# Youngju-Na/UFORecon

Hardware: AMD Instinct MI355X
Metric: rays/s (per-ray volume-rendering path, 64+64 hierarchical samples, DTU-shaped 3-view 512x640) (higher is better)
Workload: dtype f32; 1 GPU; configs[1]: full 512x640 frame = 327680 rays, 3 source views, 64+64 samples, rays sharded by row tiles over 1 GPU(s), depth/RGB tiles all-gathered; rays_per_frame=327680, chunk_rays=4096, side_streams=3

## Files before the change

uforecon_amd/csrc/composite.hip:

```cpp
#include "ufr_internal.h"

#pragma clang fp contract(off)

namespace ufr {

constexpr int kMaxK = 4;

__device__ __forceinline__ float sigmoidf(float x) { return 1.f / (1.f + expf(-x)); }

__device__ __forceinline__ float wave_sum(float v) {
#pragma unroll
  for (int d = 32; d >= 1; d >>= 1) v += __shfl_xor(v, d);
  return v;
}

__global__ void __launch_bounds__(256) composite_kernel(const float* __restrict__ z, const float* __restrict__ radiance,
                                                         const int* __restrict__ rad_row, const float* __restrict__ srdf,
                                                         const float* __restrict__ variance, int RN, int SN,
                                                         float* __restrict__ rgb, float* __restrict__ depth,
                                                         float* __restrict__ opacity, float* __restrict__ weight,
                                                         const float* __restrict__ camz, float* __restrict__ depth_z) {
  const int wave = threadIdx.x >> 6, lane = threadIdx.x & 63;
  const int ray = blockIdx.x * 4 + wave;
  if (ray >= RN) return;
  const float* zr = z + (size_t)ray * SN;
  const float* sr = srdf + (size_t)ray * SN;
  const float inv_s = fminf(fmaxf(expf(variance[0] * 10.0f), 1e-6f), 1e6f);
  const int K = (SN + 63) / 64;

  float alpha[kMaxK], zz[kMaxK];
  float prod = 1.f;
#pragma unroll
  for (int k = 0; k < kMaxK; ++k) {
    alpha[k] = 0.f;
    zz[k] = 0.f;
    int i = lane * K + k;
    if (k < K && i < SN) {
      float zc = zr[i];
      float gl = (i == 0) ? zr[1] - zr[0] : zc - zr[i - 1];
      float gr = (i == SN - 1) ? zr[SN - 1] - zr[SN - 2] : zr[i + 1] - zc;
      float interval = (gl + gr) / 2.f;
      float s = sr[i];
      const float iter_cos = -1.5f;
      float nxt = s + iter_cos * interval * 0.5f;
      float prv = s - iter_cos * interval * 0.5f;
      float pc = sigmoidf(prv * inv_s), nc = sigmoidf(nxt * inv_s);
      float a = ((pc - nc) + 1e-5f) / (pc + 1e-5f);
      a = fminf(fmaxf(a, 0.f), 1.f);
      alpha[k] = a;
      zz[k] = zc;
      prod *= (1.f - a) + 1e-7f;
    }
  }
  float incl = prod;
#pragma unroll
  for (int d = 1; d < 64; d <<= 1) {
    float o = __shfl_up(incl, d);
    if (lane >= d) incl *= o;
  }
  float T = __shfl_up(incl, 1);
  if (lane == 0) T = 1.f;

  float acc_d = 0.f, acc_o = 0.f, acc_r = 0.f, acc_g = 0.f, acc_b = 0.f;
#pragma unroll
  for (int k = 0; k < kMaxK; ++k) {
    int i = lane * K + k;
    if (k < K && i < SN) {
      float w = alpha[k] * T;
      T *= (1.f - alpha[k]) + 1e-7f;
      if (weight) weight[(size_t)ray * SN + i] = w;
      const float* c = radiance + (rad_row ? (size_t)rad_row[(size_t)ray * SN + i] : (size_t)ray * SN + i) * 3;
      acc_r += c[0] * w;
      acc_g += c[1] * w;
      acc_b += c[2] * w;
      acc_d += w * zz[k];
      acc_o += w;
    }
  }
  acc_d = wave_sum(acc_d);
  acc_o = wave_sum(acc_o);
  acc_r = wave_sum(acc_r);
  acc_g = wave_sum(acc_g);
  acc_b = wave_sum(acc_b);
  if (lane == 0) {
    depth[ray] = acc_d;
    if (opacity) opacity[ray] = acc_o;
    if (rgb) {
      rgb[3 * ray + 0] = acc_r;
      rgb[3 * ray + 1] = acc_g;
      rgb[3 * ray + 2] = acc_b;
    }
    if (depth_z) depth_z[ray] = acc_d * camz[ray];
  }
}

__global__ void __launch_bounds__(256) composite_bwd_kernel(const float* __restrict__ z, const float* __restrict__ radiance,
                                                             const int* __restrict__ rad_row, int accumulate,
                                                             const float* __restrict__ srdf,
                                                             const float* __restrict__ variance, int RN, int SN,
                                                             const float* __restrict__ d_rgb, const float* __restrict__ d_depth,
                                                             const float* __restrict__ d_opacity,
                                                             const float* __restrict__ d_weight,
                                                             float* __restrict__ d_radiance, float* __restrict__ d_srdf,
                                                             float* __restrict__ d_variance) {
  const int wave = threadIdx.x >> 6, lane = threadIdx.x & 63;
  const int ray = blockIdx.x * 4 + wave;
  if (ray >= RN) return;
  const float* zr = z + (size_t)ray * SN;
  const float* sr = srdf + (size_t)ray * SN;
  const float e10 = expf(variance[0] * 10.0f);
  const float inv_s = fminf(fmaxf(e10, 1e-6f), 1e6f);
  const bool s_live = e10 >= 1e-6f && e10 <= 1e6f;
  const int K = (SN + 63) / 64;
  const float gr = d_rgb ? d_rgb[3 * ray + 0] : 0.f, gg = d_rgb ? d_rgb[3 * ray + 1] : 0.f, gb = d_rgb ? d_rgb[3 * ray + 2] : 0.f;
  const float gd = d_depth ? d_depth[ray] : 0.f, go = d_opacity ? d_opacity[ray] : 0.f;

  float alpha[kMaxK], araw[kMaxK], pcv[kMaxK], ncv[kMaxK], prvv[kMaxK], nxtv[kMaxK];
  float prod = 1.f;
#pragma unroll
  for (int k = 0; k < kMaxK; ++k) {
    alpha[k] = 0.f; araw[k] = 0.f; pcv[k] = 0.f; ncv[k] = 0.f; prvv[k] = 0.f; nxtv[k] = 0.f;
    const int i = lane * K + k;
    if (k < K && i < SN) {
      const float zc = zr[i];
      const float gl = (i == 0) ? zr[1] - zr[0] : zc - zr[i - 1];
      const float gr_ = (i == SN - 1) ? zr[SN - 1] - zr[SN - 2] : zr[i + 1] - zc;
      const float interval = (gl + gr_) / 2.f;
      const float s = sr[i];
      const float nxt = s + -1.5f * interval * 0.5f, prv = s - -1.5f * interval * 0.5f;
      const float pc = sigmoidf(prv * inv_s), nc = sigmoidf(nxt * inv_s);
      const float a = ((pc - nc) + 1e-5f) / (pc + 1e-5f);
      araw[k] = a; pcv[k] = pc; ncv[k] = nc; prvv[k] = prv; nxtv[k] = nxt;
      alpha[k] = fminf(fmaxf(a, 0.f), 1.f);
      prod *= (1.f - alpha[k]) + 1e-7f;
    }
  }
  float incl = prod;
#pragma unroll
  for (int d = 1; d < 64; d <<= 1) {
    const float o = __shfl_up(incl, d);
    if (lane >= d) incl *= o;
  }
  float T = __shfl_up(incl, 1);
  if (lane == 0) T = 1.f;

  float w[kMaxK], dw[kMaxK], Tk[kMaxK], lane_sum = 0.f;
#pragma unroll
  for (int k = 0; k < kMaxK; ++k) {
    w[k] = 0.f; dw[k] = 0.f; Tk[k] = 0.f;
    const int i = lane * K + k;
    if (k < K && i < SN) {
      Tk[k] = T;
      w[k] = alpha[k] * T;
      T *= (1.f - alpha[k]) + 1e-7f;
      const size_t slot = (size_t)ray * SN + i, rrow = rad_row ? (size_t)rad_row[slot] : slot;
      const float* c = radiance + rrow * 3;
      dw[k] = (d_weight ? d_weight[slot] : 0.f) + gr * c[0] + gg * c[1] + gb * c[2] + gd * zr[i] + go;
      lane_sum += dw[k] * w[k];
      float* dr = d_radiance + rrow * 3;
      if (accumulate) { dr[0] += w[k] * gr; dr[1] += w[k] * gg; dr[2] += w[k] * gb; }
      else { dr[0] = w[k] * gr; dr[1] = w[k] * gg; dr[2] = w[k] * gb; }
    }
  }
  float suf = lane_sum;
#pragma unroll
  for (int d = 1; d < 64; d <<= 1) {
    const float o = __shfl_down(suf, d);
    if (lane + d < 64) suf += o;
  }
  float after = __shfl_down(suf, 1);
  if (lane == 63) after = 0.f;

  float dvar = 0.f;
#pragma unroll
  for (int k = kMaxK - 1; k >= 0; --k) {
    const int i = lane * K + k;
    if (k < K && i < SN) {
      const float dalpha = dw[k] * Tk[k] - after / ((1.f - alpha[k]) + 1e-7f);
      after += dw[k] * w[k];
      const float da = (araw[k] >= 0.f && araw[k] <= 1.f) ? dalpha : 0.f;
      const float den = pcv[k] + 1e-5f;
      const float dpc = da * (1.f - araw[k]) / den, dnc = -da / den;
      const float spc = pcv[k] * (1.f - pcv[k]), snc = ncv[k] * (1.f - ncv[k]);
      d_srdf[(size_t)ray * SN + i] = (dpc * spc + dnc * snc) * inv_s;
      dvar += dpc * spc * prvv[k] + dnc * snc * nxtv[k];
    }
  }
  dvar = wave_sum(dvar);
  if (lane == 0 && s_live) atomicAdd(d_variance, dvar * 10.f * inv_s);
}

hipError_t launch_composite_bwd(const float* z, const float* radiance, const int* rad_row, bool accumulate, const float* srdf,
                                const float* variance, int RN, int SN, const float* d_rgb, const float* d_depth,
                                const float* d_opacity, const float* d_weight, float* d_radiance, float* d_srdf,
                                float* d_variance, hipStream_t s) {
  if (SN > 64 * kMaxK || SN < 2) return hipErrorInvalidValue;
  hipLaunchKernelGGL(composite_bwd_kernel, dim3((RN + 3) / 4), dim3(256), 0, s, z, radiance, rad_row, accumulate ? 1 : 0, srdf,
                     variance, RN, SN, d_rgb,
                     d_depth, d_opacity, d_weight, d_radiance, d_srdf, d_variance);
  return hipGetLastError();
}

hipError_t launch_composite(const float* z, const float* radiance, const int* rad_row, const float* srdf,
                            const float* variance, int RN, int SN, float* rgb, float* depth, float* opacity, float* weight,
                            const float* camz, float* depth_z, hipStream_t s) {
  if (SN > 64 * kMaxK || SN < 2) return hipErrorInvalidValue;
  hipLaunchKernelGGL(composite_kernel, dim3((RN + 3) / 4), dim3(256), 0, s, z, radiance, rad_row, srdf, variance, RN, SN, rgb,
                     depth, opacity, weight, camz, depth_z);
  return hipGetLastError();
}

}
```

uforecon_amd/csrc/ray_transformer.hip:

```cpp
#include "bwd_tape.h"
#include "ufr_internal.h"
#include "weight_stream_f16.h"

namespace ufr {

__device__ __forceinline__ void load_ray_tile(const float* __restrict__ token0, const int* __restrict__ tok_row,
                                              const float* __restrict__ order_pe, size_t tok_base, int s_base, int g,
                                              int j, f32x4 (&x)[6]) {
  const float* row = token0 + (tok_row ? (size_t)tok_row[tok_base + j] : tok_base + j) * UFR_TOKEN_DIM;
#pragma unroll
  for (int t = 0; t < 5; ++t) x[t] = ld4(row + 16 * t + 4 * g);
  const float* pe = order_pe + (size_t)(s_base + j) * 8 + 2 * g;
  x[5] = f32x4{pe[0], pe[1], 0.f, 0.f};
}

template <int VW, int VB, int C, class WS>
__device__ __forceinline__ void layer_norm88(f32x4 (&tt)[C][6], const WS& ws, int g, float eps, float asc, f32x4 (*XH)[6] = nullptr, float* RS = nullptr) {
#pragma unroll
  for (int c = 0; c < C; ++c) {
    f32x4 (&t)[6] = tt[c];
    float s = 0.f;
#pragma unroll
    for (int i = 0; i < 5; ++i) s += (t[i][0] + t[i][1]) + (t[i][2] + t[i][3]);
    s += t[5][0] + t[5][1];
    const float mean = sum_groups(s) * (1.f / 88.f);
    float q = 0.f;
#pragma unroll
    for (int i = 0; i < 6; ++i)
#pragma unroll
      for (int r = 0; r < 4; ++r) {
        if (i < 5 || r < 2) {
          float d = t[i][r] - mean;
          q = fmaf(d, d, q);
        }
      }
    const float rstd = fast_rsqrt(sum_groups(q) * (1.f / 88.f) + eps);
    if (RS) RS[c] = rstd * asc;
#pragma unroll
    for (int i = 0; i < 6; ++i) {
      const f32x4 gw = vec_frag<VW>(ws, i, g), gb = vec_frag<VB>(ws, i, g);
#pragma unroll
      for (int r = 0; r < 4; ++r) {
        const float xh = (t[i][r] - mean) * rstd;
        if (XH) XH[c][i][r] = (i == 5 && r >= 2) ? 0.f : xh;
        t[i][r] = xh * gw[r] + gb[r];
      }
    }
  }
}

constexpr int kRtBlock = 256;
constexpr int kRtMinW = 2;
constexpr int kRtWaves = kRtBlock / 64;

#ifdef UFR_PHASE_TIMING
__device__ unsigned long long g_rt_phase[32];
#define UFR_RT_PHASE(i)                                                                \
  {                                                                                    \
    const unsigned long long t_now = __builtin_readcyclecounter();                     \
    rt_acc[i] += t_now - rt_prev;                                                      \
    rt_prev = t_now;                                                                   \
  }
#else
#define UFR_RT_PHASE(i)
#endif

template <bool LOWP, bool TAPE = false>
__global__ void __launch_bounds__(kRtBlock, TAPE ? 2 : kRtMinW) ray_transformer_kernel(const float* __restrict__ packed,
                                                                  const float* __restrict__ token0,
                                                                  const int* __restrict__ tok_row,
                                                                  const float* __restrict__ order_pe, int RN, int SN,
                                                                  float* __restrict__ srdf,
                                                                  float* __restrict__ ray_out,
                                                                  int* __restrict__ status, float* __restrict__ tape = nullptr,
                                                                  float* __restrict__ ray_state = nullptr) {
  extern __shared__ __attribute__((aligned(16))) char smem[];
  auto ws = wstream_f16_begin<kRtWaves, LOWP>(packed, smem);
  wstream_f16_prime<B_RT1, kRtWaves>(ws);
  const int lane = threadIdx.x & 63, g = lane >> 4, j = lane & 15;
  const int ray_raw = (blockIdx.x * blockDim.x + threadIdx.x) >> 6;
  const bool valid = ray_raw < RN;
  const int ray = valid ? ray_raw : RN - 1;
  const int n_tiles = SN / 16;
  const int n_iter = n_tiles;
  const auto sc = scalar_file<false, ray_scalars_offset()>(ws);
  const float xs_x = sc[RS_XS_X];
  const float k_dsc = sc[RS_K_DSC], k_l2e = sc[RS_K_L2E], q_dsc = sc[RS_Q_DSC], q_l2e = sc[RS_Q_L2E];
  const float inv_len = uniform_f32(sc[RS_V_DSC] / (float)SN), f_len = uniform_f32((float)SN * sc[RS_V_ASC]);
  const bool pow2_len = (SN & (SN - 1)) == 0;

#ifdef UFR_PHASE_TIMING
  unsigned long long rt_acc[16] = {};
  unsigned long long rt_prev = __builtin_readcyclecounter();
#endif
  f32x4 KV[8], KVT[TAPE ? 8 : 1];
#pragma unroll
  for (int h = 0; h < 8; ++h) KV[h] = splat4(0.f);
#pragma unroll
  for (int h = 0; h < (TAPE ? 8 : 1); ++h) KVT[h] = splat4(0.f);
  for (int it = 0; it < n_iter; ++it) {
    constexpr int C = 1;
    const bool wrap = it + 1 < n_iter;
    const bool slot_ok = head11_slot(j) >= 0;
    f32x4 x[C][6], kt[C][8], vt[C][8];
    bool live[C];
#pragma unroll
    for (int c = 0; c < C; ++c) {
      const int tile = it * C + c;
      live[c] = tile < n_tiles;
      const int tl = live[c] ? tile : n_tiles - 1;
      load_ray_tile(token0, tok_row, order_pe, (size_t)ray * SN + tl * 16, tl * 16, g, j, x[c]);
#pragma unroll
      for (int h = 0; h < 8; ++h) { kt[c][h] = splat4(0.f); vt[c][h] = splat4(0.f); }
    }
    {
      BWords<C> cur;
      split_units<0, 0, 4 * C>(x, cur, xs_x);
      static_for<3>([&](auto si) __attribute__((always_inline)) {
        constexpr int s = decltype(si)::value;
        BStep b[C];
        bwords_to_bstep(cur, b);
        if constexpr (s < 2) {
          BWords<C> nxt;
          gemm_f16_panel<M_RT_K, s, C, kRtWaves, true>(ws, b, kt, wrap, [&](auto ti) __attribute__((always_inline)) {
            constexpr int to = decltype(ti)::value;
            split_units<s + 1, to * 4 * C / 8, (to + 1) * 4 * C / 8>(x, nxt, xs_x);
          });
          gemm_f16_panel<M_RT_V, s, C, kRtWaves, true>(ws, b, vt, wrap);
          cur = nxt;
        } else {
          gemm_f16_panel<M_RT_K, s, C, kRtWaves, true>(ws, b, kt, wrap);
          gemm_f16_panel<M_RT_V, s, C, kRtWaves, true>(ws, b, vt, wrap);
        }
      });
      probe_gemm(kt, ws);
      probe_gemm(vt, ws);
    }
    UFR_RT_PHASE(0)
    const float pad_v = (TAPE ? j == 3 : (j & 3) == 3) ? 1.f : 0.f;
#pragma unroll
    for (int c = 0; c < C; ++c) {
      float kk[8][4], vv[8][4];
      if (pow2_len) {
#pragma unroll
        for (int h = 0; h < 8; ++h)
#pragma unroll
          for (int r = 0; r < 4; ++r) vv[h][r] = vt[c][h][r] * inv_len;
      } else {
#pragma unroll
        for (int h = 0; h < 8; ++h)
#pragma unroll
          for (int r = 0; r < 4; ++r) vv[h][r] = vt[c][h][r] / f_len;
      }
      const bool k_ok = slot_ok && live[c];
#pragma unroll
      for (int h = 0; h < 8; ++h)
#pragma unroll
        for (int r = 0; r < 4; ++r) {
          const float e = elu1_acc(kt[c][h][r], k_dsc, k_l2e);
          kk[h][r] = k_ok ? e : 0.f;
          vv[h][r] = slot_ok ? vv[h][r] : pad_v;
        }
#pragma unroll
      for (int r = 0; r < 4; ++r) {
#pragma unroll
        for (int h = 0; h < 8; ++h) {
          KV[h] = mfma16(kk[h][r], vv[h][r], KV[h]);
          if constexpr (TAPE) KVT[h] = mfma16(vv[h][r], kk[h][r], KVT[h]);
        }
      }
    }
    wstream_f16_finish<B_RT1, kRtWaves>(ws, wrap);
    UFR_RT_PHASE(1)
  }

  if constexpr (TAPE) {
    if (valid) {
      float* st = ray_state + (size_t)ray * (kRayStateTiles * kTileFloats) + lane * 4;
#pragma unroll
      for (int h = 0; h < 8; ++h) { st4(st + h * kTileFloats, KV[h]); st4(st + (8 + h) * kTileFloats, KVT[h]); }
    }
  }
  wstream_f16_prime<B_RT2, kRtWaves>(ws);
  constexpr int C = 1;
  const int n_iter2 = TAPE ? n_iter + (n_iter & 1) : n_iter;
  typedef RayTapeLayout<LOWP> TapeL;
  for (int it = 0; it < n_iter2; ++it) {
    const bool wrap = it + 1 < n_iter2;
    char* const tape_blk = reinterpret_cast<char*>(tape) + ((size_t)ray * (n_iter2 / 2) + it / 2) * (TapeL::block_units * 512);
    auto tape_st = [&](int tile, f32x4 v) __attribute__((always_inline)) {
      if (valid) tile_store<TapeL>(tape_blk, tile, it & 1, lane, v);
    };
    f32x4 x[C][6], q[C][6], msg[C][6];
    bool live[C];
    int tbase[C];
#pragma unroll
    for (int c = 0; c < C; ++c) {
      const int tile = it * C + c;
      live[c] = tile < n_tiles;
      tbase[c] = (live[c] ? tile : n_tiles - 1) * 16;
      load_ray_tile(token0, tok_row, order_pe, (size_t)ray * SN + tbase[c], tbase[c], g, j, x[c]);
#pragma unroll
      for (int t = 0; t < 6; ++t) q[c][t] = splat4(0.f);
    }
    track_external(x, ws);
    gemm_f16<M_RT_Q, C, kRtWaves>(ws, x, q, wrap, xs_x);
    float zs_all[8];
    if constexpr (TAPE) {
#pragma unroll
      for (int t = 0; t < 6; ++t) {
        tape_st(RT_X + t, live[0] ? x[0][t] : splat4(0.f));
        f32x4 qq;
#pragma unroll
        for (int r = 0; r < 4; ++r) qq[r] = quad11(t, g, r) >= 0 ? elu1_acc(q[0][t][r], q_dsc, q_l2e) : 0.f;
        tape_st(RT_Q + t, qq);
      }
    }
    UFR_RT_PHASE(2)
#pragma unroll
    for (int c = 0; c < C; ++c) {
      static_for<8>([&](auto hi) __attribute__((always_inline)) {
        constexpr int h = decltype(hi)::value;
        f32x4 acc = splat4(0.f);
        static_for<3>([&](auto qi) __attribute__((always_inline)) {
          constexpr int qd = decltype(qi)::value, quad = 3 * h + qd;
          const float qq = (3 * g + qd < 11) ? elu1_acc(q[c][quad >> 2][quad & 3], q_dsc, q_l2e) : 0.f;
          acc = mfma16(KV[h][qd], qq, acc);
        });
        const float den = TAPE ? __shfl(acc[3], j) : acc[3];
        const float Z = fast_rcp(den + 1e-6f);
        const float zs = Z * (float)SN;
        if constexpr (TAPE) zs_all[h] = zs;
        static_for<3>([&](auto ri) __attribute__((always_inline)) {
          constexpr int rr = decltype(ri)::value, quad = 3 * h + rr;
          msg[c][quad >> 2][quad & 3] = acc[rr] * zs;
        });
      });
    }
    UFR_RT_PHASE(3)
    if constexpr (TAPE) {
#pragma unroll
      for (int t = 0; t < 6; ++t) tape_st(RT_MSG + t, msg[0][t]);
      tape_st(RT_ZS, f32x4{zs_all[0], zs_all[1], zs_all[2], zs_all[3]});
      tape_st(RT_ZS + 1, f32x4{zs_all[4], zs_all[5], zs_all[6], zs_all[7]});
    }
    f32x4 m[C][6];
#pragma unroll
    for (int c = 0; c < C; ++c)
#pragma unroll
      for (int t = 0; t < 6; ++t) m[c][t] = splat4(0.f);
    gemm_f16<M_RT_MERGE, C, kRtWaves>(ws, msg, m, wrap, sc[RS_M_XS]);
    UFR_RT_PHASE(4)
    float rstd1[C] = {}, rstd2[C] = {};
    if constexpr (TAPE) {
      f32x4 xh[C][6];
      layer_norm88<V_RT_N1W, V_RT_N1B, C>(m, ws, g, sc[RS_EPS1], sc[RS_M_ASC], xh, rstd1);
#pragma unroll
      for (int t = 0; t < 6; ++t) { tape_st(RT_XH1 + t, xh[0][t]); tape_st(RT_M + t, m[0][t]); }
    } else {
      layer_norm88<V_RT_N1W, V_RT_N1B, C>(m, ws, g, sc[RS_EPS1], 1.f);
    }
    UFR_RT_PHASE(5)

    f32x4 cat[C][12], hid[C][11], o[C][6];
#pragma unroll
    for (int c = 0; c < C; ++c) {
#pragma unroll
      for (int t = 0; t < 6; ++t) { cat[c][t] = x[c][t]; cat[c][6 + t] = m[c][t]; }
#pragma unroll
      for (int t = 0; t < 11; ++t) hid[c][t] = splat4(0.f);
    }
    gemm_f16<M_RT_MLP0, C, kRtWaves>(ws, cat, hid, wrap, xs_x);
    UFR_RT_PHASE(6)
#pragma unroll
    for (int c = 0; c < C; ++c) {
#pragma unroll
      for (int t = 0; t < 11; ++t)
#pragma unroll
        for (int r = 0; r < 4; ++r) hid[c][t][r] = relu_acc(hid[c][t][r]);
#pragma unroll
      for (int t = 0; t < 6; ++t) o[c][t] = splat4(0.f);
    }
    unsigned relu_bits[2] = {0u, 0u};
    if constexpr (TAPE) {
#pragma unroll
      for (int t = 0; t < 11; ++t) {
        tape_st(RT_HID + t, hid[0][t] * sc[RS_MLP0_DSC]);
#pragma unroll
        for (int r = 0; r < 4; ++r)
          if (hid[0][t][r] > 0.f) relu_bits[(4 * t + r) >> 5] |= 1u << ((4 * t + r) & 31);
      }
    }
    gemm_f16<M_RT_MLP2, C, kRtWaves>(ws, hid, o, wrap, sc[RS_M_MLP2]);
    UFR_RT_PHASE(7)
    if constexpr (TAPE) {
      f32x4 xh[C][6];
      layer_norm88<V_RT_N2W, V_RT_N2B, C>(o, ws, g, sc[RS_EPS2], sc[RS_MLP2_ASC], xh, rstd2);
#pragma unroll
      for (int t = 0; t < 6; ++t) tape_st(RT_XH2 + t, xh[0][t]);
    } else {
      layer_norm88<V_RT_N2W, V_RT_N2B, C>(o, ws, g, sc[RS_EPS2], 1.f);
    }
    UFR_RT_PHASE(8)
#pragma unroll
    for (int c = 0; c < C; ++c) {
#pragma unroll
      for (int t = 0; t < 6; ++t)
#pragma unroll
        for (int r = 0; r < 4; ++r) o[c][t][r] += x[c][t][r];
      if constexpr (TAPE) {
#pragma unroll
        for (int t = 0; t < 6; ++t) tape_st(RT_O + t, o[c][t]);
      }
      if (ray_out && valid && live[c]) {
        float* row = ray_out + ((size_t)ray * SN + tbase[c] + j) * UFR_RAY_DIM;
#pragma unroll
        for (int t = 0; t < 5; ++t) st4(row + 16 * t + 4 * g, o[c][t]);
        row[80 + 2 * g] = o[c][5][0];
        row[81 + 2 * g] = o[c][5][1];
      }
    }

    f32x4 d1[C][2], d2[C][1], d3[C][1];
#pragma unroll
    for (int c = 0; c < C; ++c) {
      d1[c][0] = vec_frag<V_DM_B0>(ws, 0, g) * sc[RS_DM0_ASC];
      d1[c][1] = vec_frag<V_DM_B0>(ws, 1, g) * sc[RS_DM0_ASC];
      d2[c][0] = vec_frag<V_DM_B2>(ws, 0, g) * sc[RS_DM2_ASC];
      d3[c][0] = vec_frag<V_DM_B4>(ws, 0, g) * sc[RS_DM4_ASC];
    }
    gemm_f16<M_DM0, C, kRtWaves>(ws, o, d1, wrap, sc[RS_DM0_XS]);
#pragma unroll
    for (int c = 0; c < C; ++c)
#pragma unroll
      for (int t = 0; t < 2; ++t)
#pragma unroll
        for (int r = 0; r < 4; ++r) d1[c][t][r] = relu_acc(d1[c][t][r]);
    gemm_f16<M_DM2, C, kRtWaves>(ws, d1, d2, wrap, sc[RS_M_DM2]);
#pragma unroll
    for (int c = 0; c < C; ++c)
#pragma unroll
      for (int r = 0; r < 4; ++r) d2[c][0][r] = relu_acc(d2[c][0][r]);
    if constexpr (TAPE) {
#pragma unroll
      for (int t = 0; t < 2; ++t) {
        tape_st(RT_D1 + t, d1[0][t] * sc[RS_DM0_DSC]);
#pragma unroll
        for (int r = 0; r < 4; ++r)
          if (d1[0][t][r] > 0.f) relu_bits[(44 + 4 * t + r) >> 5] |= 1u << ((44 + 4 * t + r) & 31);
      }
      tape_st(RT_D2, d2[0][0] * sc[RS_DM2_DSC]);
#pragma unroll
      for (int r = 0; r < 4; ++r)
        if (d2[0][0][r] > 0.f) relu_bits[1] |= 1u << (52 + r - 32);
      tape_st(RT_MISC, f32x4{rstd1[0], rstd2[0], __builtin_bit_cast(float, relu_bits[0]), __builtin_bit_cast(float, relu_bits[1])});
    }
    gemm_f16<M_DM4, C, kRtWaves>(ws, d2, d3, wrap, sc[RS_M_DM4]);
#pragma unroll
    for (int c = 0; c < C; ++c)
      if (g == 0 && valid && live[c]) srdf[(size_t)ray * SN + tbase[c] + j] = d3[c][0][0] * sc[RS_DM4_DSC];
    wstream_f16_finish<B_RT2, kRtWaves>(ws, wrap);
    UFR_RT_PHASE(9)
  }
  wstream_report_range(ws, status);
#ifdef UFR_PHASE_TIMING
  if (ray_raw == 5 && lane == 0)
    for (int i = 0; i < 16; ++i) g_rt_phase[i] += rt_acc[i];
#endif
}

template <bool LOWP, bool TAPE = false>
static hipError_t launch_rt(const float* packed, const float* token0, const int* tok_row, const float* order_pe, int RN,
                            int SN, float* srdf, float* ray_out, int* status, hipStream_t s, float* tape = nullptr,
                            float* ray_state = nullptr) {
  static LdsAttrOnce lds_attr;
  if (const hipError_t attr = lds_attr.set(reinterpret_cast<const void*>(&ray_transformer_kernel<LOWP, TAPE>), kF16LdsBytes); attr != hipSuccess) return attr;
  hipLaunchKernelGGL((ray_transformer_kernel<LOWP, TAPE>), dim3((RN + kRtWaves - 1) / kRtWaves), dim3(kRtBlock), kF16LdsBytes, s,
                     packed, token0, tok_row, order_pe, RN, SN, srdf, ray_out, status, tape, ray_state);
  return hipGetLastError();
}

hipError_t launch_ray_tape(const float* packed, const float* token0, const int* tok_row, const float* order_pe, int RN, int SN,
                           float* srdf, float* tape, float* ray_state, bool lowp, int* status, hipStream_t s) {
  if (SN % 16 != 0 || SN < 16) return hipErrorInvalidValue;
  return lowp ? launch_rt<true, true>(packed, token0, tok_row, order_pe, RN, SN, srdf, nullptr, status, s, tape, ray_state)
              : launch_rt<false, true>(packed, token0, tok_row, order_pe, RN, SN, srdf, nullptr, status, s, tape, ray_state);
}

hipError_t launch_ray_transformer(const float* packed, const float* token0, const int* tok_row, const float* order_pe,
                                  int RN, int SN, float* srdf, float* ray_out, bool lowp, int* status, hipStream_t s) {
  if (SN % 16 != 0 || SN < 16) return hipErrorInvalidValue;
  return lowp ? launch_rt<true>(packed, token0, tok_row, order_pe, RN, SN, srdf, ray_out, status, s)
              : launch_rt<false>(packed, token0, tok_row, order_pe, RN, SN, srdf, ray_out, status, s);
}

}

#ifdef UFR_PHASE_TIMING
extern "C" int ufr_debug_rt_phases(unsigned long long* out, int n, int reset) {
  unsigned long long h[32] = {};
  if (hipMemcpyFromSymbol(h, HIP_SYMBOL(ufr::g_rt_phase), sizeof(h)) != hipSuccess) return -1;
  for (int i = 0; i < n && i < 32; ++i) out[i] = h[i];
  if (reset) {
    unsigned long long z[32] = {};
    if (hipMemcpyToSymbol(HIP_SYMBOL(ufr::g_rt_phase), z, sizeof(z)) != hipSuccess) return -1;
  }
  return 0;
}
#endif
```

uforecon_amd/csrc/sampler.hip:

```cpp
#include "ufr_internal.h"

#pragma clang fp contract(off)

namespace ufr {

__global__ void __launch_bounds__(256) ray_setup_kernel(const int64_t* __restrict__ ray_idx,
                                                         const float* __restrict__ ray_d,
                                                         const float* __restrict__ cam_ray_d, int HW, float near_z,
                                                         float far_z, int RN, float* __restrict__ rd_out,
                                                         float* __restrict__ near_out, float* __restrict__ far_out,
                                                         float* __restrict__ camz_out, float ox, float oy, float oz,
                                                         float* __restrict__ ray_o_out) {
  int i = blockIdx.x * blockDim.x + threadIdx.x;
  if (i == 0 && ray_o_out) { ray_o_out[0] = ox; ray_o_out[1] = oy; ray_o_out[2] = oz; }
  if (i >= RN) return;
  int64_t p = ray_idx[i];
  const bool in_range = p >= 0 && p < (int64_t)HW;
  p = in_range ? p : 0;
  rd_out[3 * i + 0] = ray_d[p];
  rd_out[3 * i + 1] = ray_d[(size_t)HW + p];
  rd_out[3 * i + 2] = ray_d[2 * (size_t)HW + p];
  float cz = cam_ray_d ? cam_ray_d[2 * (size_t)HW + p] : 1.f;
  const float bad = __builtin_nanf("");
  near_out[i] = !in_range ? bad : cam_ray_d ? near_z / cz : near_z;
  far_out[i] = !in_range ? bad : cam_ray_d ? far_z / cz : far_z;
  if (camz_out) camz_out[i] = cz;
}

hipError_t launch_ray_setup(const int64_t* ray_idx, const float* ray_d, const float* cam_ray_d, int HW, float near_z,
                            float far_z, int RN, float* rd_out, float* near_out, float* far_out, float* camz_out,
                            const float* ray_o_host, float* ray_o_out, hipStream_t s) {
  hipLaunchKernelGGL(ray_setup_kernel, dim3((RN + 255) / 256), dim3(256), 0, s, ray_idx, ray_d, cam_ray_d, HW, near_z,
                     far_z, RN, rd_out, near_out, far_out, camz_out, ray_o_host ? ray_o_host[0] : 0.f,
                     ray_o_host ? ray_o_host[1] : 0.f, ray_o_host ? ray_o_host[2] : 0.f, ray_o_out);
  return hipGetLastError();
}

__global__ void __launch_bounds__(256) sample_fixed_kernel(const float* __restrict__ near,
                                                            const float* __restrict__ far,
                                                            const float* __restrict__ U, int u_stride,
                                                            float* __restrict__ z, int RN, int SN) {
  size_t i = (size_t)blockIdx.x * blockDim.x + threadIdx.x;
  if (i >= (size_t)RN * SN) return;
  int s = (int)(i / RN), ray = (int)(i % RN);
  double step = 1.0 / (double)(SN - 1);
  float lin = (s == SN - 1) ? 1.0f : (float)((double)s * step);
  float n = near[ray], f = far[ray];
  float zz = lin * (f - n) + n;
  float interval = (float)(1.0 / (double)(SN - 1));
  zz = zz + (U[(size_t)s * u_stride + ray] - 0.5f) * interval * (f - n);
  z[(size_t)ray * SN + s] = zz;
}

hipError_t launch_sample_fixed(const float* near, const float* far, const float* U, int u_stride, float* z, int RN,
                               int SN, hipStream_t s) {
  size_t n = (size_t)RN * SN;
  hipLaunchKernelGGL(sample_fixed_kernel, dim3((unsigned)((n + 255) / 256)), dim3(256), 0, s, near, far, U, u_stride, z,
                     RN, SN);
  return hipGetLastError();
}

__global__ void __launch_bounds__(256) points_kernel(const float* __restrict__ ray_o, int o_stride,
                                                      const float* __restrict__ ray_d, const float* __restrict__ z,
                                                      float* __restrict__ pts, int RN, int SN) {
  size_t i = (size_t)blockIdx.x * blockDim.x + threadIdx.x;
  if (i >= (size_t)RN * SN) return;
  int ray = (int)(i / SN);
  float zz = z[i];
  const float* o = ray_o + (size_t)ray * o_stride;
  pts[3 * i + 0] = o[0] + zz * ray_d[3 * ray + 0];
  pts[3 * i + 1] = o[1] + zz * ray_d[3 * ray + 1];
  pts[3 * i + 2] = o[2] + zz * ray_d[3 * ray + 2];
}

hipError_t launch_points(const float* ray_o, int o_stride, const float* ray_d, const float* z, float* pts, int RN,
                         int SN, hipStream_t s) {
  size_t n = (size_t)RN * SN;
  hipLaunchKernelGGL(points_kernel, dim3((unsigned)((n + 255) / 256)), dim3(256), 0, s, ray_o, o_stride, ray_d, z, pts,
                     RN, SN);
  return hipGetLastError();
}

constexpr int kMaxS = 256;

__device__ __forceinline__ double wave_incl_scan(double v, int lane) {
#pragma unroll
  for (int d = 1; d < 64; d <<= 1) {
    double o = __shfl_up(v, d);
    if (lane >= d) v += o;
  }
  return v;
}

__global__ void __launch_bounds__(256) importance_merge_kernel(const float* __restrict__ weight,
                                                                const float* __restrict__ z,
                                                                const float* __restrict__ U2, int u_stride,
                                                                float* __restrict__ z_fine, float* __restrict__ z_all,
                                                                int RN, int SN, int PN, float* __restrict__ z_new,
                                                                int* __restrict__ src_row) {
  __shared__ float lds[4][3 * kMaxS];
  const int wave = threadIdx.x >> 6, lane = threadIdx.x & 63;
  const int ray = blockIdx.x * 4 + wave;
  const bool active = ray < RN;
  float* cdf = lds[wave];
  float* all = cdf + kMaxS;
  float* zf = all + SN;
  const float* w = weight + (size_t)(active ? ray : 0) * SN;

  const int K = (SN + 63) / 64;
  double run = 0.0;
  for (int k = 0; k < K; ++k) {
    int i = lane * K + k;
    if (i < SN) run += (double)w[i];
  }
  double incl = wave_incl_scan(run, lane);
  float total;
  {
    float a4[4] = {0.f, 0.f, 0.f, 0.f};
    const int l8 = lane & 7;
    for (int c = 0; c * 32 < SN; ++c)
#pragma unroll
      for (int k = 0; k < 4; ++k) {
        int i = (c * 4 + k) * 8 + l8;
        if (i < SN) a4[k] += w[i];
      }
    const float t = ((a4[0] + a4[1]) + a4[2]) + a4[3];
    total = __shfl(t, 0);
#pragma unroll
    for (int l = 1; l < 8; ++l) total += __shfl(t, l);
  }
  float denom = total + 1e-6f;
  double acc = incl - run;
  for (int k = 0; k < K; ++k) {
    int i = lane * K + k;
    if (i < SN) {
      acc += (double)w[i];
      cdf[i] = (float)acc / denom;
      all[i] = z[(size_t)(active ? ray : 0) * SN + i];
    }
  }
  __syncthreads();

  const float c_first = cdf[0], c_last = cdf[SN - 1];
  for (int k = lane; k < PN; k += 64) {
    float u = U2[(size_t)k * u_stride + (active ? ray : 0)];
    u = fminf(fmaxf(u, c_first), c_last);
    int lo = 0, hi = SN;
    while (lo < hi) {
      int mid = (lo + hi) >> 1;
      if (cdf[mid] < u) lo = mid + 1; else hi = mid;
    }
    int ri = lo < 1 ? 1 : (lo > SN - 1 ? SN - 1 : lo);
    float cl = cdf[ri - 1], cr = cdf[ri], zl = all[ri - 1], zr = all[ri];
    zf[k] = (u - cl) / (cr - cl + 1e-6f) * (zr - zl) + zl;
  }
  __syncthreads();
  if (!active) return;

  if (z_fine) {
    for (int k = lane; k < PN; k += 64) {
      float v = zf[k];
      int rank = 0;
      for (int j = 0; j < PN; ++j) {
        float o = zf[j];
        rank += (o < v || (o == v && j < k)) ? 1 : 0;
      }
      z_fine[(size_t)ray * PN + rank] = v;
    }
  }
  const int T = SN + PN;
  float* out = z_all + (size_t)ray * T;
  bool sorted_coarse = true;
  for (int k = lane; k + 1 < SN; k += 64) sorted_coarse = sorted_coarse && all[k] <= all[k + 1];
  if (__builtin_amdgcn_ballot_w64(!sorted_coarse) == 0ull) {
    float* fs = cdf;
    for (int k = lane; k < PN; k += 64) {
      const float v = zf[k];
      int r = 0;
      for (int j = 0; j < PN; ++j) {
        const float o = zf[j];
        r += (o < v || (o == v && j < k)) ? 1 : 0;
      }
      fs[r] = v;
    }
    __builtin_amdgcn_fence(__ATOMIC_RELEASE, "wavefront");
    __builtin_amdgcn_wave_barrier();
    __builtin_amdgcn_fence(__ATOMIC_ACQUIRE, "wavefront");
    for (int k = lane; k < SN; k += 64) {
      const float v = all[k];
      int lo = 0, hi = PN;
      while (lo < hi) { const int mid = (lo + hi) >> 1; if (fs[mid] < v) lo = mid + 1; else hi = mid; }
      const int rank = k + lo;
      out[rank] = v;
      if (src_row) src_row[(size_t)ray * T + rank] = ray * SN + k;
    }
    for (int r = lane; r < PN; r += 64) {
      const float v = fs[r];
      int lo = 0, hi = SN;
      while (lo < hi) { const int mid = (lo + hi) >> 1; if (all[mid] <= v) lo = mid + 1; else hi = mid; }
      const int rank = r + lo;
      out[rank] = v;
      if (src_row) src_row[(size_t)ray * T + rank] = RN * SN + ray * PN + r;
      if (z_new) z_new[(size_t)ray * PN + r] = v;
    }
    return;
  }
  for (int k = lane; k < T; k += 64) {
    float v = all[k];
    int rank = 0, rank_new = 0;
    for (int j = 0; j < T; ++j) {
      float o = all[j];
      const int before = (o < v || (o == v && j < k)) ? 1 : 0;
      rank += before;
      rank_new += j >= SN ? before : 0;
    }
    out[rank] = v;
    if (src_row) src_row[(size_t)ray * T + rank] = k < SN ? ray * SN + k : RN * SN + ray * PN + rank_new;
    if (z_new && k >= SN) z_new[(size_t)ray * PN + rank_new] = v;
  }
}

hipError_t launch_importance_merge(const float* weight, const float* z, const float* U2, int u_stride, float* z_fine,
                                   float* z_all, int RN, int SN, int PN, float* z_new, int* src_row, hipStream_t s) {
  if (SN > kMaxS || PN > kMaxS || SN < 2) return hipErrorInvalidValue;
  hipLaunchKernelGGL(importance_merge_kernel, dim3((RN + 3) / 4), dim3(256), 0, s, weight, z, U2, u_stride, z_fine,
                     z_all, RN, SN, PN, z_new, src_row);
  return hipGetLastError();
}

}
```

uforecon_amd/csrc/ufr_api.hip:

```cpp
#include <math.h>
#include <stdarg.h>
#include <stdio.h>
#include <stdlib.h>
#include <string.h>

#include <atomic>
#include <mutex>
#include <string>
#include <vector>

#include "bwd_common.h"
#include "bwd_tape.h"
#include "mcubes_table.h"
#include "ufr_internal.h"
#include "ufr_layout_f16.h"

using namespace ufr;

namespace {

thread_local char g_err[512] = "";

int fail(int code, const char* fmt, ...) {
  va_list ap;
  va_start(ap, fmt);
  vsnprintf(g_err, sizeof(g_err), fmt, ap);
  va_end(ap);
  return code;
}
#define UFR_HIP(expr)                                                                    \
  do {                                                                                   \
    hipError_t e_ = (expr);                                                              \
    if (e_ != hipSuccess) return fail(UFR_ERR_HIP, "%s: %s", #expr, hipGetErrorString(e_)); \
  } while (0)
#define UFR_REQUIRE(cond, ...) \
  do {                         \
    if (!(cond)) return fail(UFR_ERR_ARG, __VA_ARGS__); \
  } while (0)

inline size_t align_up(size_t v, size_t a = 256) { return (v + a - 1) / a * a; }

struct Carver {
  char* base;
  size_t off = 0;
  explicit Carver(void* p) : base(static_cast<char*>(p)) {}
  float* f32(size_t n) {
    float* r = base ? reinterpret_cast<float*>(base + off) : nullptr;
    off += align_up(n * sizeof(float));
    return r;
  }
};

struct ProfEntry { const char* name; hipEvent_t a, b; };
std::atomic<bool> g_prof_on{false};
std::vector<ProfEntry> g_prof;
std::mutex g_prof_mu;

struct ProfScope {
  hipStream_t s;
  hipEvent_t a = nullptr, b = nullptr;
  const char* name;
  ProfScope(const char* n, hipStream_t st) : s(st), name(n) {
    if (g_prof_on.load(std::memory_order_relaxed)) {
      hipEventCreate(&a);
      hipEventCreate(&b);
      hipEventRecord(a, s);
    }
  }
  ~ProfScope() {
    if (a) {
      hipEventRecord(b, s);
      std::lock_guard<std::mutex> lock(g_prof_mu);
      g_prof.push_back({name, a, b});
    }
  }
};

__global__ void order_pe_kernel(float* __restrict__ table, int SN) {
  int i = blockIdx.x * blockDim.x + threadIdx.x;
  if (i >= SN * 8) return;
  int pos = i >> 3, jj = i & 7;
  double ang = (double)pos / pow(10000.0, 2.0 * (double)(jj / 2) / 8.0);
  table[i] = (float)((jj & 1) ? cos(ang) : sin(ang));
}

PreSim presim_of(const ufr_raw_weights* r) {
  return PreSim{r->pre_sim.w0, r->pre_sim.b0, r->pre_sim.w2, r->pre_sim.b2, r->pre_sim.w4, r->pre_sim.b4};
}

const FrameDev* frame_of(const ufr_frame* f) {
  const FrameDev* d = reinterpret_cast<const FrameDev*>(f);
  return (f && d->magic == kFrameMagic) ? d : nullptr;
}

}

namespace ufr {
hipError_t launch_order_pe(float* table, int SN, hipStream_t s) {
  hipLaunchKernelGGL(order_pe_kernel, dim3((SN * 8 + 255) / 256), dim3(256), 0, s, table, SN);
  return hipGetLastError();
}
}

namespace {
std::atomic<int> g_matrix_precision{UFR_PRECISION_FP32};

bool resolve_precision(int precision, bool* lowp) {
  if (precision == UFR_PRECISION_DEFAULT) precision = g_matrix_precision.load(std::memory_order_relaxed);
  if (precision != UFR_PRECISION_FP32 && precision != UFR_PRECISION_16BIT) return false;
  *lowp = precision == UFR_PRECISION_16BIT;
  return true;
}
#define UFR_PRECISION(arg, lowp_var, who)                                                        \
  bool lowp_var = false;                                                                          \
  if (!resolve_precision(arg, &lowp_var)) return fail(UFR_ERR_ARG, "%s: unknown precision %d", who, (int)(arg))

struct StatusSlot {
  std::once_flag once;
  int rc = UFR_OK;
  int* dev = nullptr;
  volatile int* host = nullptr;
  std::atomic<int> gen{0};
  std::mutex report_mu;
  hipEvent_t upd = nullptr;
  std::atomic<bool> upd_recorded{false};
};
constexpr int kStatusDevices = 16;
StatusSlot g_status[kStatusDevices];
constexpr int kStatusAll = 7;

__global__ void status_update_kernel(int* dev, int keep_mask, int gen) {
  atomicAnd(dev, keep_mask);
  dev[1] = gen;
}

int status_slot(StatusSlot** out) {
  int dev = 0;
  UFR_HIP(hipGetDevice(&dev));
  UFR_REQUIRE(dev >= 0 && dev < kStatusDevices, "status: device %d out of range", dev);
  StatusSlot& sl = g_status[dev];
  std::call_once(sl.once, [&sl] {
    int* h = nullptr;
    int* d = nullptr;
    if (hipHostMalloc(reinterpret_cast<void**>(&h), 2 * sizeof(int), hipHostMallocDefault) != hipSuccess ||
        hipMalloc(reinterpret_cast<void**>(&d), 2 * sizeof(int)) != hipSuccess || hipMemset(d, 0, 2 * sizeof(int)) != hipSuccess) {
      sl.rc = UFR_ERR_HIP;
      return;
    }
    h[0] = h[1] = 0;
    sl.host = h;
    sl.dev = d;
    if (hipEventCreateWithFlags(&sl.upd, hipEventDisableTiming) != hipSuccess) sl.upd = nullptr;
  });
  if (sl.rc != UFR_OK) return fail(sl.rc, "status: could not allocate the device's status words");
  *out = &sl;
  return UFR_OK;
}

int status_message(int bits, const char* who) {
  return fail(UFR_ERR_RANGE, "%s: range status 0x%x:%s%s%s (include/ufr.h: ufr_status_poll)", who, bits,
              (bits & 1) ? " a dense-layer input left the range of its fp16 planes (a token feature beyond the input_abs_max the weights were packed for -- ufr_weights_pack_for -- or infinite);" : "",
              (bits & 2) ? " NaN among the token / dir inputs handed to a transformer kernel;" : "",
              (bits & 4) ? " ufr_weights_pack met a parameter that is not finite (or an input bound that is not a positive finite number);" : "");
}

int status_consume(StatusSlot* sl, hipStream_t s, int mask, const char* who, int* flags_out) {
  std::lock_guard<std::mutex> lock(sl->report_mu);
  const int bits = sl->host[0], tag = sl->host[1];
  const int cur = sl->gen.load(std::memory_order_relaxed);
  const int hit = tag == cur ? bits & mask : 0;
  if (flags_out) *flags_out = tag == cur ? bits : 0;
  if (hit == 0) return UFR_OK;
  const int next = cur + 1;
  sl->gen.store(next, std::memory_order_relaxed);
  hipLaunchKernelGGL(status_update_kernel, dim3(1), dim3(1), 0, s, sl->dev, ~hit, next);
  UFR_HIP(hipGetLastError());
  if (sl->upd && hipEventRecord(sl->upd, s) == hipSuccess) sl->upd_recorded.store(true, std::memory_order_release);
  return status_message(hit, who);
}
int status_enter(StatusSlot* sl, hipStream_t s, const char* who) { return status_consume(sl, s, kStatusAll, who, nullptr); }
int status_fetch(StatusSlot* sl, hipStream_t s) {
  if (sl->upd_recorded.load(std::memory_order_acquire)) UFR_HIP(hipStreamWaitEvent(s, sl->upd, 0));
  UFR_HIP(hipMemcpyAsync(const_cast<int*>(sl->host), sl->dev, 2 * sizeof(int), hipMemcpyDeviceToHost, s));
  return UFR_OK;
}
int status_leave(StatusSlot* sl, hipStream_t s) { return status_fetch(sl, s); }
}

extern "C" {

int ufr_set_matrix_precision(int mode) {
  UFR_REQUIRE(mode == UFR_PRECISION_FP32 || mode == UFR_PRECISION_16BIT, "ufr_set_matrix_precision: unknown mode %d", mode);
  g_matrix_precision.store(mode, std::memory_order_relaxed);
  return UFR_OK;
}
int ufr_get_matrix_precision(void) { return g_matrix_precision.load(std::memory_order_relaxed); }

int ufr_status_poll_bits(ufr_stream stream, int32_t synchronize, int32_t mask, int32_t* flags_out) {
  StatusSlot* sl = nullptr;
  int rc = status_slot(&sl);
  if (rc != UFR_OK) return rc;
  hipStream_t s = static_cast<hipStream_t>(stream);
  if (synchronize) {
    rc = status_fetch(sl, s);
    if (rc != UFR_OK) return rc;
    UFR_HIP(hipStreamSynchronize(s));
  }
  int flags = 0;
  rc = status_consume(sl, s, mask, "ufr_status_poll", &flags);
  if (flags_out) *flags_out = flags;
  if (rc == UFR_OK && !synchronize) return status_leave(sl, s);
  return rc;
}

int ufr_status_poll(ufr_stream stream, int32_t synchronize, int32_t* flags_out) {
  return ufr_status_poll_bits(stream, synchronize, kStatusAll, flags_out);
}

int ufr_version(void) { return UFR_ABI_VERSION; }
const char* ufr_last_error(void) { return g_err; }

size_t ufr_packed_weights_bytes(void) { return (size_t)blob_floats() * sizeof(float) + (size_t)kF16Bytes + (size_t)kBwdBytes + 16; }
size_t ufr_packed_bwd_halfwords(void) { return (size_t)kBwdHalfwords; }
size_t ufr_packed_fp32_floats(void) { return (size_t)blob_floats(); }
size_t ufr_packed_f16_halfwords(void) { return (size_t)kF16Halfwords; }
size_t ufr_packed_scale_table_offset(void) { return (size_t)scale_table_offset(); }
int ufr_packed_scale_table_entries(void) { return M_COUNT; }

int ufr_pack_plan_f16(int32_t* param_id, int32_t* elem, int32_t* plane) {
  UFR_REQUIRE(param_id && elem && plane, "ufr_pack_plan_f16: null output");
  for (int h = 0; h < kF16Halfwords; ++h) plan_entry_f16(h, &param_id[h], &elem[h], &plane[h]);
  return UFR_OK;
}

int ufr_pack_plan_bwd(int32_t* param_id, int32_t* elem, int32_t* plane) {
  UFR_REQUIRE(param_id && elem && plane, "ufr_pack_plan_bwd: null output");
  for (int h = 0; h < kBwdHalfwords; ++h) plan_entry_f16(kF16Halfwords + h, &param_id[h], &elem[h], &plane[h]);
  return UFR_OK;
}

int ufr_pack_plan(int32_t* param_id, int32_t* elem) {
  UFR_REQUIRE(param_id && elem, "ufr_pack_plan: null output");
  for (int i = 0; i < blob_floats(); ++i) {
    int p, e;
    plan_entry(i, &p, &e);
    param_id[i] = p;
    elem[i] = e;
  }
  return UFR_OK;
}

int ufr_weights_pack_for(const ufr_raw_weights* raw, void* packed, float input_abs_max, ufr_stream stream) {
  UFR_REQUIRE(raw && packed, "ufr_weights_pack: null argument");
  static_assert(sizeof(ufr_raw_weights) == sizeof(RawPtrs), "ufr_raw_weights must be P_COUNT pointers");
  RawPtrs rp;
  memcpy(&rp, raw, sizeof(rp));
  for (int i = 0; i < P_COUNT; ++i) UFR_REQUIRE(rp.p[i], "ufr_weights_pack: parameter %d is null", i);
  UFR_REQUIRE(input_abs_max > 0.f && input_abs_max <= 3.0e38f, "ufr_weights_pack_for: input_abs_max=%g must be positive and finite",
              (double)input_abs_max);
  hipStream_t s = static_cast<hipStream_t>(stream);
  StatusSlot* sl = nullptr;
  int rc = status_slot(&sl);
  if (rc != UFR_OK) return rc;
  UFR_HIP(launch_pack_weights(rp, static_cast<float*>(packed), input_abs_max, sl->dev, s));
  return status_leave(sl, s);
}

int ufr_weights_fit_frame(void* packed, const ufr_frame* frame, ufr_stream stream) {
  const FrameDev* f = frame_of(frame);
  UFR_REQUIRE(packed && f, "ufr_weights_fit_frame: null weights / frame handle not prepared");
  hipStream_t s = static_cast<hipStream_t>(stream);
  StatusSlot* sl = nullptr;
  int rc = status_slot(&sl);
  if (rc != UFR_OK) return rc;
  UFR_HIP(launch_refit_weights(static_cast<float*>(packed), f->abs_max, sl->dev, s));
  return UFR_OK;
}

int ufr_weights_pack(const ufr_raw_weights* raw, void* packed, ufr_stream stream) {
  return ufr_weights_pack_for(raw, packed, kDefaultInputAbsMax, stream);
}

static int frame_check(const ufr_frame_desc* d) {
  UFR_REQUIRE(d, "frame desc is null");
  UFR_REQUIRE(d->NV >= 2 && d->NV <= UFR_MAX_VIEWS, "NV=%d unsupported (2..%d)", d->NV, UFR_MAX_VIEWS);
  UFR_REQUIRE(d->H >= 8 && d->W >= 8 && d->H % 4 == 0 && d->W % 4 == 0, "H,W must be multiples of 4 (got %dx%d)",
              d->H, d->W);
  UFR_REQUIRE(d->source_imgs && d->depth_info && d->feat, "null frame tensor");
  UFR_REQUIRE((long long)d->H * d->W < (1 << 24) && (long long)(d->H / 4) * (d->W / 4) * 32 * (d->NV - 1) < (1ll << 32),
              "image of %dx%d is too large for the gather's 24-bit texel indices", d->H, d->W);
  {
    const long long px = (long long)d->H * d->W, mpx = (long long)(d->H / 4) * (d->W / 4), lim = 1ll << 31;
    UFR_REQUIRE(px * 16 < lim && d->NV * mpx * 128 < lim && d->NV * mpx * 32 * (d->NV - 1) * 4 < lim,
                "frame of %dx%d with %d views: an image / feature-map buffer reaches 2 GiB (the gathers' zero-fill offset)",
                d->H, d->W, d->NV);
  }
  const bool has_vol = d->vol_feat[0] != nullptr;
  for (int s = 0; s < UFR_NUM_STAGES; ++s) {
    UFR_REQUIRE((d->vol_feat[s] != nullptr) == has_vol && (d->vol_weight[s] != nullptr) == has_vol,
                "volumes must be given for all stages or for none (stage %d)", s + 1);
    if (has_vol) UFR_REQUIRE(d->vol_D[s] >= 2 && d->vol_H[s] >= 2 && d->vol_W[s] >= 2, "degenerate volume (stage %d)", s + 1);
    if (has_vol)
      UFR_REQUIRE((long long)d->vol_D[s] * d->vol_H[s] < (1 << 24) && (long long)d->vol_W[s] * kVolCh < (1 << 24) &&
                      (long long)d->vol_D[s] * d->vol_H[s] * d->vol_W[s] * kVolCh * 4 < (1ll << 31),
                  "volume of stage %d is too large for the gather's 31-bit byte offsets (per view: < 2 GiB)", s + 1);
  }
  UFR_REQUIRE(d->source_poses && d->source_cam_pos && d->ref_cam_pos && d->w2c_row2, "null camera constants");
  return UFR_OK;
}

size_t ufr_frame_workspace_bytes(const ufr_frame_desc* d) {
  if (frame_check(d) != UFR_OK) return 0;
  Carver c(nullptr);
  const size_t h = d->H / 4, w = d->W / 4, NV = d->NV;
  c.f32(NV * h * w * 32);
  if (d->match) c.f32(NV * h * w * 32 * (NV - 1));
  c.f32(NV * (size_t)d->H * d->W * 4);
  if (d->vol_feat[0])
    for (int s = 0; s < UFR_NUM_STAGES; ++s) c.f32(NV * (size_t)d->vol_D[s] * d->vol_H[s] * d->vol_W[s] * kVolCh);
  c.f32(64);
  return c.off;
}

int ufr_frame_prepare(const ufr_frame_desc* d, void* workspace, size_t workspace_bytes, ufr_frame* out,
                      ufr_stream stream) {
  int rc = frame_check(d);
  if (rc != UFR_OK) return rc;
  UFR_REQUIRE(workspace && out, "ufr_frame_prepare: null workspace/out");
  if (workspace_bytes < ufr_frame_workspace_bytes(d))
    return fail(UFR_ERR_WORKSPACE, "frame workspace too small: %zu < %zu", workspace_bytes, ufr_frame_workspace_bytes(d));
  hipStream_t s = static_cast<hipStream_t>(stream);
  const int NV = d->NV, h = d->H / 4, w = d->W / 4;
  Carver c(workspace);
  const bool has_vol = d->vol_feat[0] != nullptr;
  float* feat = c.f32((size_t)NV * h * w * 32);
  float* match = d->match ? c.f32((size_t)NV * h * w * 32 * (NV - 1)) : nullptr;
  float* rgb = c.f32((size_t)NV * d->H * d->W * 4);
  float* vol[UFR_NUM_STAGES] = {};
  if (has_vol)
    for (int st = 0; st < UFR_NUM_STAGES; ++st)
      vol[st] = c.f32((size_t)NV * d->vol_D[st] * d->vol_H[st] * d->vol_W[st] * kVolCh);
  unsigned* abs_max = reinterpret_cast<unsigned*>(c.f32(64));

  UFR_HIP(hipMemsetAsync(abs_max, 0, 256, s));
  UFR_HIP(launch_nchw_to_nhwc(d->feat, feat, NV, 32, h * w, 32, s, abs_max));
  if (match) UFR_HIP(launch_nchw_to_nhwc(d->match, match, NV, 32 * (NV - 1), h * w, 32 * (NV - 1), s));
  UFR_HIP(launch_nchw_to_nhwc(d->source_imgs, rgb, NV, 3, d->H * d->W, 4, s));
  if (has_vol)
    for (int st = 0; st < UFR_NUM_STAGES; ++st)
      UFR_HIP(launch_volume_pack(d->vol_feat[st], d->vol_weight[st], vol[st], NV, d->vol_D[st] * d->vol_H[st] * d->vol_W[st], s, abs_max));

  FrameDev f;
  memset(&f, 0, sizeof(f));
  f.NV = NV; f.H = d->H; f.W = d->W; f.h = h; f.w = w; f.match_ch = 32 * (NV - 1);
  f.feat = feat; f.match = match; f.rgb = rgb; f.depth = d->depth_info;
  for (int st = 0; st < UFR_NUM_STAGES; ++st) {
    f.vol[st] = vol[st];
    if (has_vol) { f.vD[st] = d->vol_D[st]; f.vH[st] = d->vol_H[st]; f.vW[st] = d->vol_W[st]; }
  }
  for (int v = 0; v < NV; ++v) {
    memcpy(f.pose[v], d->source_poses + 16 * v, 12 * sizeof(float));
    memcpy(f.cam_pos[v], d->source_cam_pos + 3 * v, 3 * sizeof(float));
    memcpy(f.w2c_z[v], d->w2c_row2 + 4 * v, 4 * sizeof(float));
  }
  memcpy(f.ref_pos, d->ref_cam_pos, 3 * sizeof(float));
  f.vol_near = d->vol_near; f.vol_far = d->vol_far;
  f.abs_max = abs_max;
  f.magic = kFrameMagic;
  memset(out, 0, sizeof(*out));
  memcpy(out, &f, sizeof(f));
  return UFR_OK;
}

int ufr_sample_fixed(const float* near, const float* far, const float* U, float* z_out, int32_t RN, int32_t SN,
                     ufr_stream stream) {
  UFR_REQUIRE(near && far && U && z_out, "ufr_sample_fixed: null argument");
  UFR_REQUIRE(RN > 0 && SN >= 2, "ufr_sample_fixed: RN=%d SN=%d", RN, SN);
  UFR_HIP(launch_sample_fixed(near, far, U, RN, z_out, RN, SN, static_cast<hipStream_t>(stream)));
  return UFR_OK;
}

int ufr_sample_importance_merge(const float* weight, const float* z, const float* U2, float* z_fine, float* z_all,
                                int32_t RN, int32_t SN, int32_t PN, ufr_stream stream) {
  UFR_REQUIRE(weight && z && U2 && z_all, "ufr_sample_importance_merge: null argument");
  UFR_REQUIRE(RN > 0 && SN >= 2 && SN <= 256 && PN >= 1 && PN <= 256, "ufr_sample_importance_merge: RN=%d SN=%d PN=%d",
              RN, SN, PN);
  UFR_HIP(launch_importance_merge(weight, z, U2, RN, z_fine, z_all, RN, SN, PN, nullptr, nullptr,
                                  static_cast<hipStream_t>(stream)));
  return UFR_OK;
}

int ufr_points(const float* ray_o, int32_t ray_o_stride, const float* ray_d, const float* z, float* points, int32_t RN,
               int32_t SN, ufr_stream stream) {
  UFR_REQUIRE(ray_o && ray_d && z && points, "ufr_points: null argument");
  UFR_REQUIRE(ray_o_stride == 0 || ray_o_stride == 3, "ufr_points: ray_o_stride must be 0 or 3");
  UFR_HIP(launch_points(ray_o, ray_o_stride, ray_d, z, points, RN, SN, static_cast<hipStream_t>(stream)));
  return UFR_OK;
}

int ufr_project_gather(const ufr_frame* frame, const ufr_raw_weights* raw, const float* ray_o, int32_t ray_o_stride,
                       const float* ray_d, const float* z, int32_t RN, int32_t SN, float* x_tokens, float* rgb,
                       float* dir, float* sim8, float* vol24, float* xy, float* mask_z, const float* vol24_in,
                       const float* sim8_in, ufr_stream stream) {
  const FrameDev* f = frame_of(frame);
  UFR_REQUIRE(f, "ufr_project_gather: frame handle not prepared");
  UFR_REQUIRE(raw && ray_o && ray_d && z && x_tokens && rgb && dir, "ufr_project_gather: null argument");
  UFR_REQUIRE(ray_o_stride == 0 || ray_o_stride == 3, "ufr_project_gather: ray_o_stride must be 0 or 3");
  UFR_REQUIRE(RN > 0 && SN > 0, "ufr_project_gather: RN=%d SN=%d", RN, SN);
  UFR_REQUIRE(f->match || sim8_in, "ufr_project_gather: the frame has no matching features: sim8_in is required");
  UFR_REQUIRE(f->vol[0] || vol24_in, "ufr_project_gather: the frame has no volumes: vol24_in is required");
  ProfScope prof("gather", static_cast<hipStream_t>(stream));
  UFR_HIP(launch_gather(*f, presim_of(raw), ray_o, ray_o_stride, ray_d, z, RN, SN, x_tokens, nullptr, rgb, dir, sim8, vol24, xy,
                        mask_z, vol24_in, sim8_in, static_cast<hipStream_t>(stream)));
  return UFR_OK;
}

size_t ufr_aggregate_workspace_bytes(int32_t RN, int32_t SN, int32_t NV) {
  (void)NV;
  Carver c(nullptr);
  c.f32((size_t)RN * SN * UFR_TOKEN_DIM);
  c.f32((size_t)SN * 8);
  return c.off;
}

static int aggregate_impl(const void* packed, const float* x_tokens, const float* x_point, const float* rgb, const float* dir, int RN, int SN,
                          int NV, float* radiance, float* srdf, float* token0, float* order_pe, bool pe_ready,
                          float* view_out, float* ray_out, bool lowp, int* status, hipStream_t s) {
  UFR_REQUIRE((unsigned long long)RN * SN * (NV + 1) * UFR_TOKEN_DIM < (1ull << 30),
              "view transformer: %d x %d points x %d tokens exceed the 2^30 token values one call addresses; chunk the points", RN, SN, NV + 1);
  {
    ProfScope ps("view_transformer", s);
    UFR_HIP(launch_view_transformer(static_cast<const float*>(packed), x_tokens, x_point, rgb, dir, RN * SN, NV, token0, radiance,
                                    view_out, lowp, status, s));
  }
  if (!pe_ready) UFR_HIP(launch_order_pe(order_pe, SN, s));
  {
    ProfScope ps("ray_transformer", s);
    UFR_HIP(launch_ray_transformer(static_cast<const float*>(packed), token0, nullptr, order_pe, RN, SN, srdf, ray_out, lowp,
                                   status, s));
  }
  return UFR_OK;
}

int ufr_aggregate(const void* packed_weights, const float* x_tokens, const float* rgb, const float* dir, int32_t RN,
                  int32_t SN, int32_t NV, float* radiance, float* srdf, void* workspace, float* view_out,
                  float* ray_out, int32_t precision, ufr_stream stream) {
  UFR_REQUIRE(packed_weights && x_tokens && rgb && dir && radiance && srdf && workspace, "ufr_aggregate: null argument");
  UFR_REQUIRE(NV >= 2 && NV <= UFR_MAX_VIEWS, "ufr_aggregate: NV=%d unsupported", NV);
  UFR_REQUIRE(RN > 0 && SN >= 16 && SN % 16 == 0 && SN <= 256, "ufr_aggregate: SN=%d must be a multiple of 16 in [16,256]", SN);
  UFR_PRECISION(precision, lowp, "ufr_aggregate");
  hipStream_t s = static_cast<hipStream_t>(stream);
  StatusSlot* sl = nullptr;
  int rc = status_slot(&sl);
  if (rc == UFR_OK) rc = status_enter(sl, s, "ufr_aggregate");
  if (rc != UFR_OK) return rc;
  Carver c(workspace);
  float* token0 = c.f32((size_t)RN * SN * UFR_TOKEN_DIM);
  float* order_pe = c.f32((size_t)SN * 8);
  rc = aggregate_impl(packed_weights, x_tokens, nullptr, rgb, dir, RN, SN, NV, radiance, srdf, token0, order_pe, false, view_out,
                      ray_out, lowp, sl->dev, s);
  return rc != UFR_OK ? rc : status_leave(sl, s);
}

int ufr_composite(const float* z, const float* radiance, const int32_t* row, const float* srdf, const float* variance,
                  int32_t RN, int32_t SN, float* rgb, float* depth, float* opacity, float* weight, ufr_stream stream) {
  UFR_REQUIRE(z && radiance && srdf && variance && depth, "ufr_composite: null argument");
  UFR_REQUIRE(RN > 0 && SN >= 2 && SN <= 256, "ufr_composite: SN=%d out of range [2,256]", SN);
  ProfScope prof("composite", static_cast<hipStream_t>(stream));
  UFR_HIP(launch_composite(z, radiance, row, srdf, variance, RN, SN, rgb, depth, opacity, weight, nullptr, nullptr,
                           static_cast<hipStream_t>(stream)));
  return UFR_OK;
}

static int raw_and_grads(const ufr_raw_weights* raw, const ufr_raw_grads* grads, RawPtrs& rp, GradPtrs& gp, const char* who) {
  static_assert(sizeof(ufr_raw_grads) == sizeof(GradPtrs) && UFR_NUM_PARAMS == P_COUNT, "ufr_raw_grads layout");
  UFR_REQUIRE(raw && grads, "%s: null weights / grads", who);
  memcpy(&rp, raw, sizeof(rp));
  memcpy(&gp, grads, sizeof(gp));
  for (int i = 0; i < P_COUNT; ++i) UFR_REQUIRE(rp.p[i] && gp.p[i], "%s: parameter %d has a null pointer", who, i);
  return UFR_OK;
}

int ufr_composite_bwd(const float* z, const float* radiance, const int32_t* row, const float* srdf, const float* variance,
                      int32_t RN, int32_t SN, const float* d_rgb, const float* d_depth, const float* d_opacity,
                      const float* d_weight, float* d_radiance, int32_t accumulate, float* d_srdf, float* d_variance,
                      ufr_stream stream) {
  UFR_REQUIRE(z && radiance && srdf && variance && d_radiance && d_srdf && d_variance, "ufr_composite_bwd: null argument");
  UFR_REQUIRE(RN > 0 && SN >= 2 && SN <= 256, "ufr_composite_bwd: SN=%d out of range [2,256]", SN);
  hipStream_t s = static_cast<hipStream_t>(stream);
  ProfScope p("composite_bwd", s);
  UFR_HIP(launch_composite_bwd(z, radiance, row, accumulate != 0, srdf, variance, RN, SN, d_rgb, d_depth, d_opacity, d_weight,
                               d_radiance, d_srdf, d_variance, s));
  return UFR_OK;
}

int ufr_render_loss(const float* rgb_c, const float* depth_c, const float* rgb_f, const float* depth_f, const float* rgb_gt,
                    const float* depth_gt, const float* near_far, int32_t nf_stride, int32_t B, int32_t RN, float weight_rgb,
                    float weight_depth, float* loss, float* d_rgb_c, float* d_depth_c, float* d_rgb_f, float* d_depth_f,
                    ufr_stream stream) {
  UFR_REQUIRE(rgb_c && depth_c && rgb_f && depth_f && rgb_gt && depth_gt && near_far && loss && d_rgb_c && d_depth_c && d_rgb_f && d_depth_f,
              "ufr_render_loss: null argument");
  UFR_REQUIRE(B > 0 && RN > 0 && nf_stride >= 2 && (long long)B * RN < (1ll << 24), "ufr_render_loss: B=%d RN=%d nf_stride=%d", B, RN, nf_stride);
  hipStream_t s = static_cast<hipStream_t>(stream);
  ProfScope p("render_loss", s);
  UFR_HIP(launch_render_loss(rgb_c, depth_c, rgb_f, depth_f, rgb_gt, depth_gt, near_far, nf_stride, B, RN, weight_rgb, weight_depth,
                             loss, d_rgb_c, d_depth_c, d_rgb_f, d_depth_f, s));
  return UFR_OK;
}

struct ViewBwdWs { float *tape, *dbuf, *token0, *radiance; int blocks; };
static ViewBwdWs carve_view_bwd(Carver& c, int P, int NV) {
  ViewBwdWs w;
  w.blocks = view_tape_blocks(P, NV);
  w.tape = c.f32((size_t)w.blocks * ViewTapeLayout<false>::block_units * 128);
  w.dbuf = c.f32((size_t)w.blocks * ViewGradLayout<false>::block_units * 128);
  w.token0 = c.f32((size_t)P * UFR_TOKEN_DIM);
  w.radiance = c.f32((size_t)P * 3);
  return w;
}
static int view_bwd_impl(const void* packed, const GradPtrs& gp, const float* x_tokens, const float* rgb, const float* dir,
                         const float* d_tok_a, const float* d_tok_b, const float* d_radiance, int P, int NV, float* d_pv,
                         const ViewBwdWs& w, bool lowp, int* status, hipStream_t s, int stages = UFR_BWD_STAGE_ALL) {
  UFR_REQUIRE((unsigned long long)P * (NV + 1) * UFR_TOKEN_DIM < (1ull << 30),
              "view transformer backward: %d points x %d tokens exceed the 2^30 token values one call addresses; chunk the points", P, NV + 1);
  const float* pk = static_cast<const float*>(packed);
  if (stages & UFR_BWD_STAGE_TAPE) {
    ProfScope p("view_tape", s);
    UFR_HIP(launch_view_tape(pk, x_tokens, rgb, dir, P, NV, w.token0, w.radiance, w.tape, lowp, status, s));
  }
  if (stages & UFR_BWD_STAGE_DGRAD) {
    ProfScope p("view_dgrad", s);
    UFR_HIP(launch_view_dgrad(pk, w.tape, rgb, d_tok_a, d_tok_b, d_radiance, P, NV, w.dbuf, d_pv, gp, lowp, s));
  }
  if (stages & UFR_BWD_STAGE_WGRAD) {
    ProfScope p("view_wgrad", s);
    UFR_HIP(launch_view_wgrad(w.tape, w.dbuf, w.blocks, gp, lowp, s));
  }
  return UFR_OK;
}

struct RayBwdWs { float *order_pe, *tape, *state, *dbuf, *srdf; int blocks; };
static RayBwdWs carve_ray_bwd(Carver& c, int RN, int SN) {
  RayBwdWs w;
  w.blocks = RN * ((SN / 16 + 1) / 2);
  w.order_pe = c.f32((size_t)SN * 8);
  w.tape = c.f32((size_t)w.blocks * RayTapeLayout<false>::block_units * 128);
  w.state = c.f32((size_t)RN * kRayStateTiles * kTileFloats);
  w.dbuf = c.f32((size_t)w.blocks * RayGradLayout<false>::block_units * 128);
  w.srdf = c.f32((size_t)RN * SN);
  return w;
}
static int ray_bwd_impl(const void* packed, const GradPtrs& gp, const float* token0, const int* row, bool accumulate,
                        const float* d_srdf, int RN, int SN, float* d_tok_a, float* d_tok_b, const RayBwdWs& w, bool lowp,
                        int* status, hipStream_t s, int stages = UFR_BWD_STAGE_ALL) {
  const float* pk = static_cast<const float*>(packed);
  if (stages & UFR_BWD_STAGE_TAPE) {
    UFR_HIP(launch_order_pe(w.order_pe, SN, s));
    ProfScope p("ray_tape", s);
    UFR_HIP(launch_ray_tape(pk, token0, row, w.order_pe, RN, SN, w.srdf, w.tape, w.state, lowp, status, s));
  }
  if (stages & UFR_BWD_STAGE_DGRAD) {
    ProfScope p("ray_dgrad", s);
    UFR_HIP(launch_ray_dgrad(pk, w.tape, w.state, d_srdf, row, accumulate, RN, SN, w.dbuf, d_tok_a, d_tok_b, gp, lowp, s));
  }
  if (stages & UFR_BWD_STAGE_WGRAD) {
    ProfScope p("ray_wgrad", s);
    UFR_HIP(launch_ray_wgrad(w.tape, w.dbuf, w.blocks, gp, lowp, s));
  }
  return UFR_OK;
}

size_t ufr_ray_transform_bwd_workspace_bytes(int32_t RN, int32_t SN) {
  if (RN <= 0 || SN < 16 || SN % 16 != 0) return 0;
  Carver c(nullptr);
  carve_ray_bwd(c, RN, SN);
  return c.off;
}

size_t ufr_view_transform_bwd_workspace_bytes(int32_t P, int32_t NV) {
  if (P <= 0 || NV < 2 || NV > UFR_MAX_VIEWS) return 0;
  Carver c(nullptr);
  carve_view_bwd(c, P, NV);
  return c.off;
}

size_t ufr_aggregate_bwd_workspace_bytes(int32_t RN, int32_t SN, int32_t NV) {
  if (RN <= 0 || SN <= 0 || NV < 2 || NV > UFR_MAX_VIEWS) return 0;
  if (SN < 16 || SN % 16 != 0) return 0;
  Carver c(nullptr);
  c.f32((size_t)RN * SN * UFR_TOKEN_DIM);
  carve_ray_bwd(c, RN, SN);
  carve_view_bwd(c, RN * SN, NV);
  return c.off;
}

int ufr_aggregate_bwd(const ufr_raw_weights* raw, const ufr_raw_grads* grads, const void* packed_weights, const float* x_tokens,
                      const float* rgb, const float* dir, const float* token0, int32_t RN, int32_t SN, int32_t NV,
                      const float* d_radiance, const float* d_srdf, float* d_pv, void* workspace,
                      int32_t precision, ufr_stream stream) {
  RawPtrs rp;
  GradPtrs gp;
  int rc = raw_and_grads(raw, grads, rp, gp, "ufr_aggregate_bwd");
  if (rc != UFR_OK) return rc;
  UFR_PRECISION(precision, lowp, "ufr_aggregate_bwd");
  UFR_REQUIRE(packed_weights && x_tokens && rgb && dir && token0 && d_radiance && d_srdf && d_pv && workspace, "ufr_aggregate_bwd: null argument");
  UFR_REQUIRE(NV >= 2 && NV <= UFR_MAX_VIEWS, "ufr_aggregate_bwd: NV=%d unsupported", NV);
  UFR_REQUIRE(RN > 0 && SN >= 16 && SN % 16 == 0 && SN <= 256, "ufr_aggregate_bwd: SN=%d must be a multiple of 16 in [16,256]", SN);
  hipStream_t s = static_cast<hipStream_t>(stream);
  Carver c(workspace);
  float* d_tok = c.f32((size_t)RN * SN * UFR_TOKEN_DIM);
  const RayBwdWs rw = carve_ray_bwd(c, RN, SN);
  const ViewBwdWs vw = carve_view_bwd(c, RN * SN, NV);
  StatusSlot* sl = nullptr;
  rc = status_slot(&sl);
  if (rc != UFR_OK) return rc;
  rc = ray_bwd_impl(packed_weights, gp, token0, nullptr, false, d_srdf, RN, SN, d_tok, nullptr, rw, lowp, sl->dev, s);
  if (rc != UFR_OK) return rc;
  return view_bwd_impl(packed_weights, gp, x_tokens, rgb, dir, d_tok, nullptr, d_radiance, RN * SN, NV, d_pv, vw, lowp, sl->dev, s);
}

size_t ufr_project_gather_bwd_workspace_bytes(const ufr_frame* frame) {
  const FrameDev* f = frame_of(frame);
  return (f && f->vol[0]) ? align_up(gather_bwd_scratch_floats(*f) * sizeof(float)) : 0;
}

int ufr_project_gather_bwd(const ufr_frame* frame, const ufr_raw_weights* raw, const ufr_raw_grads* grads,
                           const float* ray_o, int32_t ray_o_stride, const float* ray_d, const float* z, int32_t RN,
                           int32_t SN, const float* sim8, const float* d_pv, const int32_t* row,
                           float* const* grad_vol_feat, float* const* grad_vol_weight, int32_t accumulate, void* workspace,
                           int32_t precision, ufr_stream stream) {
  const FrameDev* f = frame_of(frame);
  UFR_REQUIRE(f, "ufr_project_gather_bwd: frame handle not prepared");
  UFR_PRECISION(precision, lowp, "ufr_project_gather_bwd");
  RawPtrs rp;
  GradPtrs gp;
  int rc = raw_and_grads(raw, grads, rp, gp, "ufr_project_gather_bwd");
  if (rc != UFR_OK) return rc;
  UFR_REQUIRE(ray_o && ray_d && z && sim8 && d_pv, "ufr_project_gather_bwd: null argument");
  const bool scatter = grad_vol_feat != nullptr || grad_vol_weight != nullptr;
  UFR_REQUIRE(!scatter || (grad_vol_feat && grad_vol_weight && f->vol[0]),
              "ufr_project_gather_bwd: volume gradients need both pointer arrays and a frame prepared with volumes");
  UFR_REQUIRE(ray_o_stride == 0 || ray_o_stride == 3, "ufr_project_gather_bwd: ray_o_stride must be 0 or 3");
  UFR_REQUIRE(RN > 0 && SN > 0, "ufr_project_gather_bwd: RN=%d SN=%d", RN, SN);
  for (int i = 0; scatter && i < UFR_NUM_STAGES; ++i)
    UFR_REQUIRE(grad_vol_feat[i] && grad_vol_weight[i], "ufr_project_gather_bwd: null volume gradient (stage %d)", i + 1);
  UFR_REQUIRE(!scatter || workspace, "ufr_project_gather_bwd: the volume scatter needs its workspace");
  hipStream_t s = static_cast<hipStream_t>(stream);
  if (scatter) {
    ProfScope p("gather_bwd", s);
    UFR_HIP(launch_gather_bwd(*f, grad_vol_feat, grad_vol_weight, ray_o, ray_o_stride, ray_d, z, d_pv, row, RN, SN,
                              static_cast<float*>(workspace), (accumulate & UFR_GBWD_ACCUMULATE) != 0,
                              (accumulate & UFR_GBWD_WORKSPACE_ZEROED) != 0, s));
  }
  if (!(accumulate & UFR_GBWD_NO_PRESIM)) {
    ProfScope p("presim_bwd", s);
    UFR_HIP(launch_presim_bwd(rp, gp, sim8, d_pv, RN * SN, lowp, s));
  }
  return UFR_OK;
}

int ufr_sample_importance_pool(const float* weight, const float* z, const float* U2, float* z_all, float* z_new,
                               int32_t* row, int32_t RN, int32_t SN, int32_t PN, ufr_stream stream) {
  UFR_REQUIRE(weight && z && U2 && z_all && z_new && row, "ufr_sample_importance_pool: null argument");
  UFR_REQUIRE(RN > 0 && SN >= 2 && SN <= 256 && PN >= 1 && PN <= 256, "ufr_sample_importance_pool: RN=%d SN=%d PN=%d", RN, SN, PN);
  UFR_HIP(launch_importance_merge(weight, z, U2, RN, nullptr, z_all, RN, SN, PN, z_new, row, static_cast<hipStream_t>(stream)));
  return UFR_OK;
}

int ufr_view_transform(const void* packed_weights, const float* x_tokens, const float* rgb, const float* dir, int32_t P,
                       int32_t NV, float* token0, float* radiance, int32_t precision, ufr_stream stream) {
  UFR_REQUIRE(packed_weights && x_tokens && rgb && dir && token0 && radiance, "ufr_view_transform: null argument");
  UFR_REQUIRE(NV >= 2 && NV <= UFR_MAX_VIEWS && P > 0, "ufr_view_transform: P=%d NV=%d", P, NV);
  UFR_PRECISION(precision, lowp, "ufr_view_transform");
  hipStream_t s = static_cast<hipStream_t>(stream);
  StatusSlot* sl = nullptr;
  int rc = status_slot(&sl);
  if (rc == UFR_OK) rc = status_enter(sl, s, "ufr_view_transform");
  if (rc != UFR_OK) return rc;
  {
    ProfScope p("view_transformer", s);
    UFR_REQUIRE((unsigned long long)P * (NV + 1) * UFR_TOKEN_DIM < (1ull << 30),
                "ufr_view_transform: %d points x %d tokens exceed the 2^30 token values one call addresses; chunk the points", P, NV + 1);
    UFR_HIP(launch_view_transformer(static_cast<const float*>(packed_weights), x_tokens, nullptr, rgb, dir, P, NV, token0, radiance,
                                    nullptr, lowp, sl->dev, s));
  }
  return status_leave(sl, s);
}

int32_t ufr_view_tape_block_points(int32_t NV) {
  return (NV >= 2 && NV <= UFR_MAX_VIEWS) ? (16 / (NV + 1)) * kBlockCols : 0;
}

int ufr_view_transform_tape(const void* packed_weights, const float* x_tokens, const float* rgb, const float* dir, int32_t P,
                            int32_t NV, float* token0, float* radiance, void* workspace, int32_t p0, int32_t P_total,
                            int32_t precision, ufr_stream stream) {
  UFR_REQUIRE(packed_weights && x_tokens && rgb && dir && token0 && radiance && workspace, "ufr_view_transform_tape: null argument");
  UFR_REQUIRE(NV >= 2 && NV <= UFR_MAX_VIEWS && P > 0 && p0 >= 0 && p0 + P <= P_total, "ufr_view_transform_tape: P=%d p0=%d P_total=%d NV=%d",
              P, p0, P_total, NV);
  const int ppw = ufr_view_tape_block_points(NV);
  UFR_REQUIRE(p0 % ppw == 0 && (p0 + P == P_total || P % ppw == 0),
              "ufr_view_transform_tape: the point range [%d, %d) must start and (unless it closes the pool) end on a multiple of %d points",
              p0, p0 + P, ppw);
  UFR_REQUIRE((unsigned long long)P_total * (NV + 1) * UFR_TOKEN_DIM < (1ull << 30),
              "ufr_view_transform_tape: %d points x %d tokens exceed the 2^30 token values one backward addresses", P_total, NV + 1);
  UFR_PRECISION(precision, lowp, "ufr_view_transform_tape");
  hipStream_t s = static_cast<hipStream_t>(stream);
  Carver c(workspace);
  const ViewBwdWs vw = carve_view_bwd(c, P_total, NV);
  StatusSlot* sl = nullptr;
  int rc = status_slot(&sl);
  if (rc == UFR_OK) rc = status_enter(sl, s, "ufr_view_transform_tape");
  if (rc != UFR_OK) return rc;
  const size_t blk_floats = (size_t)(lowp ? ViewTapeLayout<true>::block_units : ViewTapeLayout<false>::block_units) * 128;
  {
    ProfScope p("view_tape", s);
    UFR_HIP(launch_view_tape(static_cast<const float*>(packed_weights), x_tokens, rgb, dir, P, NV, token0, radiance,
                             vw.tape + (size_t)(p0 / ppw) * blk_floats, lowp, sl->dev, s));
  }
  return status_leave(sl, s);
}

int ufr_ray_transform_tape(const void* packed_weights, const float* token0, const int32_t* row, int32_t RN, int32_t SN,
                           float* srdf, void* workspace, int32_t precision, ufr_stream stream) {
  UFR_REQUIRE(packed_weights && token0 && srdf && workspace, "ufr_ray_transform_tape: null argument");
  UFR_REQUIRE(RN > 0 && SN >= 16 && SN % 16 == 0 && SN <= 256, "ufr_ray_transform_tape: SN=%d must be a multiple of 16 in [16,256]", SN);
  UFR_PRECISION(precision, lowp, "ufr_ray_transform_tape");
  hipStream_t s = static_cast<hipStream_t>(stream);
  Carver c(workspace);
  const RayBwdWs rw = carve_ray_bwd(c, RN, SN);
  StatusSlot* sl = nullptr;
  int rc = status_slot(&sl);
  if (rc == UFR_OK) rc = status_enter(sl, s, "ufr_ray_transform_tape");
  if (rc != UFR_OK) return rc;
  UFR_HIP(launch_order_pe(rw.order_pe, SN, s));
  {
    ProfScope p("ray_tape", s);
    UFR_HIP(launch_ray_tape(static_cast<const float*>(packed_weights), token0, row, rw.order_pe, RN, SN, srdf, rw.tape, rw.state, lowp,
                            sl->dev, s));
  }
  return status_leave(sl, s);
}

size_t ufr_ray_transform_workspace_bytes(int32_t SN) { return align_up((size_t)(SN > 0 ? SN : 1) * 8 * sizeof(float)); }

int ufr_ray_transform(const void* packed_weights, const float* token0, const int32_t* row, int32_t RN, int32_t SN,
                      float* srdf, void* workspace, int32_t precision, ufr_stream stream) {
  UFR_REQUIRE(packed_weights && token0 && srdf && workspace, "ufr_ray_transform: null argument");
  UFR_REQUIRE(RN > 0 && SN >= 16 && SN % 16 == 0 && SN <= 256, "ufr_ray_transform: SN=%d must be a multiple of 16 in [16,256]", SN);
  UFR_PRECISION(precision, lowp, "ufr_ray_transform");
  hipStream_t s = static_cast<hipStream_t>(stream);
  StatusSlot* sl = nullptr;
  int rc = status_slot(&sl);
  if (rc == UFR_OK) rc = status_enter(sl, s, "ufr_ray_transform");
  if (rc != UFR_OK) return rc;
  float* order_pe = static_cast<float*>(workspace);
  UFR_HIP(launch_order_pe(order_pe, SN, s));
  {
    ProfScope p("ray_transformer", s);
    UFR_HIP(launch_ray_transformer(static_cast<const float*>(packed_weights), token0, row, order_pe, RN, SN, srdf, nullptr,
                                   lowp, sl->dev, s));
  }
  return status_leave(sl, s);
}

int ufr_ray_transform_bwd(const ufr_raw_weights* raw, const ufr_raw_grads* grads, const void* packed_weights, const float* token0,
                          const int32_t* row, int32_t RN, int32_t SN, const float* d_srdf, float* d_token0_a, float* d_token0_b,
                          int32_t accumulate, void* workspace, int32_t precision, ufr_stream stream) {
  return ufr_ray_transform_bwd_stages(raw, grads, packed_weights, token0, row, RN, SN, d_srdf, d_token0_a, d_token0_b, accumulate,
                                      workspace, UFR_BWD_STAGE_ALL, precision, stream);
}

int ufr_ray_transform_bwd_stages(const ufr_raw_weights* raw, const ufr_raw_grads* grads, const void* packed_weights,
                                 const float* token0, const int32_t* row, int32_t RN, int32_t SN, const float* d_srdf,
                                 float* d_token0_a, float* d_token0_b, int32_t accumulate, void* workspace, int32_t stages,
                                 int32_t precision, ufr_stream stream) {
  RawPtrs rp;
  GradPtrs gp;
  int rc = raw_and_grads(raw, grads, rp, gp, "ufr_ray_transform_bwd");
  if (rc != UFR_OK) return rc;
  UFR_PRECISION(precision, lowp, "ufr_ray_transform_bwd");
  UFR_REQUIRE(stages > 0 && (stages & ~UFR_BWD_STAGE_ALL) == 0, "ufr_ray_transform_bwd_stages: stages=%d", stages);
  UFR_REQUIRE(packed_weights && workspace, "ufr_ray_transform_bwd: null argument");
  UFR_REQUIRE(!(stages & UFR_BWD_STAGE_TAPE) || token0, "ufr_ray_transform_bwd: the tape stage needs token0");
  UFR_REQUIRE(!(stages & UFR_BWD_STAGE_DGRAD) || (d_srdf && d_token0_a), "ufr_ray_transform_bwd: the data-gradient stage needs d_srdf, d_token0_a");
  UFR_REQUIRE(RN > 0 && SN >= 16 && SN % 16 == 0 && SN <= 256, "ufr_ray_transform_bwd: SN=%d must be a multiple of 16 in [16,256]", SN);
  hipStream_t s = static_cast<hipStream_t>(stream);
  Carver c(workspace);
  const RayBwdWs rw = carve_ray_bwd(c, RN, SN);
  StatusSlot* sl = nullptr;
  rc = status_slot(&sl);
  if (rc != UFR_OK) return rc;
  return ray_bwd_impl(packed_weights, gp, token0, row, accumulate != 0, d_srdf, RN, SN, d_token0_a, d_token0_b, rw, lowp, sl->dev, s,
                      stages);
}

int ufr_view_transform_bwd(const ufr_raw_weights* raw, const ufr_raw_grads* grads, const void* packed_weights,
                           const float* x_tokens, const float* rgb, const float* dir, const float* d_token0_a,
                           const float* d_token0_b, const float* d_radiance, int32_t P, int32_t NV, float* d_pv, void* workspace,
                           int32_t precision, ufr_stream stream) {
  return ufr_view_transform_bwd_stages(raw, grads, packed_weights, x_tokens, rgb, dir, d_token0_a, d_token0_b, d_radiance, P, NV, d_pv,
                                       workspace, UFR_BWD_STAGE_ALL, precision, stream);
}

int ufr_view_transform_bwd_stages(const ufr_raw_weights* raw, const ufr_raw_grads* grads, const void* packed_weights,
                                  const float* x_tokens, const float* rgb, const float* dir, const float* d_token0_a,
                                  const float* d_token0_b, const float* d_radiance, int32_t P, int32_t NV, float* d_pv,
                                  void* workspace, int32_t stages, int32_t precision, ufr_stream stream) {
  RawPtrs rp;
  GradPtrs gp;
  int rc = raw_and_grads(raw, grads, rp, gp, "ufr_view_transform_bwd");
  if (rc != UFR_OK) return rc;
  UFR_PRECISION(precision, lowp, "ufr_view_transform_bwd");
  UFR_REQUIRE(stages > 0 && (stages & ~UFR_BWD_STAGE_ALL) == 0, "ufr_view_transform_bwd_stages: stages=%d", stages);
  UFR_REQUIRE(packed_weights && workspace, "ufr_view_transform_bwd: null argument");
  UFR_REQUIRE(!(stages & UFR_BWD_STAGE_TAPE) || (x_tokens && rgb && dir), "ufr_view_transform_bwd: the tape stage needs x_tokens, rgb, dir");
  UFR_REQUIRE(!(stages & UFR_BWD_STAGE_DGRAD) || (rgb && d_token0_a && d_radiance && d_pv),
              "ufr_view_transform_bwd: the data-gradient stage needs rgb, d_token0_a, d_radiance, d_pv");
  UFR_REQUIRE(NV >= 2 && NV <= UFR_MAX_VIEWS && P > 0, "ufr_view_transform_bwd: P=%d NV=%d", P, NV);
  hipStream_t s = static_cast<hipStream_t>(stream);
  Carver c(workspace);
  const ViewBwdWs vw = carve_view_bwd(c, P, NV);
  StatusSlot* sl = nullptr;
  rc = status_slot(&sl);
  if (rc != UFR_OK) return rc;
  return view_bwd_impl(packed_weights, gp, x_tokens, rgb, dir, d_token0_a, d_token0_b, d_radiance, P, NV, d_pv, vw, lowp, sl->dev, s, stages);
}

int32_t ufr_default_chunk_rays(void) { return 4096; }

namespace {
struct RenderWs {
  float *ray_o, *rd, *near, *far, *camz, *z1, *w1, *srdf1, *depth1, *rgb1, *z2, *srdf2, *rad, *x, *xp, *rgbm, *dir, *token0,
      *pe1, *pe2, *z_new;
  int* row;
  size_t bytes;
};
RenderWs carve_render(void* ws, int R, int SN, int PN, int NV) {
  const size_t S2 = (size_t)SN + PN, Smax = S2 > (size_t)SN ? S2 : SN, Sg = (size_t)(SN > PN ? SN : PN);
  Carver c(ws);
  RenderWs r;
  r.ray_o = c.f32(4);
  r.rd = c.f32((size_t)R * 3);
  r.near = c.f32(R);
  r.far = c.f32(R);
  r.camz = c.f32(R);
  r.z1 = c.f32((size_t)R * SN);
  r.w1 = c.f32((size_t)R * SN);
  r.srdf1 = c.f32((size_t)R * SN);
  r.depth1 = c.f32(R);
  r.rgb1 = c.f32((size_t)R * 3);
  r.z2 = c.f32((size_t)R * S2);
  r.srdf2 = c.f32((size_t)R * S2);
  r.rad = c.f32((size_t)R * Smax * 3);
  r.x = c.f32((size_t)R * Sg * NV * kViewCols);
  r.xp = c.f32((size_t)R * Sg * kPointCols);
  r.rgbm = c.f32((size_t)R * Sg * NV * 4);
  r.dir = c.f32((size_t)R * Sg * NV * 4);
  r.z_new = c.f32((size_t)R * (PN > 0 ? PN : 1));
  r.row = reinterpret_cast<int*>(c.f32((size_t)R * S2));
  r.token0 = c.f32((size_t)R * Smax * UFR_TOKEN_DIM);
  r.pe1 = c.f32((size_t)SN * 8);
  r.pe2 = c.f32(S2 * 8);
  r.bytes = c.off;
  return r;
}
}

size_t ufr_render_workspace_bytes(int32_t chunk_rays, int32_t SN, int32_t PN, int32_t NV) {
  if (chunk_rays <= 0) chunk_rays = ufr_default_chunk_rays();
  return carve_render(nullptr, chunk_rays, SN, PN, NV).bytes;
}

namespace {
constexpr int kMaxLanes = 4;
struct SidePool {
  hipStream_t s[kMaxLanes] = {};
  hipEvent_t fork = nullptr, join[kMaxLanes] = {};
  int n = 0;
};
constexpr int kMaxDevices = 16;
thread_local SidePool g_side_by_device[kMaxDevices];

int side_pool_get(int n, SidePool** out) {
  int dev = 0;
  UFR_HIP(hipGetDevice(&dev));
  UFR_REQUIRE(dev >= 0 && dev < kMaxDevices, "side streams: device %d out of range", dev);
  SidePool& p = g_side_by_device[dev];
  if (!p.fork) UFR_HIP(hipEventCreateWithFlags(&p.fork, hipEventDisableTiming));
  for (; p.n < n; ++p.n) {
    int least = 0, greatest = 0;
    UFR_HIP(hipDeviceGetStreamPriorityRange(&least, &greatest));
    UFR_HIP(hipStreamCreateWithPriority(&p.s[p.n], hipStreamNonBlocking, greatest));
    UFR_HIP(hipEventCreateWithFlags(&p.join[p.n], hipEventDisableTiming));
  }
  *out = &p;
  return UFR_OK;
}

int render_chunk(const ufr_render_args* a, const FrameDev* f, const RenderWs& w, bool& pe_ready, int r0, int R, bool lowp,
                 int* status, hipStream_t s) {
  const int RN = a->RN, SN = a->SN, PN = a->coarse_only ? 0 : a->PN, NV = f->NV;
  const PreSim ps = presim_of(a->raw);
  const int S2 = SN + PN, HW = f->H * f->W;
  {
    ProfScope p("sampler", s);
    UFR_HIP(launch_ray_setup(a->ray_idx + r0, a->ray_d, a->cam_ray_d, HW, a->near_z, a->far_z, R, w.rd, w.near, w.far,
                             w.camz, a->ray_o, w.ray_o, s));
    UFR_HIP(launch_sample_fixed(w.near, w.far, a->U1 + r0, RN, w.z1, R, SN, s));
    if (!pe_ready) {
      UFR_HIP(launch_order_pe(w.pe1, SN, s));
      if (!a->coarse_only) UFR_HIP(launch_order_pe(w.pe2, S2, s));
      pe_ready = true;
    }
  }
  {
    ProfScope p("gather", s);
    UFR_HIP(launch_gather(*f, ps, w.ray_o, 0, w.rd, w.z1, R, SN, w.x, w.xp, w.rgbm, w.dir, nullptr, nullptr, nullptr, nullptr, nullptr, nullptr, s));
  }
  int rc = aggregate_impl(a->packed_weights, w.x, w.xp, w.rgbm, w.dir, R, SN, NV, w.rad, w.srdf1, w.token0, w.pe1, true,
                          nullptr, nullptr, lowp, status, s);
  if (rc != UFR_OK) return rc;
  const bool last = a->coarse_only != 0;
  {
    ProfScope p("composite", s);
    UFR_HIP(launch_composite(w.z1, w.rad, nullptr, w.srdf1, a->raw->variance, R, SN, last ? a->rgb + 3 * (size_t)r0 : w.rgb1,
                             last ? a->depth + r0 : w.depth1, nullptr, w.w1, w.camz,
                             (last && a->depth_z) ? a->depth_z + r0 : nullptr, s));
  }
  if (last) {
    if (a->srdf) UFR_HIP(hipMemcpyAsync(a->srdf + (size_t)r0 * SN, w.srdf1, (size_t)R * SN * 4, hipMemcpyDeviceToDevice, s));
    if (a->z_all) UFR_HIP(hipMemcpyAsync(a->z_all + (size_t)r0 * SN, w.z1, (size_t)R * SN * 4, hipMemcpyDeviceToDevice, s));
    return UFR_OK;
  }
  {
    ProfScope p("sampler", s);
    UFR_HIP(launch_importance_merge(w.w1, w.z1, a->U2 + r0, RN, nullptr, w.z2, R, SN, PN, w.z_new, w.row, s));
  }
  {
    ProfScope p("gather", s);
    UFR_HIP(launch_gather(*f, ps, w.ray_o, 0, w.rd, w.z_new, R, PN, w.x, w.xp, w.rgbm, w.dir, nullptr, nullptr, nullptr, nullptr, nullptr, nullptr, s));
  }
  {
    ProfScope p("view_transformer", s);
    UFR_HIP(launch_view_transformer(static_cast<const float*>(a->packed_weights), w.x, w.xp, w.rgbm, w.dir, R * PN, NV,
                                    w.token0 + (size_t)R * SN * UFR_TOKEN_DIM, w.rad + (size_t)R * SN * 3, nullptr, lowp,
                                    status, s));
  }
  {
    ProfScope p("ray_transformer", s);
    UFR_HIP(launch_ray_transformer(static_cast<const float*>(a->packed_weights), w.token0, w.row, w.pe2, R, S2, w.srdf2,
                                   nullptr, lowp, status, s));
  }
  {
    ProfScope p("composite", s);
    UFR_HIP(launch_composite(w.z2, w.rad, w.row, w.srdf2, a->raw->variance, R, S2, a->rgb + 3 * (size_t)r0, a->depth + r0,
                             nullptr, nullptr, w.camz, a->depth_z ? a->depth_z + r0 : nullptr, s));
  }
  if (a->srdf) UFR_HIP(hipMemcpyAsync(a->srdf + (size_t)r0 * S2, w.srdf2, (size_t)R * S2 * 4, hipMemcpyDeviceToDevice, s));
  if (a->z_all) UFR_HIP(hipMemcpyAsync(a->z_all + (size_t)r0 * S2, w.z2, (size_t)R * S2 * 4, hipMemcpyDeviceToDevice, s));
  return UFR_OK;
}
}

int ufr_render_rays(const ufr_render_args* a, ufr_stream stream) {
  UFR_REQUIRE(a, "ufr_render_rays: null args");
  const FrameDev* f = frame_of(a->frame);
  UFR_REQUIRE(f, "ufr_render_rays: frame handle not prepared");
  UFR_REQUIRE(f->match && f->vol[0], "ufr_render_rays: the frame was prepared without matching features / volumes");
  UFR_REQUIRE(a->packed_weights && a->raw && a->ray_idx && a->ray_d && a->U1 && a->depth && a->rgb && a->workspace,
              "ufr_render_rays: null argument");
  UFR_REQUIRE(a->coarse_only || a->U2, "ufr_render_rays: U2 required unless coarse_only");
  const int RN = a->RN, SN = a->SN, PN = a->coarse_only ? 0 : a->PN, NV = f->NV;
  UFR_REQUIRE(RN > 0, "ufr_render_rays: RN=%d", RN);
  UFR_REQUIRE(SN >= 16 && SN % 16 == 0 && SN <= 256, "ufr_render_rays: coarse samples %d must be a multiple of 16 in [16,256]", SN);
  UFR_REQUIRE(a->coarse_only || (PN >= 16 && (SN + PN) % 16 == 0 && SN + PN <= 256 && PN <= 256),
              "ufr_render_rays: fine samples %d unsupported", PN);
  const int chunk = a->chunk_rays > 0 ? a->chunk_rays : ufr_default_chunk_rays();
  UFR_REQUIRE((unsigned long long)chunk * (SN > PN ? SN : PN) * (NV + 1) * UFR_TOKEN_DIM < (1ull << 30),
              "ufr_render_rays: chunk_rays=%d x %d samples x %d tokens exceeds the 2^30 token values one launch addresses; use a "
              "smaller chunk", chunk, SN > PN ? SN : PN, NV + 1);
  const size_t need = ufr_render_workspace_bytes(chunk, SN, PN, NV);
  if (a->workspace_bytes < need) return fail(UFR_ERR_WORKSPACE, "render workspace too small: %zu < %zu", a->workspace_bytes, need);
  UFR_PRECISION(a->precision, lowp, "ufr_render_rays");
  hipStream_t s = static_cast<hipStream_t>(stream);
  StatusSlot* sl = nullptr;
  int src = status_slot(&sl);
  if (src == UFR_OK) src = status_enter(sl, s, "ufr_render_rays");
  if (src != UFR_OK) return src;
  UFR_HIP(launch_refit_weights(static_cast<float*>(const_cast<void*>(a->packed_weights)), f->abs_max, sl->dev, s));
  int lanes = a->n_streams > 1 ? a->n_streams : 1;
  if (lanes > kMaxLanes) lanes = kMaxLanes;
  if ((size_t)lanes * need > a->workspace_bytes) lanes = (int)(a->workspace_bytes / need);
  int eff_chunk = chunk;
  if (lanes > 1) {
    int target = (RN + 4 * lanes - 1) / (4 * lanes) / 2048 * 2048;
    if (target < 2048) target = 2048;
    if (target < eff_chunk) eff_chunk = target;
  }
  const int n_chunks = (RN + eff_chunk - 1) / eff_chunk;
  if (lanes > n_chunks) lanes = n_chunks;

  if (lanes <= 1) {
    RenderWs w = carve_render(a->workspace, chunk, SN, PN, NV);
    bool pe_ready = false;
    for (int r0 = 0; r0 < RN; r0 += eff_chunk) {
      int rc = render_chunk(a, f, w, pe_ready, r0, (RN - r0) < eff_chunk ? (RN - r0) : eff_chunk, lowp, sl->dev, s);
      if (rc != UFR_OK) return rc;
    }
    return status_leave(sl, s);
  }
  SidePool* side = nullptr;
  int rc = side_pool_get(lanes, &side);
  if (rc != UFR_OK) return rc;
  UFR_HIP(hipEventRecord(side->fork, s));
  RenderWs w[kMaxLanes];
  bool pe_ready[kMaxLanes] = {};
  for (int l = 0; l < lanes; ++l) {
    w[l] = carve_render(static_cast<char*>(a->workspace) + (size_t)l * need, chunk, SN, PN, NV);
    UFR_HIP(hipStreamWaitEvent(side->s[l], side->fork, 0));
  }
  for (int c = 0; c < n_chunks && rc == UFR_OK; ++c) {
    const int l = c % lanes, r0 = c * eff_chunk;
    rc = render_chunk(a, f, w[l], pe_ready[l], r0, (RN - r0) < eff_chunk ? (RN - r0) : eff_chunk, lowp, sl->dev, side->s[l]);
  }
  for (int l = 0; l < lanes; ++l) {
    hipError_t e = hipEventRecord(side->join[l], side->s[l]);
    if (e == hipSuccess) e = hipStreamWaitEvent(s, side->join[l], 0);
    if (e != hipSuccess) hipStreamSynchronize(side->s[l]);
  }
  return rc != UFR_OK ? rc : status_leave(sl, s);
}

size_t ufr_correlate_workspace_bytes(int32_t C, int32_t H, int32_t W, int32_t NS) {
  Carver c(nullptr);
  c.f32((size_t)H * W * C);
  c.f32((size_t)NS * H * W * C);
  return c.off;
}

int ufr_frustum_correlate(const float* ref_fea, const float* src_fea, const float* rel_proj, const float* depth_values,
                          const float* view_weights, int32_t C, int32_t H, int32_t W, int32_t D, int32_t NS,
                          float* similarity, float* aggregated, void* workspace, size_t workspace_bytes,
                          ufr_stream stream) {
  UFR_REQUIRE(ref_fea && src_fea && rel_proj && depth_values && workspace, "ufr_frustum_correlate: null argument");
  UFR_REQUIRE(similarity || aggregated, "ufr_frustum_correlate: no output requested");
  UFR_REQUIRE(!aggregated || view_weights, "ufr_frustum_correlate: aggregated output needs view_weights");
  UFR_REQUIRE(C == 4 || C == 8 || C == 16 || C == 32 || C == 64, "ufr_frustum_correlate: C=%d unsupported (4,8,16,32,64)", C);
  UFR_REQUIRE(NS >= 1 && NS <= UFR_MAX_VIEWS, "ufr_frustum_correlate: NS=%d unsupported (1..%d)", NS, UFR_MAX_VIEWS);
  UFR_REQUIRE(H >= 2 && W >= 2 && D >= 1, "ufr_frustum_correlate: H=%d W=%d D=%d", H, W, D);
  const size_t need = ufr_correlate_workspace_bytes(C, H, W, NS);
  if (workspace_bytes < need) return fail(UFR_ERR_WORKSPACE, "correlate workspace too small: %zu < %zu", workspace_bytes, need);
  hipStream_t s = static_cast<hipStream_t>(stream);
  Carver c(workspace);
  float* ref_cl = c.f32((size_t)H * W * C);
  float* src_cl = c.f32((size_t)NS * H * W * C);
  ProfScope p("correlate", s);
  UFR_HIP(launch_chw_to_hwc(ref_fea, ref_cl, 1, C, H * W, s));
  UFR_HIP(launch_chw_to_hwc(src_fea, src_cl, NS, C, H * W, s));
  UFR_HIP(launch_correlate(ref_cl, src_cl, rel_proj, NS, depth_values, view_weights, similarity, aggregated, C, H, W, D, s));
  return UFR_OK;
}

int ufr_conv3d(const float* in, const float* weight, const float* weight2, const float* bias, const float* bn_scale,
               const float* bn_shift, const float* skip, float* out, float* out2, int32_t B, int32_t D, int32_t H,
               int32_t W, int32_t cin, int32_t cout, int32_t cout2, int32_t mode, int32_t relu, int32_t out_ncdhw,
               float* out_absmax, ufr_stream stream) {
  UFR_REQUIRE(in && weight && out, "ufr_conv3d: null argument");
  UFR_REQUIRE(B > 0 && D > 0 && H > 0 && W > 0, "ufr_conv3d: B=%d D=%d H=%d W=%d", B, D, H, W);
  UFR_REQUIRE(mode == UFR_CONV3D_S1 || mode == UFR_CONV3D_S2 || mode == UFR_CONV3D_T2, "ufr_conv3d: unknown mode %d", mode);
  UFR_REQUIRE((bn_scale == nullptr) == (bn_shift == nullptr), "ufr_conv3d: bn_scale and bn_shift go together");
  UFR_REQUIRE(cout2 == 0 || (weight2 && out2 && out_ncdhw && mode == UFR_CONV3D_S1),
              "ufr_conv3d: a second head needs weight2, out2, out_ncdhw and stride 1");
  UFR_REQUIRE(out_ncdhw || (cout % 4 == 0 && cout2 == 0), "ufr_conv3d: channel-last outputs need cout %% 4 == 0 (got %d)", cout);
  UFR_REQUIRE(!skip || !out_ncdhw, "ufr_conv3d: skip is a channel-last tensor; not with out_ncdhw");
  UFR_REQUIRE((long long)B * D * H * W * (cin > cout ? cin : cout) < (1ll << 40), "ufr_conv3d: volume too large");
  hipStream_t s = static_cast<hipStream_t>(stream);
  ProfScope p("conv3d", s);
  UFR_REQUIRE(!out_absmax || (!out_ncdhw && cout <= 16), "ufr_conv3d: out_absmax goes with channel-last outputs of at most 16 channels");
  const hipError_t e = launch_conv3d(in, weight, weight2, bias, bn_scale, bn_shift, skip, out, out2, B, D, H, W, cin, cout,
                                     cout2, mode, relu, out_ncdhw, s, 0, out_absmax);
  if (e == hipErrorInvalidValue)
    return fail(UFR_ERR_ARG, "ufr_conv3d: (cin %d, cout %d+%d, mode %d) is not a layer of CostRegNet / CostRegNetWeight", cin,
                cout, cout2, mode);
  UFR_HIP(e);
  return UFR_OK;
}

size_t ufr_conv3d_planes_workspace_bytes(int32_t cin, int32_t cout, int32_t cout2, int32_t mode) {
  return conv3d_planes_workspace_bytes(cin, cout, cout2, mode);
}

int ufr_conv3d_planes(const float* in, const float* in_absmax, const float* weight, const float* weight2, const float* bias,
                      const float* bn_scale, const float* bn_shift, const float* skip, float* out, float* out2,
                      float* out_absmax, int32_t B, int32_t D, int32_t H, int32_t W, int32_t cin, int32_t cout, int32_t cout2,
                      int32_t mode, int32_t relu, int32_t out_ncdhw, int32_t flip, void* workspace, size_t workspace_bytes, int32_t planes_ready,
                      ufr_stream stream) {
  UFR_REQUIRE(in && in_absmax && weight && out && workspace, "ufr_conv3d_planes: null argument");
  UFR_REQUIRE(B > 0 && D > 0 && H > 0 && W > 0, "ufr_conv3d_planes: B=%d D=%d H=%d W=%d", B, D, H, W);
  UFR_REQUIRE((bn_scale == nullptr) == (bn_shift == nullptr), "ufr_conv3d_planes: bn_scale and bn_shift go together");
  UFR_REQUIRE(cout2 == 0 || (weight2 && out2 && out_ncdhw && !flip), "ufr_conv3d_planes: a second head needs weight2, out2, out_ncdhw");
  UFR_REQUIRE(out_ncdhw || (cout % 4 == 0 && cout2 == 0), "ufr_conv3d_planes: channel-last outputs need cout %% 4 == 0 (got %d)", cout);
  UFR_REQUIRE(!(out_ncdhw && (skip || out_absmax)), "ufr_conv3d_planes: skip / out_absmax go with channel-last outputs");
  UFR_REQUIRE(mode == UFR_CONV3D_S1 || mode == UFR_CONV3D_S2 || mode == UFR_CONV3D_T2, "ufr_conv3d_planes: unknown mode %d", mode);
  UFR_REQUIRE(!(mode != UFR_CONV3D_S1 && flip), "ufr_conv3d_planes: flip is the stride-1 data gradient");
  UFR_REQUIRE(!(mode == UFR_CONV3D_T2 && out_ncdhw), "ufr_conv3d_planes: the transposed layers write channel-last");
  const size_t need = conv3d_planes_workspace_bytes(cin, cout, cout2, mode);
  if (!need) return fail(UFR_ERR_ARG, "ufr_conv3d_planes: (cin %d, cout %d+%d, mode %d) is not a layer of this kernel family", cin, cout, cout2, mode);
  if (workspace_bytes < need) return fail(UFR_ERR_WORKSPACE, "ufr_conv3d_planes: workspace %zu < %zu", workspace_bytes, need);
  UFR_REQUIRE((long long)D * H * W * cin * 4 < (1ll << 31), "ufr_conv3d_planes: one batch element reaches 2 GiB");
  hipStream_t s = static_cast<hipStream_t>(stream);
  ProfScope p(flip ? "conv3d_dgrad" : "conv3d", s);
  UFR_HIP(launch_conv3d_planes(in, in_absmax, weight, weight2, bias, bn_scale, bn_shift, skip, out, out2, out_absmax, B, D, H, W, cin,
                               cout, cout2, mode, relu, out_ncdhw, flip, workspace, planes_ready != 0, s));
  return UFR_OK;
}

int ufr_absmax(const float* x, size_t n, float* absmax, ufr_stream stream) {
  UFR_REQUIRE(x && absmax, "ufr_absmax: null argument");
  UFR_HIP(launch_absmax(x, n, absmax, static_cast<hipStream_t>(stream)));
  return UFR_OK;
}

int ufr_conv3d_bwd_data(const float* d_out, const float* weight, const float* accumulate, float* d_in, int32_t B, int32_t D,
                        int32_t H, int32_t W, int32_t cin, int32_t cout, int32_t mode, ufr_stream stream) {
  UFR_REQUIRE(d_out && weight && d_in, "ufr_conv3d_bwd_data: null argument");
  UFR_REQUIRE(B > 0 && D > 0 && H > 0 && W > 0, "ufr_conv3d_bwd_data: B=%d D=%d H=%d W=%d", B, D, H, W);
  UFR_REQUIRE(mode == UFR_CONV3D_S1 || mode == UFR_CONV3D_S2 || mode == UFR_CONV3D_T2, "ufr_conv3d_bwd_data: unknown mode %d", mode);
  UFR_REQUIRE(mode != UFR_CONV3D_S2 || (D % 2 == 0 && H % 2 == 0 && W % 2 == 0), "ufr_conv3d_bwd_data: stride 2 needs even extents");
  UFR_REQUIRE(cin == 1 || cin % 4 == 0, "ufr_conv3d_bwd_data: cin=%d", cin);
  UFR_REQUIRE(!(cin == 1 && accumulate), "ufr_conv3d_bwd_data: no fused addition into a 1-channel gradient");
  hipStream_t s = static_cast<hipStream_t>(stream);
  ProfScope p("conv3d_dgrad", s);
  const hipError_t e = launch_conv3d_bwd_data(d_out, weight, accumulate, d_in, B, D, H, W, cin, cout, mode, s);
  if (e == hipErrorInvalidValue)
    return fail(UFR_ERR_ARG, "ufr_conv3d_bwd_data: (cin %d, cout %d, mode %d) is not a layer of CostRegNetWeight", cin, cout, mode);
  UFR_HIP(e);
  return UFR_OK;
}

int ufr_conv3d_bwd_weight(const float* in, const float* d_out, float* d_weight, float* d_bias, int32_t B, int32_t D, int32_t H,
                          int32_t W, int32_t cin, int32_t cout, int32_t mode, ufr_stream stream) {
  UFR_REQUIRE(in && d_out && d_weight, "ufr_conv3d_bwd_weight: null argument");
  UFR_REQUIRE(B > 0 && D > 0 && H > 0 && W > 0, "ufr_conv3d_bwd_weight: B=%d D=%d H=%d W=%d", B, D, H, W);
  UFR_REQUIRE(mode == UFR_CONV3D_S1 || mode == UFR_CONV3D_S2 || mode == UFR_CONV3D_T2, "ufr_conv3d_bwd_weight: unknown mode %d", mode);
  UFR_REQUIRE(mode != UFR_CONV3D_S2 || (D % 2 == 0 && H % 2 == 0 && W % 2 == 0), "ufr_conv3d_bwd_weight: stride 2 needs even extents");
  hipStream_t s = static_cast<hipStream_t>(stream);
  ProfScope p("conv3d_wgrad", s);
  const hipError_t e = launch_conv3d_bwd_weight(in, d_out, d_weight, d_bias, B, D, H, W, cin, cout, mode, s);
  if (e == hipErrorInvalidValue)
    return fail(UFR_ERR_ARG, "ufr_conv3d_bwd_weight: (cin %d, cout %d, mode %d) is not a layer of CostRegNetWeight", cin, cout, mode);
  UFR_HIP(e);
  return UFR_OK;
}

int ufr_conv3d_bwd_weight_heads(const float* in, const float* d_out, const float* d_out2, float* d_weight, float* d_weight2, int32_t B,
                                int32_t D, int32_t H, int32_t W, ufr_stream stream) {
  UFR_REQUIRE(in && d_out && d_out2 && d_weight && d_weight2, "ufr_conv3d_bwd_weight_heads: null argument");
  UFR_REQUIRE(B > 0 && D > 0 && H > 0 && W > 0, "ufr_conv3d_bwd_weight_heads: B=%d D=%d H=%d W=%d", B, D, H, W);
  UFR_REQUIRE((long long)D * H * W * 32 < (1ll << 31), "ufr_conv3d_bwd_weight_heads: one batch element reaches 2 GiB");
  hipStream_t s = static_cast<hipStream_t>(stream);
  ProfScope p("conv3d_wgrad", s);
  UFR_HIP(launch_conv3d_wgrad_heads(in, d_out, d_out2, d_weight, d_weight2, B, D, H, W, s));
  return UFR_OK;
}

int ufr_tsdf_integrate(float* tsdf, float* weight, float* color, const int32_t* dim, const float* origin,
                       float voxel_size, float trunc_margin, const float* cam_intr, const float* cam_pose,
                       const float* depth_im, const float* color_im, int32_t im_h, int32_t im_w, float obs_weight,
                       int32_t integrate_color, ufr_stream stream) {
  UFR_REQUIRE(tsdf && weight && dim && origin && cam_intr && cam_pose && depth_im, "ufr_tsdf_integrate: null argument");
  UFR_REQUIRE(dim[0] > 0 && dim[1] > 0 && dim[2] > 0, "ufr_tsdf_integrate: volume %dx%dx%d", dim[0], dim[1], dim[2]);
  UFR_REQUIRE(im_h > 0 && im_w > 0, "ufr_tsdf_integrate: image %dx%d", im_h, im_w);
  UFR_REQUIRE(voxel_size > 0.f && trunc_margin > 0.f, "ufr_tsdf_integrate: voxel_size %g, trunc_margin %g", voxel_size, trunc_margin);
  UFR_REQUIRE(!integrate_color || (color && color_im), "ufr_tsdf_integrate: colour integration needs color and color_im");
  hipStream_t s = static_cast<hipStream_t>(stream);
  ProfScope p("tsdf_integrate", s);
  UFR_HIP(launch_tsdf_integrate(tsdf, weight, color, dim, origin, voxel_size, trunc_margin, cam_intr, cam_pose, depth_im,
                                color_im, im_h, im_w, obs_weight, integrate_color, s));
  return UFR_OK;
}

namespace {
struct McWorkspace {
  int* tile_counts;
  long long *tile_off, *totals;
  int* index;
  size_t bytes;
  McWorkspace(void* base, const int32_t* dim) {
    const size_t tiles = (size_t)mcubes_tiles(dim), n = (size_t)dim[0] * dim[1] * dim[2];
    char* b = static_cast<char*>(base);
    size_t off = 0;
    tile_counts = reinterpret_cast<int*>(b + off);
    off += align_up(tiles * 2 * sizeof(int));
    tile_off = reinterpret_cast<long long*>(b + off);
    off += align_up(tiles * 2 * sizeof(long long));
    totals = reinterpret_cast<long long*>(b + off);
    off += align_up(2 * sizeof(long long));
    index = reinterpret_cast<int*>(b + off);
    off += align_up(n * sizeof(int));
    bytes = off;
  }
};

int mc_check(const char* who, const float* vol, const int32_t* dim, void* ws, size_t ws_bytes) {
  UFR_REQUIRE(vol && dim && ws, "%s: null argument", who);
  UFR_REQUIRE(dim[0] >= 2 && dim[1] >= 2 && dim[2] >= 2, "%s: volume %dx%dx%d (every dim must be >= 2)", who, dim[0], dim[1], dim[2]);
  UFR_REQUIRE((long long)dim[0] * dim[1] * dim[2] < (1ll << 31), "%s: volume %dx%dx%d has 2^31 voxels or more", who, dim[0], dim[1],
              dim[2]);
  const size_t need = McWorkspace(nullptr, dim).bytes;
  if (ws_bytes < need) return fail(UFR_ERR_WORKSPACE, "%s: workspace %zu bytes, needs %zu", who, ws_bytes, need);
  return UFR_OK;
}
}

size_t ufr_marching_cubes_workspace_bytes(const int32_t* dim) {
  if (!dim || dim[0] < 2 || dim[1] < 2 || dim[2] < 2 || (long long)dim[0] * dim[1] * dim[2] >= (1ll << 31)) return 0;
  return McWorkspace(nullptr, dim).bytes;
}

int ufr_marching_cubes_count(const float* vol, const int32_t* dim, float level, void* workspace, size_t workspace_bytes,
                             int32_t* counts_host, ufr_stream stream) {
  if (int rc = mc_check("ufr_marching_cubes_count", vol, dim, workspace, workspace_bytes)) return rc;
  UFR_REQUIRE(counts_host, "ufr_marching_cubes_count: null argument (counts_host)");
  hipStream_t s = static_cast<hipStream_t>(stream);
  McWorkspace w(workspace, dim);
  {
    ProfScope p("mcubes_count", s);
    UFR_HIP(launch_mcubes_count(vol, dim, level, w.tile_counts, s));
  }
  {
    ProfScope p("mcubes_scan", s);
    UFR_HIP(launch_mcubes_scan(w.tile_counts, mcubes_tiles(dim), w.tile_off, w.totals, s));
  }
  long long tot[2] = {0, 0};
  UFR_HIP(hipMemcpyAsync(tot, w.totals, sizeof(tot), hipMemcpyDeviceToHost, s));
  UFR_HIP(hipStreamSynchronize(s));
  UFR_REQUIRE(tot[0] < (1ll << 31) && tot[1] < (1ll << 31), "ufr_marching_cubes_count: %lld vertices, %lld faces: 2^31 or more",
              tot[0], tot[1]);
  counts_host[0] = (int32_t)tot[0];
  counts_host[1] = (int32_t)tot[1];
  return UFR_OK;
}

int ufr_marching_cubes_emit(const float* vol, const int32_t* dim, float level, void* workspace, size_t workspace_bytes,
                            float* verts, float* normals, int32_t* faces, int32_t n_verts, int32_t n_faces, ufr_stream stream) {
  if (int rc = mc_check("ufr_marching_cubes_emit", vol, dim, workspace, workspace_bytes)) return rc;
  UFR_REQUIRE(n_verts >= 0 && n_faces >= 0, "ufr_marching_cubes_emit: n_verts %d, n_faces %d", n_verts, n_faces);
  UFR_REQUIRE((n_verts == 0 || (verts && normals)) && (n_faces == 0 || faces), "ufr_marching_cubes_emit: null argument");
  hipStream_t s = static_cast<hipStream_t>(stream);
  McWorkspace w(workspace, dim);
  if (n_verts == 0 && n_faces == 0) return UFR_OK;
  {
    ProfScope p("mcubes_verts", s);
    UFR_HIP(launch_mcubes_verts(vol, dim, level, w.tile_off, w.index, verts, normals, n_verts, s));
  }
  if (n_faces > 0) {
    ProfScope p("mcubes_faces", s);
    UFR_HIP(launch_mcubes_faces(vol, dim, level, w.tile_off, w.index, faces, n_faces, s));
  }
  return UFR_OK;
}

int ufr_marching_cubes_table(int8_t* out, int32_t out_len) {
  static_assert(sizeof(kMcTable[0]) == UFR_MC_TABLE_ROW, "mcubes_table.h and ufr.h disagree on the row length");
  UFR_REQUIRE(out, "ufr_marching_cubes_table: null argument");
  UFR_REQUIRE(out_len >= 256 * UFR_MC_TABLE_ROW, "ufr_marching_cubes_table: out_len %d < %d", out_len, 256 * UFR_MC_TABLE_ROW);
  memcpy(out, kMcTable, sizeof(kMcTable));
  return UFR_MC_TABLE_ROW;
}

namespace {
constexpr long long kChMax = (1ll << 31) - 1;

struct SampleWorkspace {
  long long *tri_off, *block_tot, *block_off, *total;
  size_t bytes;
  SampleWorkspace(void* base, long long F) {
    const size_t blocks = (size_t)chamfer_blocks(F);
    char* b = static_cast<char*>(base);
    size_t off = 0;
    tri_off = reinterpret_cast<long long*>(b + off);
    off += align_up((size_t)F * sizeof(long long));
    block_tot = reinterpret_cast<long long*>(b + off);
    off += align_up(blocks * sizeof(long long));
    block_off = reinterpret_cast<long long*>(b + off);
    off += align_up(blocks * sizeof(long long));
    total = reinterpret_cast<long long*>(b + off);
    off += align_up(sizeof(long long));
    bytes = off;
  }
};

int sample_check(const char* who, const double* verts, const int32_t* faces, int64_t V, int64_t F, double density, void* ws,
                 size_t ws_bytes) {
  UFR_REQUIRE(verts && faces && ws, "%s: null argument", who);
  UFR_REQUIRE(V >= 1 && V <= kChMax && F >= 1 && F <= kChMax, "%s: V %lld, F %lld (each must be 1 .. 2^31 - 1)", who, (long long)V,
              (long long)F);
  UFR_REQUIRE(density > 0.0 && std::isfinite(density), "%s: density %g (must be positive and finite)", who, density);
  const size_t need = SampleWorkspace(nullptr, F).bytes;
  if (ws_bytes < need) return fail(UFR_ERR_WORKSPACE, "%s: workspace %zu bytes, needs %zu", who, ws_bytes, need);
  return UFR_OK;
}

struct NnWorkspace {
  double* block_sum;
  long long* block_cnt;
  size_t bytes;
  NnWorkspace(void* base, long long nq) {
    const size_t blocks = (size_t)chamfer_blocks(nq);
    char* b = static_cast<char*>(base);
    block_sum = reinterpret_cast<double*>(b);
    size_t off = align_up(blocks * sizeof(double));
    block_cnt = reinterpret_cast<long long*>(b + off);
    off += align_up(blocks * sizeof(long long));
    bytes = off;
  }
};
}

size_t ufr_mesh_sample_workspace_bytes(int64_t F) { return (F >= 1 && F <= kChMax) ? SampleWorkspace(nullptr, F).bytes : 0; }

int ufr_mesh_sample_count(const double* verts, const int32_t* faces, int64_t V, int64_t F, double density, void* workspace,
                          size_t workspace_bytes, int64_t* total_host, ufr_stream stream) {
  if (int rc = sample_check("ufr_mesh_sample_count", verts, faces, V, F, density, workspace, workspace_bytes)) return rc;
  UFR_REQUIRE(total_host, "ufr_mesh_sample_count: null argument (total_host)");
  hipStream_t s = static_cast<hipStream_t>(stream);
  SampleWorkspace w(workspace, F);
  {
    ProfScope p("mesh_sample_count", s);
    UFR_HIP(launch_mesh_sample_count(verts, faces, V, F, density, w.tri_off, w.block_tot, s));
  }
  {
    ProfScope p("mesh_sample_scan", s);
    UFR_HIP(launch_mesh_sample_scan(w.block_tot, chamfer_blocks(F), w.block_off, w.total, s));
  }
  long long tot = 0;
  UFR_HIP(hipMemcpyAsync(&tot, w.total, sizeof(tot), hipMemcpyDeviceToHost, s));
  UFR_HIP(hipStreamSynchronize(s));
  *total_host = (int64_t)tot;
  return UFR_OK;
}

int ufr_mesh_sample_emit(const double* verts, const int32_t* faces, int64_t V, int64_t F, double density, void* workspace,
                         size_t workspace_bytes, double* out, int64_t capacity, ufr_stream stream) {
  if (int rc = sample_check("ufr_mesh_sample_emit", verts, faces, V, F, density, workspace, workspace_bytes)) return rc;
  UFR_REQUIRE(capacity >= 0, "ufr_mesh_sample_emit: capacity %lld", (long long)capacity);
  UFR_REQUIRE(capacity == 0 || out, "ufr_mesh_sample_emit: null argument (out)");
  if (capacity == 0) return UFR_OK;
  hipStream_t s = static_cast<hipStream_t>(stream);
  SampleWorkspace w(workspace, F);
  ProfScope p("mesh_sample_emit", s);
  UFR_HIP(launch_mesh_sample_emit(verts, faces, V, F, density, w.tri_off, w.block_off, out, capacity, s));
  return UFR_OK;
}

int ufr_points_cell_keys(const double* points, int64_t n, const double* origin, double cell, int64_t* keys, ufr_stream stream) {
  UFR_REQUIRE(points && origin && keys, "ufr_points_cell_keys: null argument");
  UFR_REQUIRE(n >= 1 && n <= kChMax, "ufr_points_cell_keys: n %lld (must be 1 .. 2^31 - 1)", (long long)n);
  UFR_REQUIRE(cell > 0.0 && std::isfinite(cell) && std::isfinite(origin[0]) && std::isfinite(origin[1]) && std::isfinite(origin[2]),
              "ufr_points_cell_keys: cell %g, origin (%g, %g, %g) (cell must be positive, all finite)", cell, origin[0], origin[1],
              origin[2]);
  hipStream_t s = static_cast<hipStream_t>(stream);
  ProfScope p("points_cell_keys", s);
  UFR_HIP(launch_points_cell_keys(points, n, origin, cell, reinterpret_cast<long long*>(keys), s));
  return UFR_OK;
}

size_t ufr_points_thin_workspace_bytes(int64_t n) { return (n >= 1 && n <= kChMax) ? align_up(sizeof(int)) : 0; }

int ufr_points_thin(const double* points, const int64_t* keys, const int32_t* rank, int64_t n, double radius, uint8_t* state,
                    void* workspace, size_t workspace_bytes, int32_t* rounds_host, ufr_stream stream) {
  UFR_REQUIRE(points && keys && rank && state && workspace, "ufr_points_thin: null argument");
  UFR_REQUIRE(n >= 1 && n <= kChMax, "ufr_points_thin: n %lld (must be 1 .. 2^31 - 1)", (long long)n);
  UFR_REQUIRE(radius >= 0.0 && std::isfinite(radius), "ufr_points_thin: radius %g (must be finite and >= 0)", radius);
  const size_t need = ufr_points_thin_workspace_bytes(n);
  if (workspace_bytes < need) return fail(UFR_ERR_WORKSPACE, "ufr_points_thin: workspace %zu bytes, needs %zu", workspace_bytes, need);
  hipStream_t s = static_cast<hipStream_t>(stream);
  int* undecided = static_cast<int*>(workspace);
  UFR_HIP(hipMemsetAsync(state, 0, (size_t)n, s));
  long long prev = n;
  int rounds = 0;
  while (prev > 0) {
    if (rounds >= n) return fail(UFR_ERR_HIP, "ufr_points_thin: no fixpoint after %d rounds", rounds);
    int und = 0;
    UFR_HIP(hipMemsetAsync(undecided, 0, sizeof(int), s));
    {
      ProfScope p("points_thin_round", s);
      UFR_HIP(launch_thin_round(points, reinterpret_cast<const long long*>(keys), rank, n, radius, state, undecided, s));
    }
    UFR_HIP(hipMemcpyAsync(&und, undecided, sizeof(int), hipMemcpyDeviceToHost, s));
    UFR_HIP(hipStreamSynchronize(s));
    ++rounds;
    if (und < 0 || und >= prev)
      return fail(UFR_ERR_HIP, "ufr_points_thin: round %d left %d of %lld points undecided (rank is not a permutation?)", rounds, und,
                  prev);
    prev = und;
  }
  if (rounds_host) *rounds_host = rounds;
  return UFR_OK;
}

size_t ufr_points_nn_dist_workspace_bytes(int64_t nq) { return (nq >= 1 && nq <= kChMax) ? NnWorkspace(nullptr, nq).bytes : 0; }

int ufr_points_nn_dist(const double* query, int64_t nq, const double* ref, const int64_t* ref_keys, int64_t nr,
                       const double* origin, double cell, double max_dist, double* dist, double* mean_out, void* workspace,
                       size_t workspace_bytes, ufr_stream stream) {
  UFR_REQUIRE(query && ref && ref_keys && origin && dist && workspace, "ufr_points_nn_dist: null argument");
  UFR_REQUIRE(nq >= 1 && nq <= kChMax && nr >= 1 && nr <= kChMax, "ufr_points_nn_dist: nq %lld, nr %lld (each must be 1 .. 2^31 - 1)",
              (long long)nq, (long long)nr);
  UFR_REQUIRE(cell > 0.0 && std::isfinite(cell) && std::isfinite(origin[0]) && std::isfinite(origin[1]) && std::isfinite(origin[2]),
              "ufr_points_nn_dist: cell %g, origin (%g, %g, %g) (cell must be positive, all finite)", cell, origin[0], origin[1],
              origin[2]);
  UFR_REQUIRE(max_dist > 0.0 && max_dist < 1e150, "ufr_points_nn_dist: max_dist %g (must be positive, below 1e150)", max_dist);
  const size_t need = NnWorkspace(nullptr, nq).bytes;
  if (workspace_bytes < need) return fail(UFR_ERR_WORKSPACE, "ufr_points_nn_dist: workspace %zu bytes, needs %zu", workspace_bytes, need);
  hipStream_t s = static_cast<hipStream_t>(stream);
  NnWorkspace w(workspace, nq);
  ProfScope p("points_nn_dist", s);
  UFR_HIP(launch_nn_dist(query, nq, ref, reinterpret_cast<const long long*>(ref_keys), nr, origin, cell, max_dist, dist, w.block_sum,
                         w.block_cnt, mean_out, s));
  return UFR_OK;
}

int ufr_pixelwise_view_weights(const float* similarity, const float* params, float* view_weights, float* aggregated, int32_t NS,
                               int32_t D, int32_t H, int32_t W, ufr_stream stream) {
  UFR_REQUIRE(similarity && params && view_weights, "ufr_pixelwise_view_weights: null argument");
  UFR_REQUIRE(NS >= 1 && NS <= UFR_MAX_VIEWS && D >= 1 && H >= 1 && W >= 1, "ufr_pixelwise_view_weights: NS=%d D=%d H=%d W=%d", NS, D, H, W);
  hipStream_t s = static_cast<hipStream_t>(stream);
  ProfScope p("pixelwise_view_weights", s);
  UFR_HIP(launch_pixelwise_weights(similarity, params, view_weights, aggregated, NS, D, H, W, s));
  return UFR_OK;
}

size_t ufr_deform_conv2d_workspace_bytes(int32_t B, int32_t C, int32_t H, int32_t W) {
  Carver c(nullptr);
  c.f32((size_t)B * H * W * C);
  return c.off;
}

int ufr_deform_conv2d(const float* input, const float* offset, const float* mask, const float* weight,
                      const float* bias, float* output, int32_t B, int32_t C, int32_t Cout, int32_t H, int32_t W,
                      void* workspace, size_t workspace_bytes, ufr_stream stream) {
  UFR_REQUIRE(input && offset && weight && output && workspace, "ufr_deform_conv2d: null argument");
  UFR_REQUIRE(C > 0 && C % 4 == 0 && C <= 32, "ufr_deform_conv2d: C=%d unsupported (multiple of 4, <= 32)", C);
  UFR_REQUIRE(Cout == 8 || Cout == 16 || Cout == 32, "ufr_deform_conv2d: Cout=%d unsupported (8, 16, 32)", Cout);
  UFR_REQUIRE(B > 0 && H > 0 && W > 0, "ufr_deform_conv2d: B=%d H=%d W=%d", B, H, W);
  const size_t need = ufr_deform_conv2d_workspace_bytes(B, C, H, W);
  if (workspace_bytes < need) return fail(UFR_ERR_WORKSPACE, "deform_conv2d workspace too small: %zu < %zu", workspace_bytes, need);
  hipStream_t s = static_cast<hipStream_t>(stream);
  Carver c(workspace);
  float* in_cl = c.f32((size_t)B * H * W * C);
  ProfScope p("deform_conv2d", s);
  UFR_HIP(launch_chw_to_hwc(input, in_cl, B, C, H * W, s));
  UFR_HIP(launch_deform_conv3x3(in_cl, offset, mask, weight, bias, output, B, C, Cout, H, W, s));
  return UFR_OK;
}

int ufr_conv2d(const float* input, const float* weight, const float* scale, const float* shift, const float* skip, float* output,
               int32_t B, int32_t cin, int32_t cout, int32_t H, int32_t W, int32_t ksize, int32_t stride, int32_t flags,
               int32_t sigmoid_from, ufr_stream stream) {
  UFR_REQUIRE(input && weight && output, "ufr_conv2d: null argument");
  UFR_REQUIRE(B > 0 && H > 0 && W > 0 && cout > 0 && cout <= 32, "ufr_conv2d: B=%d H=%d W=%d cout=%d", B, H, W, cout);
  UFR_REQUIRE((ksize == 1 || ksize == 3 || ksize == 5) && (stride == 1 || stride == 2), "ufr_conv2d: ksize=%d stride=%d", ksize, stride);
  UFR_REQUIRE((unsigned long long)H * W * (cin > 3 ? cin : 4) * 4ull < (1ull << 31), "ufr_conv2d: %d x %d x %d exceeds 2^31 bytes per image", H, W, cin);
  Conv2dArgs a;
  a.in = input; a.w = weight; a.scale = scale; a.shift = shift; a.skip = skip; a.out = output;
  a.B = B; a.H = H; a.W = W; a.cout = cout;
  a.Ho = (H + 2 * (ksize / 2) - ksize) / stride + 1;
  a.Wo = (W + 2 * (ksize / 2) - ksize) / stride + 1;
  a.relu = (flags & UFR_CONV2D_RELU) != 0;
  a.out_planar = (flags & UFR_CONV2D_OUT_PLANAR) != 0;
  a.sigmoid_from = sigmoid_from;
  UFR_REQUIRE(!skip || (a.Ho % 2 == 0 && a.Wo % 2 == 0 && cout % 4 == 0), "ufr_conv2d: the upsampled skip needs even output extents and cout %% 4 == 0");
  hipStream_t s = static_cast<hipStream_t>(stream);
  ProfScope p("conv2d", s);
  const hipError_t e = launch_conv2d(a, cin, ksize, stride, (flags & UFR_CONV2D_IN_PLANAR) != 0, s);
  if (e == hipErrorInvalidValue)
    return fail(UFR_ERR_ARG, "ufr_conv2d: %d -> %d channels, %dx%d, stride %d is not a layer shape of FeatureNet (conv2d.hip)", cin, cout, ksize, ksize, stride);
  UFR_HIP(e);
  return UFR_OK;
}

int ufr_upsample_add(const float* reduced_cl, const float* fine, float* output_cl, int32_t B, int32_t C, int32_t h, int32_t w,
                     ufr_stream stream) {
  UFR_REQUIRE(reduced_cl && fine && output_cl, "ufr_upsample_add: null argument");
  UFR_REQUIRE((C == 8 || C == 16) && B > 0 && h > 0 && w > 0, "ufr_upsample_add: B=%d C=%d h=%d w=%d (C in {8, 16})", B, C, h, w);
  hipStream_t s = static_cast<hipStream_t>(stream);
  ProfScope p("upsample_add", s);
  UFR_HIP(launch_upsample_add(reduced_cl, fine, output_cl, B, C, h, w, s));
  return UFR_OK;
}

int ufr_deform_conv2d_cl(const float* input_cl, const float* offset_mask, const float* weight, const float* bias,
                         const float* scale, const float* shift, float* output, int32_t B, int32_t C, int32_t Cout, int32_t H,
                         int32_t W, int32_t flags, ufr_stream stream) {
  const float* offset = offset_mask;
  UFR_REQUIRE(input_cl && offset && weight && output, "ufr_deform_conv2d_cl: null argument");
  const float* mask = offset_mask + (size_t)18 * H * W;
  UFR_REQUIRE(C == 32, "ufr_deform_conv2d_cl: C=%d (the channel-last form exists for the 32-channel layers of FeatureNet)", C);
  UFR_REQUIRE(Cout == 8 || Cout == 16 || Cout == 32, "ufr_deform_conv2d_cl: Cout=%d unsupported (8, 16, 32)", Cout);
  UFR_REQUIRE(B > 0 && H > 0 && W > 0, "ufr_deform_conv2d_cl: B=%d H=%d W=%d", B, H, W);
  UFR_REQUIRE((scale == nullptr) == (shift == nullptr), "ufr_deform_conv2d_cl: scale and shift come together");
  hipStream_t s = static_cast<hipStream_t>(stream);
  ProfScope p("deform_conv2d", s);
  UFR_HIP(launch_deform_conv3x3(input_cl, offset, mask, weight, bias, output, B, C, Cout, H, W, s,
                                DcnEpilogue{scale, shift, (flags & UFR_CONV2D_RELU) != 0, (flags & UFR_CONV2D_OUT_PLANAR) == 0, 27}));
  return UFR_OK;
}

size_t ufr_fmt_layer_workspace_bytes(int32_t N, int32_t S) {
  return align_up((size_t)(N > 0 ? N : 1) * 160 * sizeof(float) * (1 + (size_t)fmt_state_parts(S > 0 ? S : 1)));
}

int ufr_fmt_layer(const ufr_fmt_layer_weights* w, const float* x, const float* src, int32_t N, int32_t T, int32_t S,
                  float* out, void* workspace, ufr_stream stream) {
  static_assert(sizeof(ufr_fmt_layer_weights) == sizeof(FmtWeights), "ufr_fmt_layer_weights layout");
  UFR_REQUIRE(w && x && out && workspace, "ufr_fmt_layer: null argument");
  FmtWeights fw;
  memcpy(&fw, w, sizeof(fw));
  const float* const* pw = reinterpret_cast<const float* const*>(&fw);
  for (int i = 0; i < 16; ++i) UFR_REQUIRE(pw[i], "ufr_fmt_layer: weight pointer %d is null", i);
  if (!src) { src = x; S = T; }
  UFR_REQUIRE(N > 0 && T > 0 && S > 0, "ufr_fmt_layer: N=%d T=%d S=%d", N, T, S);
  UFR_REQUIRE(out != x && out != src, "ufr_fmt_layer: out must not alias an input");
  hipStream_t s = static_cast<hipStream_t>(stream);
  ProfScope p("fmt_layer", s);
  UFR_HIP(launch_fmt_layer(fw, x, src, N, T, S, out, static_cast<float*>(workspace), s));
  return UFR_OK;
}

void ufr_profile_enable(int on) {
  std::lock_guard<std::mutex> lock(g_prof_mu);
  for (auto& e : g_prof) { hipEventDestroy(e.a); hipEventDestroy(e.b); }
  g_prof.clear();
  g_prof_on.store(on != 0, std::memory_order_relaxed);
}

int ufr_profile_read(const char** names, float* ms, int32_t* launches, int cap) {
  std::lock_guard<std::mutex> lock(g_prof_mu);
  int n = 0;
  for (auto& e : g_prof) {
    float t = 0.f;
    if (hipEventSynchronize(e.b) != hipSuccess || hipEventElapsedTime(&t, e.a, e.b) != hipSuccess) continue;
    int k = 0;
    for (; k < n; ++k)
      if (strcmp(names[k], e.name) == 0) break;
    if (k == n) {
      if (n >= cap) continue;
      names[n] = e.name; ms[n] = 0.f; launches[n] = 0; ++n;
    }
    ms[k] += t;
    launches[k] += 1;
  }
  for (auto& e : g_prof) { hipEventDestroy(e.a); hipEventDestroy(e.b); }
  g_prof.clear();
  return n;
}

}
```

uforecon_amd/csrc/ufr_internal.h:

```cpp
#pragma once
#include <hip/hip_runtime.h>
#include <stdint.h>

#include <mutex>

#include "../../include/ufr.h"
#include "ufr_layout.h"

namespace ufr {

constexpr int kVolCh = 12;

struct FrameDev {
  int32_t NV, H, W, h, w, match_ch;
  const float* feat;
  const float* match;
  const float* rgb;
  const float* depth;
  const float* vol[UFR_NUM_STAGES];
  int32_t vD[UFR_NUM_STAGES], vH[UFR_NUM_STAGES], vW[UFR_NUM_STAGES];
  float pose[UFR_MAX_VIEWS][12];
  float cam_pos[UFR_MAX_VIEWS][3];
  float w2c_z[UFR_MAX_VIEWS][4];
  float ref_pos[3];
  float vol_near, vol_far;
  uint32_t magic;
  const unsigned* abs_max;
};
static_assert(sizeof(FrameDev) <= sizeof(ufr_frame), "ufr_frame too small");
constexpr uint32_t kFrameMagic = 0x55465246u;

struct PreSim {
  const float *w0, *b0, *w2, *b2, *w4, *b4;
};

struct LdsAttrOnce {
  std::once_flag flag[16];
  hipError_t err[16];
  hipError_t set(const void* kernel, int bytes) {
    int dev = 0;
    if (hipGetDevice(&dev) != hipSuccess || dev < 0 || dev >= 16) return hipErrorInvalidDevice;
    std::call_once(flag[dev], [&] { err[dev] = hipFuncSetAttribute(kernel, hipFuncAttributeMaxDynamicSharedMemorySize, bytes); });
    return err[dev];
  }
};

hipError_t launch_nchw_to_nhwc(const float* in, float* out, int N, int C, int S, int Cpad, hipStream_t s, unsigned* abs_max = nullptr);
hipError_t launch_volume_pack(const float* feat, const float* weight, float* out, int N, int S, hipStream_t s, unsigned* abs_max = nullptr);
hipError_t launch_ray_setup(const int64_t* ray_idx, const float* ray_d, const float* cam_ray_d, int HW, float near_z,
                            float far_z, int RN, float* rd_out, float* near_out, float* far_out, float* camz_out,
                            const float* ray_o_host, float* ray_o_out, hipStream_t s);
hipError_t launch_sample_fixed(const float* near, const float* far, const float* U, int u_stride, float* z, int RN,
                               int SN, hipStream_t s);
hipError_t launch_importance_merge(const float* weight, const float* z, const float* U2, int u_stride, float* z_fine,
                                   float* z_all, int RN, int SN, int PN, float* z_new, int* src_row, hipStream_t s);
hipError_t launch_order_pe(float* table, int SN, hipStream_t s);
hipError_t launch_points(const float* ray_o, int o_stride, const float* ray_d, const float* z, float* pts, int RN,
                         int SN, hipStream_t s);
constexpr int kViewCols = 40, kPointCols = 40;
hipError_t launch_gather(const FrameDev& f, const PreSim& ps, const float* ray_o, int o_stride, const float* ray_d,
                         const float* z, int RN, int SN, float* x_tokens, float* x_point, float* rgb, float* dir, float* sim8,
                         float* vol24, float* xy, float* mask_z, const float* vol24_in, const float* sim8_in,
                         hipStream_t s);
hipError_t launch_view_transformer(const float* packed, const float* x_tokens, const float* x_point, const float* rgb,
                                   const float* dir, int P, int NV, float* token0, float* radiance, float* view_out, bool lowp, int* status,
                                   hipStream_t s);
hipError_t launch_ray_transformer(const float* packed, const float* token0, const int* tok_row, const float* order_pe,
                                  int RN, int SN, float* srdf, float* ray_out, bool lowp, int* status, hipStream_t s);
hipError_t launch_composite(const float* z, const float* radiance, const int* rad_row, const float* srdf,
                            const float* variance, int RN, int SN, float* rgb, float* depth, float* opacity, float* weight,
                            const float* camz, float* depth_z, hipStream_t s);
hipError_t launch_render_loss(const float* rgb_c, const float* depth_c, const float* rgb_f, const float* depth_f,
                              const float* rgb_gt, const float* depth_gt, const float* near_far, int nf_stride, int B, int RN,
                              float weight_rgb, float weight_depth, float* loss, float* d_rgb_c, float* d_depth_c,
                              float* d_rgb_f, float* d_depth_f, hipStream_t s);
hipError_t launch_composite_bwd(const float* z, const float* radiance, const int* rad_row, bool accumulate, const float* srdf,
                                const float* variance, int RN, int SN, const float* d_rgb, const float* d_depth,
                                const float* d_opacity, const float* d_weight, float* d_radiance, float* d_srdf,
                                float* d_variance, hipStream_t s);
struct GradPtrs;
int view_tape_blocks(int P, int NV);
hipError_t launch_view_tape(const float* packed, const float* x_tokens, const float* rgb, const float* dir, int P, int NV,
                            float* token0, float* radiance, float* tape, bool lowp, int* status, hipStream_t s);
hipError_t launch_view_dgrad(const float* packed, const float* tape, const float* rgbm, const float* d_tok_a,
                             const float* d_tok_b, const float* d_radiance, int P, int NV, float* dbuf, float* d_pv,
                             const GradPtrs& gp, bool lowp, hipStream_t s);
hipError_t launch_view_wgrad(const float* tape, const float* dbuf, int n_blocks, const GradPtrs& gp, bool lowp, hipStream_t s);
hipError_t launch_ray_tape(const float* packed, const float* token0, const int* tok_row, const float* order_pe, int RN, int SN,
                           float* srdf, float* tape, float* ray_state, bool lowp, int* status, hipStream_t s);
hipError_t launch_ray_dgrad(const float* packed, const float* tape, const float* ray_state, const float* d_srdf, const int* tok_row,
                            bool accumulate, int RN, int SN, float* dbuf, float* d_tok_a, float* d_tok_b, const GradPtrs& gp, bool lowp,
                            hipStream_t s);
hipError_t launch_ray_wgrad(const float* tape, const float* dbuf, int n_blocks, const GradPtrs& gp, bool lowp, hipStream_t s);
hipError_t launch_presim_bwd(const RawPtrs& wp, const GradPtrs& gp, const float* sim8, const float* d_pv, int P, bool lowp,
                             hipStream_t s);
size_t gather_bwd_scratch_floats(const FrameDev& f);
hipError_t launch_gather_bwd(const FrameDev& f, float* const* grad_feat, float* const* grad_weight, const float* ray_o,
                             int o_stride, const float* ray_d, const float* z, const float* d_pv, const int* pv_row, int RN,
                             int SN, float* scratch, bool accumulate, bool scratch_zeroed, hipStream_t s);
struct FmtWeights {
  const float *wq, *bq, *wk, *bk, *wv, *bv, *wo, *bo, *w1, *b1, *w2, *b2, *n1w, *n1b, *n2w, *n2b;
};
int fmt_state_parts(int S);
hipError_t launch_fmt_layer(const FmtWeights& w, const float* x, const float* src, int N, int T, int S, float* out,
                            float* state, hipStream_t s);
hipError_t launch_pack_weights(const RawPtrs& raw, float* packed, float input_abs_max, int* range_flag, hipStream_t s);
hipError_t launch_refit_weights(float* packed, const unsigned* frame_bound, int* range_flag, hipStream_t s);
hipError_t launch_tsdf_integrate(float* tsdf, float* weight, float* color, const int* dim, const float* origin,
                                 float voxel_size, float trunc_margin, const float* K, const float* P,
                                 const float* depth_im, const float* color_im, int im_h, int im_w, float obs_weight,
                                 int integrate_color, hipStream_t s);
int mcubes_tiles(const int* dim);
hipError_t launch_mcubes_count(const float* vol, const int* dim, float level, int* tile_counts, hipStream_t s);
hipError_t launch_mcubes_scan(const int* tile_counts, int n_tiles, long long* tile_off, long long* totals, hipStream_t s);
hipError_t launch_mcubes_verts(const float* vol, const int* dim, float level, const long long* tile_off, int* index,
                               float* verts, float* normals, long long n_verts, hipStream_t s);
hipError_t launch_mcubes_faces(const float* vol, const int* dim, float level, const long long* tile_off, const int* index,
                               int* faces, long long n_faces, hipStream_t s);
long long chamfer_blocks(long long n);
hipError_t launch_points_cell_keys(const double* pts, long long n, const double* origin, double cell, long long* keys,
                                   hipStream_t s);
hipError_t launch_mesh_sample_count(const double* verts, const int* faces, long long V, long long F, double density,
                                    long long* tri_off, long long* block_tot, hipStream_t s);
hipError_t launch_mesh_sample_scan(const long long* block_tot, long long n_blocks, long long* block_off, long long* total,
                                   hipStream_t s);
hipError_t launch_mesh_sample_emit(const double* verts, const int* faces, long long V, long long F, double density,
                                   const long long* tri_off, const long long* block_off, double* out, long long capacity,
                                   hipStream_t s);
hipError_t launch_thin_round(const double* pts, const long long* keys, const int* rank, long long n, double radius,
                             unsigned char* state, int* undecided, hipStream_t s);
hipError_t launch_nn_dist(const double* query, long long nq, const double* ref, const long long* keys, long long nr,
                          const double* origin, double cell, double max_dist, double* dist, double* block_sum,
                          long long* block_cnt, double* mean_out, hipStream_t s);
struct Conv2dArgs {
  const float* in;
  const float* w;
  const float* scale;
  const float* shift;
  const float* skip;
  float* out;
  int B, H, W, Ho, Wo, cout;
  int relu, out_planar, sigmoid_from;
};
hipError_t launch_conv2d(const Conv2dArgs& a, int cin, int ks, int stride, int in_planar, hipStream_t s);
hipError_t launch_upsample_add(const float* reduced, const float* fine, float* out, int B, int C, int h, int w, hipStream_t s);
struct DcnEpilogue {
  const float* scale;
  const float* shift;
  int relu, out_cl;
  int om_planes;
};
hipError_t launch_deform_conv3x3(const float* in_cl, const float* offset, const float* mask, const float* weight,
                                 const float* bias, float* out, int B, int C, int Cout, int H, int W, hipStream_t s,
                                 DcnEpilogue ep = DcnEpilogue{nullptr, nullptr, 0, 0, 0});
size_t conv3d_planes_workspace_bytes(int cin, int cout, int cout2, int mode);
hipError_t launch_conv3d_wgrad_heads(const float* in, const float* d_out, const float* d_out2, float* dw, float* dw2, int B, int D, int H,
                                     int W, hipStream_t s);
hipError_t launch_conv3d_wgrad_planes(const float* tp, const float* tq, float* dw, float* dbias, int B, int Dp, int Hp, int Wp, int Dq,
                                      int Hq, int Wq, int ca, int cb, int S, hipStream_t s);
hipError_t launch_absmax(const float* x, size_t n, float* absmax, hipStream_t s);
hipError_t launch_conv3d_planes(const float* in, const float* in_absmax, const float* weight, const float* weight2, const float* bias,
                                const float* scale, const float* shift, const float* skip, float* out, float* out2, float* out_absmax,
                                int B, int D, int H, int W, int cin, int cout, int cout2, int mode, int relu, int ncdhw, int flip,
                                void* ws, int planes_ready, hipStream_t s);
hipError_t launch_conv3d(const float* in, const float* weight, const float* weight2, const float* bias, const float* scale,
                         const float* shift, const float* skip, float* out, float* out2, int B, int D, int H, int W,
                         int cin, int cout, int cout2, int mode, int relu, int ncdhw, hipStream_t s, int flip = 0,
                         float* out_absmax = nullptr);
hipError_t launch_conv3d_bwd_data(const float* d_out, const float* weight, const float* accumulate, float* d_in, int B, int D,
                                  int H, int W, int cin, int cout, int mode, hipStream_t s);
hipError_t launch_conv3d_bwd_weight(const float* in, const float* d_out, float* d_weight, float* d_bias, int B, int D, int H, int W,
                                    int cin, int cout, int mode, hipStream_t s);
hipError_t launch_chw_to_hwc(const float* in, float* out, int N, int C, int S, hipStream_t s);
hipError_t launch_pixelwise_weights(const float* sim, const float* params, float* vw, float* agg, int NS, int D, int H, int W,
                                    hipStream_t s);
hipError_t launch_correlate(const float* ref_cl, const float* src_cl, const float* proj_host, int NS, const float* depth,
                            const float* vw, float* sim, float* agg, int C, int H, int W, int D, hipStream_t s);

}
```

Baseline: 2.680 million rays/s.

## Fuse composite and importance merge into ray transformer epilogue; merge ray setup and sampling

Moves per-ray compositing, and for the coarse pass also importance resampling, into an epilogue of the ray transformer kernel. Each wave composites its own ray right after writing srdf, which removes two or three separate kernel launches per chunk and the re-reads of srdf and weights. Ray setup and fixed sampling are merged into one kernel, so the near/far buffers are no longer needed. The cost is extra LDS for the merge region and more register pressure in the transformer kernel, which could lower its occupancy.

```diff
diff --git a/uforecon_amd/csrc/composite.hip b/uforecon_amd/csrc/composite.hip
--- a/uforecon_amd/csrc/composite.hip
+++ b/uforecon_amd/csrc/composite.hip
@@ -1,18 +1,9 @@
+#include "composite_device.h"
 #include "ufr_internal.h"
 
 #pragma clang fp contract(off)
 
 namespace ufr {
-
-constexpr int kMaxK = 4;
-
-__device__ __forceinline__ float sigmoidf(float x) { return 1.f / (1.f + expf(-x)); }
-
-__device__ __forceinline__ float wave_sum(float v) {
-#pragma unroll
-  for (int d = 32; d >= 1; d >>= 1) v += __shfl_xor(v, d);
-  return v;
-}
 
 __global__ void __launch_bounds__(256) composite_kernel(const float* __restrict__ z, const float* __restrict__ radiance,
                                                          const int* __restrict__ rad_row, const float* __restrict__ srdf,
@@ -23,75 +14,7 @@
   const int wave = threadIdx.x >> 6, lane = threadIdx.x & 63;
   const int ray = blockIdx.x * 4 + wave;
   if (ray >= RN) return;
-  const float* zr = z + (size_t)ray * SN;
-  const float* sr = srdf + (size_t)ray * SN;
-  const float inv_s = fminf(fmaxf(expf(variance[0] * 10.0f), 1e-6f), 1e6f);
-  const int K = (SN + 63) / 64;
-
-  float alpha[kMaxK], zz[kMaxK];
-  float prod = 1.f;
-#pragma unroll
-  for (int k = 0; k < kMaxK; ++k) {
-    alpha[k] = 0.f;
-    zz[k] = 0.f;
-    int i = lane * K + k;
-    if (k < K && i < SN) {
-      float zc = zr[i];
-      float gl = (i == 0) ? zr[1] - zr[0] : zc - zr[i - 1];
-      float gr = (i == SN - 1) ? zr[SN - 1] - zr[SN - 2] : zr[i + 1] - zc;
-      float interval = (gl + gr) / 2.f;
-      float s = sr[i];
-      const float iter_cos = -1.5f;
-      float nxt = s + iter_cos * interval * 0.5f;
-      float prv = s - iter_cos * interval * 0.5f;
-      float pc = sigmoidf(prv * inv_s), nc = sigmoidf(nxt * inv_s);
-      float a = ((pc - nc) + 1e-5f) / (pc + 1e-5f);
-      a = fminf(fmaxf(a, 0.f), 1.f);
-      alpha[k] = a;
-      zz[k] = zc;
-      prod *= (1.f - a) + 1e-7f;
-    }
-  }
-  float incl = prod;
-#pragma unroll
-  for (int d = 1; d < 64; d <<= 1) {
-    float o = __shfl_up(incl, d);
-    if (lane >= d) incl *= o;
-  }
-  float T = __shfl_up(incl, 1);
-  if (lane == 0) T = 1.f;
-
-  float acc_d = 0.f, acc_o = 0.f, acc_r = 0.f, acc_g = 0.f, acc_b = 0.f;
-#pragma unroll
-  for (int k = 0; k < kMaxK; ++k) {
-    int i = lane * K + k;
-    if (k < K && i < SN) {
-      float w = alpha[k] * T;
-      T *= (1.f - alpha[k]) + 1e-7f;
-      if (weight) weight[(size_t)ray * SN + i] = w;
-      const float* c = radiance + (rad_row ? (size_t)rad_row[(size_t)ray * SN + i] : (size_t)ray * SN + i) * 3;
-      acc_r += c[0] * w;
-      acc_g += c[1] * w;
-      acc_b += c[2] * w;
-      acc_d += w * zz[k];
-      acc_o += w;
-    }
-  }
-  acc_d = wave_sum(acc_d);
-  acc_o = wave_sum(acc_o);
-  acc_r = wave_sum(acc_r);
-  acc_g = wave_sum(acc_g);
-  acc_b = wave_sum(acc_b);
-  if (lane == 0) {
-    depth[ray] = acc_d;
-    if (opacity) opacity[ray] = acc_o;
-    if (rgb) {
-      rgb[3 * ray + 0] = acc_r;
-      rgb[3 * ray + 1] = acc_g;
-      rgb[3 * ray + 2] = acc_b;
-    }
-    if (depth_z) depth_z[ray] = acc_d * camz[ray];
-  }
+  composite_ray(ray, lane, z, radiance, rad_row, srdf, variance, SN, rgb, depth, opacity, weight, camz, depth_z);
 }
 
 __global__ void __launch_bounds__(256) composite_bwd_kernel(const float* __restrict__ z, const float* __restrict__ radiance,
diff --git a/uforecon_amd/csrc/composite_device.h b/uforecon_amd/csrc/composite_device.h
--- /dev/null
+++ b/uforecon_amd/csrc/composite_device.h
@@ -0,0 +1,97 @@
+#pragma once
+#include <hip/hip_runtime.h>
+
+namespace ufr {
+
+constexpr int kMaxK = 4;
+
+__device__ __forceinline__ float sigmoidf(float x) {
+#pragma clang fp contract(off)
+  return 1.f / (1.f + expf(-x));
+}
+
+__device__ __forceinline__ float wave_sum(float v) {
+#pragma unroll
+  for (int d = 32; d >= 1; d >>= 1) v += __shfl_xor(v, d);
+  return v;
+}
+
+__device__ __forceinline__ void composite_ray(int ray, int lane, const float* __restrict__ z, const float* __restrict__ radiance,
+                                              const int* __restrict__ rad_row, const float* __restrict__ srdf,
+                                              const float* __restrict__ variance, int SN, float* __restrict__ rgb,
+                                              float* __restrict__ depth, float* __restrict__ opacity,
+                                              float* __restrict__ weight, const float* __restrict__ camz,
+                                              float* __restrict__ depth_z) {
+#pragma clang fp contract(off)
+  const float* zr = z + (size_t)ray * SN;
+  const float* sr = srdf + (size_t)ray * SN;
+  const float inv_s = fminf(fmaxf(expf(variance[0] * 10.0f), 1e-6f), 1e6f);
+  const int K = (SN + 63) / 64;
+
+  float alpha[kMaxK], zz[kMaxK];
+  float prod = 1.f;
+#pragma unroll
+  for (int k = 0; k < kMaxK; ++k) {
+    alpha[k] = 0.f;
+    zz[k] = 0.f;
+    int i = lane * K + k;
+    if (k < K && i < SN) {
+      float zc = zr[i];
+      float gl = (i == 0) ? zr[1] - zr[0] : zc - zr[i - 1];
+      float gr = (i == SN - 1) ? zr[SN - 1] - zr[SN - 2] : zr[i + 1] - zc;
+      float interval = (gl + gr) / 2.f;
+      float s = sr[i];
+      const float iter_cos = -1.5f;
+      float nxt = s + iter_cos * interval * 0.5f;
+      float prv = s - iter_cos * interval * 0.5f;
+      float pc = sigmoidf(prv * inv_s), nc = sigmoidf(nxt * inv_s);
+      float a = ((pc - nc) + 1e-5f) / (pc + 1e-5f);
+      a = fminf(fmaxf(a, 0.f), 1.f);
+      alpha[k] = a;
+      zz[k] = zc;
+      prod *= (1.f - a) + 1e-7f;
+    }
+  }
+  float incl = prod;
+#pragma unroll
+  for (int d = 1; d < 64; d <<= 1) {
+    float o = __shfl_up(incl, d);
+    if (lane >= d) incl *= o;
+  }
+  float T = __shfl_up(incl, 1);
+  if (lane == 0) T = 1.f;
+
+  float acc_d = 0.f, acc_o = 0.f, acc_r = 0.f, acc_g = 0.f, acc_b = 0.f;
+#pragma unroll
+  for (int k = 0; k < kMaxK; ++k) {
+    int i = lane * K + k;
+    if (k < K && i < SN) {
+      float w = alpha[k] * T;
+      T *= (1.f - alpha[k]) + 1e-7f;
+      if (weight) weight[(size_t)ray * SN + i] = w;
+      const float* c = radiance + (rad_row ? (size_t)rad_row[(size_t)ray * SN + i] : (size_t)ray * SN + i) * 3;
+      acc_r += c[0] * w;
+      acc_g += c[1] * w;
+      acc_b += c[2] * w;
+      acc_d += w * zz[k];
+      acc_o += w;
+    }
+  }
+  acc_d = wave_sum(acc_d);
+  acc_o = wave_sum(acc_o);
+  acc_r = wave_sum(acc_r);
+  acc_g = wave_sum(acc_g);
+  acc_b = wave_sum(acc_b);
+  if (lane == 0) {
+    depth[ray] = acc_d;
+    if (opacity) opacity[ray] = acc_o;
+    if (rgb) {
+      rgb[3 * ray + 0] = acc_r;
+      rgb[3 * ray + 1] = acc_g;
+      rgb[3 * ray + 2] = acc_b;
+    }
+    if (depth_z) depth_z[ray] = acc_d * camz[ray];
+  }
+}
+
+}
diff --git a/uforecon_amd/csrc/ray_transformer.hip b/uforecon_amd/csrc/ray_transformer.hip
--- a/uforecon_amd/csrc/ray_transformer.hip
+++ b/uforecon_amd/csrc/ray_transformer.hip
@@ -1,4 +1,6 @@
 #include "bwd_tape.h"
+#include "composite_device.h"
+#include "sampler_device.h"
 #include "ufr_internal.h"
 #include "weight_stream_f16.h"
 
@@ -52,6 +54,8 @@
 constexpr int kRtBlock = 256;
 constexpr int kRtMinW = 2;
 constexpr int kRtWaves = kRtBlock / 64;
+constexpr int kRayMergeLdsBytes = kRtWaves * 3 * kMaxS * 4;
+static_assert(kF16LdsBytes % 16 == 0, "the merge region follows the vector region");
 
 #ifdef UFR_PHASE_TIMING
 __device__ unsigned long long g_rt_phase[32];
@@ -72,8 +76,8 @@
                                                                   const float* __restrict__ order_pe, int RN, int SN,
                                                                   float* __restrict__ srdf,
                                                                   float* __restrict__ ray_out,
-                                                                  int* __restrict__ status, float* __restrict__ tape = nullptr,
-                                                                  float* __restrict__ ray_state = nullptr) {
+                                                                  int* __restrict__ status, float* __restrict__ tape,
+                                                                  float* __restrict__ ray_state, const RayEpilogue ep) {
   extern __shared__ __attribute__((aligned(16))) char smem[];
   auto ws = wstream_f16_begin<kRtWaves, LOWP>(packed, smem);
   wstream_f16_prime<B_RT1, kRtWaves>(ws);
@@ -363,6 +367,20 @@
     UFR_RT_PHASE(9)
   }
   wstream_report_range(ws, status);
+  if constexpr (!TAPE) {
+    if (ep.z && valid) {
+      wave_sync_memory();
+      composite_ray(ray, lane, ep.z, ep.radiance, ep.rad_row, srdf, ep.variance, SN, ep.rgb, ep.depth, nullptr, ep.weight, ep.camz,
+                    ep.depth_z);
+      if (ep.U2) {
+        wave_sync_memory();
+        float* const lds = reinterpret_cast<float*>(smem + kF16LdsBytes) + ws.wave * (3 * kMaxS);
+        importance_merge_ray(lds, ray, lane, ep.weight, ep.z, ep.U2, ep.u_stride, nullptr, ep.z_all, RN, SN, ep.PN, ep.z_new,
+                             ep.src_row);
+      }
+    }
+  }
+  UFR_RT_PHASE(10)
 #ifdef UFR_PHASE_TIMING
   if (ray_raw == 5 && lane == 0)
     for (int i = 0; i < 16; ++i) g_rt_phase[i] += rt_acc[i];
@@ -372,11 +390,17 @@
 template <bool LOWP, bool TAPE = false>
 static hipError_t launch_rt(const float* packed, const float* token0, const int* tok_row, const float* order_pe, int RN,
                             int SN, float* srdf, float* ray_out, int* status, hipStream_t s, float* tape = nullptr,
-                            float* ray_state = nullptr) {
+                            float* ray_state = nullptr, const RayEpilogue* epilogue = nullptr) {
+  const RayEpilogue ep = (epilogue && !TAPE) ? *epilogue : RayEpilogue{};
+  if (ep.z) {
+    if (SN > 64 * kMaxK) return hipErrorInvalidValue;
+    if (ep.U2 && (SN > kMaxS || ep.PN > kMaxS || ep.PN < 1)) return hipErrorInvalidValue;
+  }
+  const int lds_max = kF16LdsBytes + (TAPE ? 0 : kRayMergeLdsBytes), lds_bytes = kF16LdsBytes + (ep.U2 ? kRayMergeLdsBytes : 0);
   static LdsAttrOnce lds_attr;
-  if (const hipError_t attr = lds_attr.set(reinterpret_cast<const void*>(&ray_transformer_kernel<LOWP, TAPE>), kF16LdsBytes); attr != hipSuccess) return attr;
-  hipLaunchKernelGGL((ray_transformer_kernel<LOWP, TAPE>), dim3((RN + kRtWaves - 1) / kRtWaves), dim3(kRtBlock), kF16LdsBytes, s,
-                     packed, token0, tok_row, order_pe, RN, SN, srdf, ray_out, status, tape, ray_state);
+  if (const hipError_t attr = lds_attr.set(reinterpret_cast<const void*>(&ray_transformer_kernel<LOWP, TAPE>), lds_max); attr != hipSuccess) return attr;
+  hipLaunchKernelGGL((ray_transformer_kernel<LOWP, TAPE>), dim3((RN + kRtWaves - 1) / kRtWaves), dim3(kRtBlock), lds_bytes, s,
+                     packed, token0, tok_row, order_pe, RN, SN, srdf, ray_out, status, tape, ray_state, ep);
   return hipGetLastError();
 }
 
@@ -388,10 +412,11 @@
 }
 
 hipError_t launch_ray_transformer(const float* packed, const float* token0, const int* tok_row, const float* order_pe,
-                                  int RN, int SN, float* srdf, float* ray_out, bool lowp, int* status, hipStream_t s) {
+                                  int RN, int SN, float* srdf, float* ray_out, bool lowp, int* status, hipStream_t s,
+                                  const RayEpilogue* epilogue) {
   if (SN % 16 != 0 || SN < 16) return hipErrorInvalidValue;
-  return lowp ? launch_rt<true>(packed, token0, tok_row, order_pe, RN, SN, srdf, ray_out, status, s)
-              : launch_rt<false>(packed, token0, tok_row, order_pe, RN, SN, srdf, ray_out, status, s);
+  return lowp ? launch_rt<true>(packed, token0, tok_row, order_pe, RN, SN, srdf, ray_out, status, s, nullptr, nullptr, epilogue)
+              : launch_rt<false>(packed, token0, tok_row, order_pe, RN, SN, srdf, ray_out, status, s, nullptr, nullptr, epilogue);
 }
 
 }
diff --git a/uforecon_amd/csrc/sampler.hip b/uforecon_amd/csrc/sampler.hip
--- a/uforecon_amd/csrc/sampler.hip
+++ b/uforecon_amd/csrc/sampler.hip
@@ -1,3 +1,4 @@
+#include "sampler_device.h"
 #include "ufr_internal.h"
 
 #pragma clang fp contract(off)
@@ -14,16 +15,14 @@
   int i = blockIdx.x * blockDim.x + threadIdx.x;
   if (i == 0 && ray_o_out) { ray_o_out[0] = ox; ray_o_out[1] = oy; ray_o_out[2] = oz; }
   if (i >= RN) return;
-  int64_t p = ray_idx[i];
-  const bool in_range = p >= 0 && p < (int64_t)HW;
-  p = in_range ? p : 0;
+  int64_t p;
+  float cz, n, f;
+  ray_near_far(ray_idx, cam_ray_d, HW, near_z, far_z, i, p, cz, n, f);
   rd_out[3 * i + 0] = ray_d[p];
   rd_out[3 * i + 1] = ray_d[(size_t)HW + p];
   rd_out[3 * i + 2] = ray_d[2 * (size_t)HW + p];
-  float cz = cam_ray_d ? cam_ray_d[2 * (size_t)HW + p] : 1.f;
-  const float bad = __builtin_nanf("");
-  near_out[i] = !in_range ? bad : cam_ray_d ? near_z / cz : near_z;
-  far_out[i] = !in_range ? bad : cam_ray_d ? far_z / cz : far_z;
+  near_out[i] = n;
+  far_out[i] = f;
   if (camz_out) camz_out[i] = cz;
 }
 
@@ -43,13 +42,7 @@
   size_t i = (size_t)blockIdx.x * blockDim.x + threadIdx.x;
   if (i >= (size_t)RN * SN) return;
   int s = (int)(i / RN), ray = (int)(i % RN);
-  double step = 1.0 / (double)(SN - 1);
-  float lin = (s == SN - 1) ? 1.0f : (float)((double)s * step);
-  float n = near[ray], f = far[ray];
-  float zz = lin * (f - n) + n;
-  float interval = (float)(1.0 / (double)(SN - 1));
-  zz = zz + (U[(size_t)s * u_stride + ray] - 0.5f) * interval * (f - n);
-  z[(size_t)ray * SN + s] = zz;
+  z[(size_t)ray * SN + s] = fixed_sample_z(near[ray], far[ray], U[(size_t)s * u_stride + ray], s, SN);
 }
 
 hipError_t launch_sample_fixed(const float* near, const float* far, const float* U, int u_stride, float* z, int RN,
@@ -57,6 +50,38 @@
   size_t n = (size_t)RN * SN;
   hipLaunchKernelGGL(sample_fixed_kernel, dim3((unsigned)((n + 255) / 256)), dim3(256), 0, s, near, far, U, u_stride, z,
                      RN, SN);
+  return hipGetLastError();
+}
+
+__global__ void __launch_bounds__(256) ray_begin_kernel(const int64_t* __restrict__ ray_idx, const float* __restrict__ ray_d,
+                                                         const float* __restrict__ cam_ray_d, int HW, float near_z,
+                                                         float far_z, const float* __restrict__ U, int u_stride, int RN,
+                                                         int SN, float* __restrict__ rd_out, float* __restrict__ camz_out,
+                                                         float* __restrict__ z, float ox, float oy, float oz,
+                                                         float* __restrict__ ray_o_out) {
+  size_t i = (size_t)blockIdx.x * blockDim.x + threadIdx.x;
+  if (i == 0 && ray_o_out) { ray_o_out[0] = ox; ray_o_out[1] = oy; ray_o_out[2] = oz; }
+  if (i >= (size_t)RN * SN) return;
+  int s = (int)(i / RN), ray = (int)(i % RN);
+  int64_t p;
+  float cz, n, f;
+  ray_near_far(ray_idx, cam_ray_d, HW, near_z, far_z, ray, p, cz, n, f);
+  if (s == 0) {
+    rd_out[3 * ray + 0] = ray_d[p];
+    rd_out[3 * ray + 1] = ray_d[(size_t)HW + p];
+    rd_out[3 * ray + 2] = ray_d[2 * (size_t)HW + p];
+    if (camz_out) camz_out[ray] = cz;
+  }
+  z[(size_t)ray * SN + s] = fixed_sample_z(n, f, U[(size_t)s * u_stride + ray], s, SN);
+}
+
+hipError_t launch_ray_begin(const int64_t* ray_idx, const float* ray_d, const float* cam_ray_d, int HW, float near_z,
+                            float far_z, const float* U, int u_stride, int RN, int SN, float* rd_out, float* camz_out,
+                            float* z, const float* ray_o_host, float* ray_o_out, hipStream_t s) {
+  size_t n = (size_t)RN * SN;
+  hipLaunchKernelGGL(ray_begin_kernel, dim3((unsigned)((n + 255) / 256)), dim3(256), 0, s, ray_idx, ray_d, cam_ray_d, HW,
+                     near_z, far_z, U, u_stride, RN, SN, rd_out, camz_out, z, ray_o_host ? ray_o_host[0] : 0.f,
+                     ray_o_host ? ray_o_host[1] : 0.f, ray_o_host ? ray_o_host[2] : 0.f, ray_o_out);
   return hipGetLastError();
 }
 
@@ -81,17 +106,6 @@
   return hipGetLastError();
 }
 
-constexpr int kMaxS = 256;
-
-__device__ __forceinline__ double wave_incl_scan(double v, int lane) {
-#pragma unroll
-  for (int d = 1; d < 64; d <<= 1) {
-    double o = __shfl_up(v, d);
-    if (lane >= d) v += o;
-  }
-  return v;
-}
-
 __global__ void __launch_bounds__(256) importance_merge_kernel(const float* __restrict__ weight,
                                                                 const float* __restrict__ z,
                                                                 const float* __restrict__ U2, int u_stride,
@@ -101,123 +115,8 @@
   __shared__ float lds[4][3 * kMaxS];
   const int wave = threadIdx.x >> 6, lane = threadIdx.x & 63;
   const int ray = blockIdx.x * 4 + wave;
-  const bool active = ray < RN;
-  float* cdf = lds[wave];
-  float* all = cdf + kMaxS;
-  float* zf = all + SN;
-  const float* w = weight + (size_t)(active ? ray : 0) * SN;
-
-  const int K = (SN + 63) / 64;
-  double run = 0.0;
-  for (int k = 0; k < K; ++k) {
-    int i = lane * K + k;
-    if (i < SN) run += (double)w[i];
-  }
-  double incl = wave_incl_scan(run, lane);
-  float total;
-  {
-    float a4[4] = {0.f, 0.f, 0.f, 0.f};
-    const int l8 = lane & 7;
-    for (int c = 0; c * 32 < SN; ++c)
-#pragma unroll
-      for (int k = 0; k < 4; ++k) {
-        int i = (c * 4 + k) * 8 + l8;
-        if (i < SN) a4[k] += w[i];
-      }
-    const float t = ((a4[0] + a4[1]) + a4[2]) + a4[3];
-    total = __shfl(t, 0);
-#pragma unroll
-    for (int l = 1; l < 8; ++l) total += __shfl(t, l);
-  }
-  float denom = total + 1e-6f;
-  double acc = incl - run;
-  for (int k = 0; k < K; ++k) {
-    int i = lane * K + k;
-    if (i < SN) {
-      acc += (double)w[i];
-      cdf[i] = (float)acc / denom;
-      all[i] = z[(size_t)(active ? ray : 0) * SN + i];
-    }
-  }
-  __syncthreads();
-
-  const float c_first = cdf[0], c_last = cdf[SN - 1];
-  for (int k = lane; k < PN; k += 64) {
-    float u = U2[(size_t)k * u_stride + (active ? ray : 0)];
-    u = fminf(fmaxf(u, c_first), c_last);
-    int lo = 0, hi = SN;
-    while (lo < hi) {
-      int mid = (lo + hi) >> 1;
-      if (cdf[mid] < u) lo = mid + 1; else hi = mid;
-    }
-    int ri = lo < 1 ? 1 : (lo > SN - 1 ? SN - 1 : lo);
-    float cl = cdf[ri - 1], cr = cdf[ri], zl = all[ri - 1], zr = all[ri];
-    zf[k] = (u - cl) / (cr - cl + 1e-6f) * (zr - zl) + zl;
-  }
-  __syncthreads();
-  if (!active) return;
-
-  if (z_fine) {
-    for (int k = lane; k < PN; k += 64) {
-      float v = zf[k];
-      int rank = 0;
-      for (int j = 0; j < PN; ++j) {
-        float o = zf[j];
-        rank += (o < v || (o == v && j < k)) ? 1 : 0;
-      }
-      z_fine[(size_t)ray * PN + rank] = v;
-    }
-  }
-  const int T = SN + PN;
-  float* out = z_all + (size_t)ray * T;
-  bool sorted_coarse = true;
-  for (int k = lane; k + 1 < SN; k += 64) sorted_coarse = sorted_coarse && all[k] <= all[k + 1];
-  if (__builtin_amdgcn_ballot_w64(!sorted_coarse) == 0ull) {
-    float* fs = cdf;
-    for (int k = lane; k < PN; k += 64) {
-      const float v = zf[k];
-      int r = 0;
-      for (int j = 0; j < PN; ++j) {
-        const float o = zf[j];
-        r += (o < v || (o == v && j < k)) ? 1 : 0;
-      }
-      fs[r] = v;
-    }
-    __builtin_amdgcn_fence(__ATOMIC_RELEASE, "wavefront");
-    __builtin_amdgcn_wave_barrier();
-    __builtin_amdgcn_fence(__ATOMIC_ACQUIRE, "wavefront");
-    for (int k = lane; k < SN; k += 64) {
-      const float v = all[k];
-      int lo = 0, hi = PN;
-      while (lo < hi) { const int mid = (lo + hi) >> 1; if (fs[mid] < v) lo = mid + 1; else hi = mid; }
-      const int rank = k + lo;
-      out[rank] = v;
-      if (src_row) src_row[(size_t)ray * T + rank] = ray * SN + k;
-    }
-    for (int r = lane; r < PN; r += 64) {
-      const float v = fs[r];
-      int lo = 0, hi = SN;
-      while (lo < hi) { const int mid = (lo + hi) >> 1; if (all[mid] <= v) lo = mid + 1; else hi = mid; }
-      const int rank = r + lo;
-      out[rank] = v;
-      if (src_row) src_row[(size_t)ray * T + rank] = RN * SN + ray * PN + r;
-      if (z_new) z_new[(size_t)ray * PN + r] = v;
-    }
-    return;
-  }
-  for (int k = lane; k < T; k += 64) {
-    float v = all[k];
-    int rank = 0, rank_new = 0;
-    for (int j = 0; j < T; ++j) {
-      float o = all[j];
-      const int before = (o < v || (o == v && j < k)) ? 1 : 0;
-      rank += before;
-      rank_new += j >= SN ? before : 0;
-    }
-    out[rank] = v;
-    if (src_row) src_row[(size_t)ray * T + rank] = k < SN ? ray * SN + k : RN * SN + ray * PN + rank_new;
-    if (z_new && k >= SN) z_new[(size_t)ray * PN + rank_new] = v;
-  }
+  if (ray >= RN) return;
+  importance_merge_ray(lds[wave], ray, lane, weight, z, U2, u_stride, z_fine, z_all, RN, SN, PN, z_new, src_row);
 }
 
 hipError_t launch_importance_merge(const float* weight, const float* z, const float* U2, int u_stride, float* z_fine,
diff --git a/uforecon_amd/csrc/sampler_device.h b/uforecon_amd/csrc/sampler_device.h
--- /dev/null
+++ b/uforecon_amd/csrc/sampler_device.h
@@ -0,0 +1,167 @@
+#pragma once
+#include <hip/hip_runtime.h>
+#include <stdint.h>
+
+namespace ufr {
+
+__device__ __forceinline__ void ray_near_far(const int64_t* __restrict__ ray_idx, const float* __restrict__ cam_ray_d, int HW,
+                                             float near_z, float far_z, int i, int64_t& p, float& cz, float& n, float& f) {
+#pragma clang fp contract(off)
+  p = ray_idx[i];
+  const bool in_range = p >= 0 && p < (int64_t)HW;
+  p = in_range ? p : 0;
+  cz = cam_ray_d ? cam_ray_d[2 * (size_t)HW + p] : 1.f;
+  const float bad = __builtin_nanf("");
+  n = !in_range ? bad : cam_ray_d ? near_z / cz : near_z;
+  f = !in_range ? bad : cam_ray_d ? far_z / cz : far_z;
+}
+
+__device__ __forceinline__ float fixed_sample_z(float n, float f, float u, int s, int SN) {
+#pragma clang fp contract(off)
+  double step = 1.0 / (double)(SN - 1);
+  float lin = (s == SN - 1) ? 1.0f : (float)((double)s * step);
+  float zz = lin * (f - n) + n;
+  float interval = (float)(1.0 / (double)(SN - 1));
+  zz = zz + (u - 0.5f) * interval * (f - n);
+  return zz;
+}
+
+constexpr int kMaxS = 256;
+
+__device__ __forceinline__ double wave_incl_scan(double v, int lane) {
+#pragma unroll
+  for (int d = 1; d < 64; d <<= 1) {
+    double o = __shfl_up(v, d);
+    if (lane >= d) v += o;
+  }
+  return v;
+}
+
+__device__ __forceinline__ void wave_sync_memory() {
+  __builtin_amdgcn_fence(__ATOMIC_RELEASE, "wavefront");
+  __builtin_amdgcn_wave_barrier();
+  __builtin_amdgcn_fence(__ATOMIC_ACQUIRE, "wavefront");
+}
+
+__device__ __forceinline__ void importance_merge_ray(float* lds, int ray, int lane, const float* __restrict__ weight,
+                                                     const float* __restrict__ z, const float* __restrict__ U2,
+                                                     int u_stride, float* __restrict__ z_fine, float* __restrict__ z_all,
+                                                     int RN, int SN, int PN, float* __restrict__ z_new,
+                                                     int* __restrict__ src_row) {
+#pragma clang fp contract(off)
+  float* cdf = lds;
+  float* all = cdf + kMaxS;
+  float* zf = all + SN;
+  const float* w = weight + (size_t)ray * SN;
+
+  const int K = (SN + 63) / 64;
+  double run = 0.0;
+  for (int k = 0; k < K; ++k) {
+    int i = lane * K + k;
+    if (i < SN) run += (double)w[i];
+  }
+  double incl = wave_incl_scan(run, lane);
+  float total;
+  {
+    float a4[4] = {0.f, 0.f, 0.f, 0.f};
+    const int l8 = lane & 7;
+    for (int c = 0; c * 32 < SN; ++c)
+#pragma unroll
+      for (int k = 0; k < 4; ++k) {
+        int i = (c * 4 + k) * 8 + l8;
+        if (i < SN) a4[k] += w[i];
+      }
+    const float t = ((a4[0] + a4[1]) + a4[2]) + a4[3];
+    total = __shfl(t, 0);
+#pragma unroll
+    for (int l = 1; l < 8; ++l) total += __shfl(t, l);
+  }
+  float denom = total + 1e-6f;
+  double acc = incl - run;
+  for (int k = 0; k < K; ++k) {
+    int i = lane * K + k;
+    if (i < SN) {
+      acc += (double)w[i];
+      cdf[i] = (float)acc / denom;
+      all[i] = z[(size_t)ray * SN + i];
+    }
+  }
+  wave_sync_memory();
+
+  const float c_first = cdf[0], c_last = cdf[SN - 1];
+  for (int k = lane; k < PN; k += 64) {
+    float u = U2[(size_t)k * u_stride + ray];
+    u = fminf(fmaxf(u, c_first), c_last);
+    int lo = 0, hi = SN;
+    while (lo < hi) {
+      int mid = (lo + hi) >> 1;
+      if (cdf[mid] < u) lo = mid + 1; else hi = mid;
+    }
+    int ri = lo < 1 ? 1 : (lo > SN - 1 ? SN - 1 : lo);
+    float cl = cdf[ri - 1], cr = cdf[ri], zl = all[ri - 1], zr = all[ri];
+    zf[k] = (u - cl) / (cr - cl + 1e-6f) * (zr - zl) + zl;
+  }
+  wave_sync_memory();
+
+  if (z_fine) {
+    for (int k = lane; k < PN; k += 64) {
+      float v = zf[k];
+      int rank = 0;
+      for (int j = 0; j < PN; ++j) {
+        float o = zf[j];
+        rank += (o < v || (o == v && j < k)) ? 1 : 0;
+      }
+      z_fine[(size_t)ray * PN + rank] = v;
+    }
+  }
+  const int T = SN + PN;
+  float* out = z_all + (size_t)ray * T;
+  bool sorted_coarse = true;
+  for (int k = lane; k + 1 < SN; k += 64) sorted_coarse = sorted_coarse && all[k] <= all[k + 1];
+  if (__builtin_amdgcn_ballot_w64(!sorted_coarse) == 0ull) {
+    float* fs = cdf;
+    for (int k = lane; k < PN; k += 64) {
+      const float v = zf[k];
+      int r = 0;
+      for (int j = 0; j < PN; ++j) {
+        const float o = zf[j];
+        r += (o < v || (o == v && j < k)) ? 1 : 0;
+      }
+      fs[r] = v;
+    }
+    wave_sync_memory();
+    for (int k = lane; k < SN; k += 64) {
+      const float v = all[k];
+      int lo = 0, hi = PN;
+      while (lo < hi) { const int mid = (lo + hi) >> 1; if (fs[mid] < v) lo = mid + 1; else hi = mid; }
+      const int rank = k + lo;
+      out[rank] = v;
+      if (src_row) src_row[(size_t)ray * T + rank] = ray * SN + k;
+    }
+    for (int r = lane; r < PN; r += 64) {
+      const float v = fs[r];
+      int lo = 0, hi = SN;
+      while (lo < hi) { const int mid = (lo + hi) >> 1; if (all[mid] <= v) lo = mid + 1; else hi = mid; }
+      const int rank = r + lo;
+      out[rank] = v;
+      if (src_row) src_row[(size_t)ray * T + rank] = RN * SN + ray * PN + r;
+      if (z_new) z_new[(size_t)ray * PN + r] = v;
+    }
+    return;
+  }
+  for (int k = lane; k < T; k += 64) {
+    float v = all[k];
+    int rank = 0, rank_new = 0;
+    for (int j = 0; j < T; ++j) {
+      float o = all[j];
+      const int before = (o < v || (o == v && j < k)) ? 1 : 0;
+      rank += before;
+      rank_new += j >= SN ? before : 0;
+    }
+    out[rank] = v;
+    if (src_row) src_row[(size_t)ray * T + rank] = k < SN ? ray * SN + k : RN * SN + ray * PN + rank_new;
+    if (z_new && k >= SN) z_new[(size_t)ray * PN + rank_new] = v;
+  }
+}
+
+}
diff --git a/uforecon_amd/csrc/ufr_api.hip b/uforecon_amd/csrc/ufr_api.hip
--- a/uforecon_amd/csrc/ufr_api.hip
+++ b/uforecon_amd/csrc/ufr_api.hip
@@ -425,7 +425,8 @@
 
 static int aggregate_impl(const void* packed, const float* x_tokens, const float* x_point, const float* rgb, const float* dir, int RN, int SN,
                           int NV, float* radiance, float* srdf, float* token0, float* order_pe, bool pe_ready,
-                          float* view_out, float* ray_out, bool lowp, int* status, hipStream_t s) {
+                          float* view_out, float* ray_out, bool lowp, int* status, hipStream_t s,
+                          const RayEpilogue* epilogue = nullptr) {
   UFR_REQUIRE((unsigned long long)RN * SN * (NV + 1) * UFR_TOKEN_DIM < (1ull << 30),
               "view transformer: %d x %d points x %d tokens exceed the 2^30 token values one call addresses; chunk the points", RN, SN, NV + 1);
   {
@@ -437,7 +438,7 @@
   {
     ProfScope ps("ray_transformer", s);
     UFR_HIP(launch_ray_transformer(static_cast<const float*>(packed), token0, nullptr, order_pe, RN, SN, srdf, ray_out, lowp,
-                                   status, s));
+                                   status, s, epilogue));
   }
   return UFR_OK;
 }
@@ -830,7 +831,7 @@
 
 namespace {
 struct RenderWs {
-  float *ray_o, *rd, *near, *far, *camz, *z1, *w1, *srdf1, *depth1, *rgb1, *z2, *srdf2, *rad, *x, *xp, *rgbm, *dir, *token0,
+  float *ray_o, *rd, *camz, *z1, *w1, *srdf1, *depth1, *rgb1, *z2, *srdf2, *rad, *x, *xp, *rgbm, *dir, *token0,
       *pe1, *pe2, *z_new;
   int* row;
   size_t bytes;
@@ -841,8 +842,6 @@
   RenderWs r;
   r.ray_o = c.f32(4);
   r.rd = c.f32((size_t)R * 3);
-  r.near = c.f32(R);
-  r.far = c.f32(R);
   r.camz = c.f32(R);
   r.z1 = c.f32((size_t)R * SN);
   r.w1 = c.f32((size_t)R * SN);
@@ -904,9 +903,8 @@
   const int S2 = SN + PN, HW = f->H * f->W;
   {
     ProfScope p("sampler", s);
-    UFR_HIP(launch_ray_setup(a->ray_idx + r0, a->ray_d, a->cam_ray_d, HW, a->near_z, a->far_z, R, w.rd, w.near, w.far,
-                             w.camz, a->ray_o, w.ray_o, s));
-    UFR_HIP(launch_sample_fixed(w.near, w.far, a->U1 + r0, RN, w.z1, R, SN, s));
+    UFR_HIP(launch_ray_begin(a->ray_idx + r0, a->ray_d, a->cam_ray_d, HW, a->near_z, a->far_z, a->U1 + r0, RN, R, SN, w.rd, w.camz,
+                             w.z1, a->ray_o, w.ray_o, s));
     if (!pe_ready) {
       UFR_HIP(launch_order_pe(w.pe1, SN, s));
       if (!a->coarse_only) UFR_HIP(launch_order_pe(w.pe2, S2, s));
@@ -917,26 +915,33 @@
     ProfScope p("gather", s);
     UFR_HIP(launch_gather(*f, ps, w.ray_o, 0, w.rd, w.z1, R, SN, w.x, w.xp, w.rgbm, w.dir, nullptr, nullptr, nullptr, nullptr, nullptr, nullptr, s));
   }
+  const bool last = a->coarse_only != 0;
+  RayEpilogue ep{};
+  ep.z = w.z1;
+  ep.radiance = w.rad;
+  ep.variance = a->raw->variance;
+  ep.camz = w.camz;
+  ep.rgb = last ? a->rgb + 3 * (size_t)r0 : w.rgb1;
+  ep.depth = last ? a->depth + r0 : w.depth1;
+  ep.depth_z = (last && a->depth_z) ? a->depth_z + r0 : nullptr;
+  ep.weight = w.w1;
+  if (!last) {
+    ep.U2 = a->U2 + r0;
+    ep.u_stride = RN;
+    ep.PN = PN;
+    ep.z_all = w.z2;
+    ep.z_new = w.z_new;
+    ep.src_row = w.row;
+  }
   int rc = aggregate_impl(a->packed_weights, w.x, w.xp, w.rgbm, w.dir, R, SN, NV, w.rad, w.srdf1, w.token0, w.pe1, true,
-                          nullptr, nullptr, lowp, status, s);
-  if (rc != UFR_OK) return rc;
-  const bool last = a->coarse_only != 0;
-  {
-    ProfScope p("composite", s);
-    UFR_HIP(launch_composite(w.z1, w.rad, nullptr, w.srdf1, a->raw->variance, R, SN, last ? a->rgb + 3 * (size_t)r0 : w.rgb1,
-                             last ? a->depth + r0 : w.depth1, nullptr, w.w1, w.camz,
-                             (last && a->depth_z) ? a->depth_z + r0 : nullptr, s));
-  }
+                          nullptr, nullptr, lowp, status, s, &ep);
+  if (rc != UFR_OK) return rc;
   if (last) {
     if (a->srdf) UFR_HIP(hipMemcpyAsync(a->srdf + (size_t)r0 * SN, w.srdf1, (size_t)R * SN * 4, hipMemcpyDeviceToDevice, s));
     if (a->z_all) UFR_HIP(hipMemcpyAsync(a->z_all + (size_t)r0 * SN, w.z1, (size_t)R * SN * 4, hipMemcpyDeviceToDevice, s));
     return UFR_OK;
   }
   {
-    ProfScope p("sampler", s);
-    UFR_HIP(launch_importance_merge(w.w1, w.z1, a->U2 + r0, RN, nullptr, w.z2, R, SN, PN, w.z_new, w.row, s));
-  }
-  {
     ProfScope p("gather", s);
     UFR_HIP(launch_gather(*f, ps, w.ray_o, 0, w.rd, w.z_new, R, PN, w.x, w.xp, w.rgbm, w.dir, nullptr, nullptr, nullptr, nullptr, nullptr, nullptr, s));
   }
@@ -948,13 +953,17 @@
   }
   {
     ProfScope p("ray_transformer", s);
+    RayEpilogue ep2{};
+    ep2.z = w.z2;
+    ep2.radiance = w.rad;
+    ep2.rad_row = w.row;
+    ep2.variance = a->raw->variance;
+    ep2.camz = w.camz;
+    ep2.rgb = a->rgb + 3 * (size_t)r0;
+    ep2.depth = a->depth + r0;
+    ep2.depth_z = a->depth_z ? a->depth_z + r0 : nullptr;
     UFR_HIP(launch_ray_transformer(static_cast<const float*>(a->packed_weights), w.token0, w.row, w.pe2, R, S2, w.srdf2,
-                                   nullptr, lowp, status, s));
-  }
-  {
-    ProfScope p("composite", s);
-    UFR_HIP(launch_composite(w.z2, w.rad, w.row, w.srdf2, a->raw->variance, R, S2, a->rgb + 3 * (size_t)r0, a->depth + r0,
-                             nullptr, nullptr, w.camz, a->depth_z ? a->depth_z + r0 : nullptr, s));
+                                   nullptr, lowp, status, s, &ep2));
   }
   if (a->srdf) UFR_HIP(hipMemcpyAsync(a->srdf + (size_t)r0 * S2, w.srdf2, (size_t)R * S2 * 4, hipMemcpyDeviceToDevice, s));
   if (a->z_all) UFR_HIP(hipMemcpyAsync(a->z_all + (size_t)r0 * S2, w.z2, (size_t)R * S2 * 4, hipMemcpyDeviceToDevice, s));
diff --git a/uforecon_amd/csrc/ufr_internal.h b/uforecon_amd/csrc/ufr_internal.h
--- a/uforecon_amd/csrc/ufr_internal.h
+++ b/uforecon_amd/csrc/ufr_internal.h
@@ -52,6 +52,9 @@
                             const float* ray_o_host, float* ray_o_out, hipStream_t s);
 hipError_t launch_sample_fixed(const float* near, const float* far, const float* U, int u_stride, float* z, int RN,
                                int SN, hipStream_t s);
+hipError_t launch_ray_begin(const int64_t* ray_idx, const float* ray_d, const float* cam_ray_d, int HW, float near_z,
+                            float far_z, const float* U, int u_stride, int RN, int SN, float* rd_out, float* camz_out,
+                            float* z, const float* ray_o_host, float* ray_o_out, hipStream_t s);
 hipError_t launch_importance_merge(const float* weight, const float* z, const float* U2, int u_stride, float* z_fine,
                                    float* z_all, int RN, int SN, int PN, float* z_new, int* src_row, hipStream_t s);
 hipError_t launch_order_pe(float* table, int SN, hipStream_t s);
@@ -65,8 +68,19 @@
 hipError_t launch_view_transformer(const float* packed, const float* x_tokens, const float* x_point, const float* rgb,
                                    const float* dir, int P, int NV, float* token0, float* radiance, float* view_out, bool lowp, int* status,
                                    hipStream_t s);
+struct RayEpilogue {
+  const float *z, *radiance;
+  const int* rad_row;
+  const float *variance, *camz;
+  float *rgb, *depth, *depth_z, *weight;
+  const float* U2;
+  int u_stride, PN;
+  float *z_all, *z_new;
+  int* src_row;
+};
 hipError_t launch_ray_transformer(const float* packed, const float* token0, const int* tok_row, const float* order_pe,
-                                  int RN, int SN, float* srdf, float* ray_out, bool lowp, int* status, hipStream_t s);
+                                  int RN, int SN, float* srdf, float* ray_out, bool lowp, int* status, hipStream_t s,
+                                  const RayEpilogue* epilogue = nullptr);
 hipError_t launch_composite(const float* z, const float* radiance, const int* rad_row, const float* srdf,
                             const float* variance, int RN, int SN, float* rgb, float* depth, float* opacity, float* weight,
                             const float* camz, float* depth_z, hipStream_t s);
```

Result: no change. 2.671 million rays/s (-0.3%).
